# noway/nzcb-circom

Hardware: AMD Instinct MI355X
Metric: PLONK proofs/sec for nzcp_live (~2^21 constraints) at 1/2/4/8 MI355X (higher is better)
Workload: dtype u32 limbs: BN254 Fr/Fq Montgomery, 8x32-bit and 9x29-bit (MSM, NTT twiddles, quotient); 1 GPU; nzcp_live fullProve: NZCPPubIdentity(1,351,0,4,2,4) witness on the GPU (600560 signals) + PLONK proof, n=2^21, nPublic=3, 2970 inputs; domain_size=2097152, n_public=3, n_constraints=1785813, n_vars=1782570, n_additions=1182010, proofs_per_gpu=140, total_proofs=140, parallelism=batch-shard x1 (no collective), proofs_in_flight_per_gpu=5

## Files before the change

include/nzcb_internal.h:

```cpp
#ifndef NZCB_INTERNAL_H
#define NZCB_INTERNAL_H

#include "nzcb.h"

#ifdef __cplusplus
extern "C" {
#endif

int nzcb_ctx_kernel_stats(nzcb_ctx* ctx, int enable, double out[4]);

int nzcb_debug_guard_check(int device, size_t* checked, int* damaged, nzcb_err* err);
int nzcb_debug_guard_selftest(int device, nzcb_err* err);

#define NZCB_FAULT_QUOTIENT 1
#define NZCB_DEBUG_GENERIC_K 2
#define NZCB_FAULT_LANE_ALLOC 3
int nzcb_debug_inject_fault(nzcb_ctx* ctx, int kind);

int nzcb_debug_f29(int device, int op, const uint32_t* in, size_t count, uint32_t* out, nzcb_err* err);

int nzcb_synth_setup(int power, int n_public, int n_inputs, uint64_t seed, uint32_t n_constraints,
                     const uint8_t* tau, int device, uint8_t** zkey_out, size_t* zkey_len, uint8_t** wtns_out,
                     size_t* wtns_len, nzcb_err* err);
#define NZCB_SYNTH_FREE_PUBLIC 1u
int nzcb_synth_setup_ex(int power, int n_public, int n_inputs, uint64_t seed, uint32_t n_constraints, uint32_t flags,
                        const uint8_t* tau, int device, uint8_t** zkey_out, size_t* zkey_len, uint8_t** wtns_out,
                        size_t* wtns_len, nzcb_err* err);
typedef struct nzcb_engine nzcb_engine;
nzcb_engine* nzcb_engine_create(int device, int max_log_ntt, size_t max_msm_points, nzcb_err* err);
void nzcb_engine_destroy(nzcb_engine* e);
int nzcb_engine_ntt(nzcb_engine* e, const uint8_t* in_lem, uint8_t* out_lem, int log_n, int inverse, nzcb_err* err);
int nzcb_engine_msm(nzcb_engine* e, const uint8_t* bases_lem, const uint8_t* scalars, size_t n, int scalars_mont,
                    uint8_t* out_affine, nzcb_err* err);
int nzcb_debug_ntt_coset(nzcb_engine* e, const uint8_t* in_lem, uint8_t* out_lem, int log_n, const uint8_t* c_lem,
                         int fold_len, nzcb_err* err);
int nzcb_engine_ntt_dev(nzcb_engine* e, const void* in, void* out, int log_n, int inverse, nzcb_err* err);
int nzcb_engine_msm_dev(nzcb_engine* e, const void* bases, const void* scalars, size_t n, int scalars_mont,
                        uint8_t* out_affine, nzcb_err* err);
int nzcb_engine_time_ntt(nzcb_engine* e, const void* in, void* out, int log_n, int inverse, int reps, double* ms,
                         nzcb_err* err);
int nzcb_engine_random_fr(nzcb_engine* e, void* dev_out, size_t n, uint64_t seed, nzcb_err* err);
int nzcb_engine_fixed_base(nzcb_engine* e, const void* dev_scalars_mont, size_t n, void* dev_out, nzcb_err* err);
int nzcb_engine_lagrange_basis(nzcb_engine* e, const void* dev_ptau, size_t ptau_n, int log_n, void* dev_out,
                               nzcb_err* err);
int nzcb_engine_time_msm(nzcb_engine* e, const void* bases, const void* scalars, size_t n, int scalars_mont, int reps,
                         double* ms, double* acc_ms, nzcb_err* err);
int nzcb_engine_msm_fixed_dev(nzcb_engine* e, const void* bases, size_t n_table, const void* scalars, size_t n,
                              int scalars_mont, uint8_t* out_affine, nzcb_err* err);
int nzcb_engine_msm_table_dev(nzcb_engine* e, const void* bases, size_t n_table, const void* scalars, size_t n,
                              int scalars_mont, int window, int sparse, int fold, uint8_t* out_affine,
                              nzcb_err* err);
int nzcb_engine_msm_sets_dev(nzcb_engine* e, const void* bases, size_t n_table, const void* const* scalars, int sets,
                             size_t n, int scalars_mont, int sparse, uint8_t* out_affine, nzcb_err* err);
int nzcb_engine_time_msm2(nzcb_engine* e, const void* bases, const void* scalars, size_t n, int scalars_mont,
                          int fixed_base, int reps, double* out, nzcb_err* err);
int nzcb_engine_fr_mul(nzcb_engine* e, const uint8_t* a_lem, const uint8_t* b_lem, uint8_t* out_lem, size_t n,
                       int field_q, nzcb_err* err);

int nzcb_engine_g1_lincomb(int device, const uint8_t* points, const uint8_t* scalars, const uint32_t* group_end,
                           size_t groups, uint8_t* out, nzcb_err* err);
int nzcb_engine_verify_batch(const uint8_t* vk, const uint8_t* proofs, const uint8_t* pubs, size_t pub_stride,
                             int n_public, int count, int transcript_public, int device, const uint8_t* seed,
                             int* valid_out, uint8_t* points_out, int* pairing_checks, nzcb_err* err);
int nzcb_debug_verify_batch_timings(double* ms, int cap);

nzcb_r1cs* nzcb_engine_r1cs_create(const uint8_t* r1cs, size_t len, int device, uint32_t long_row_threshold,
                                   int witness_tile, nzcb_err* err);
int nzcb_debug_r1cs_check_timings(double* ms, int cap);

nzcb_p256_key* nzcb_engine_p256_key_create(const uint8_t pub_xy[64], int device, int window, nzcb_err* err);
#define NZCB_P256_OP_ADD 0
#define NZCB_P256_OP_SUB 1
#define NZCB_P256_OP_MUL 2
#define NZCB_P256_OP_SQR 3
#define NZCB_P256_OP_INV 4
int nzcb_debug_p256_field(int device, int op, int field, const uint8_t* a, const uint8_t* b, size_t count,
                          uint8_t* out, nzcb_err* err);
int nzcb_debug_p256_mul2(nzcb_p256_key* k, const uint8_t* u1, const uint8_t* u2, size_t count, uint8_t* out_xy,
                         nzcb_err* err);
int nzcb_debug_p256_timings(double* ms, int cap);

int nzcb_debug_nzcp_decode_timings(double* ms, int cap);

#ifdef __cplusplus
}
#endif
#endif
```

nzcb-circom_amd/csrc/capi_engine.hip:

```cpp
#include <chrono>
#include <cstring>
#include <map>
#include <memory>
#include <mutex>
#include <vector>

#include "../../include/nzcb_internal.h"
#include "engine.h"
#include "lagrange.h"

namespace nzcb {

Engine::Engine(int dev, int max_log_ntt, size_t max_msm_points) : device(dev) {
  NZ_HIP(hipSetDevice(dev));
  NZ_HIP(hipStreamCreateWithFlags(&stream, hipStreamNonBlocking));
  if (max_log_ntt >= 0) ntt_tables.init(max_log_ntt, stream);
  if (max_msm_points) msm_scratch.init(max_msm_points);
}

Engine::~Engine() {
  if (stream) (void)hipStreamDestroy(stream);
}

thread_local int g_guard_scope = 0;
// ... 8 lines not shown
  return m;
}
}

void guard_register(void* base, size_t bytes) {
  NZ_HIP(hipMemset((uint8_t*)base + bytes, kGuardByte, kGuardBytes));
  int dev = 0;
  NZ_HIP(hipGetDevice(&dev));
  std::lock_guard<std::mutex> lk(g_guard_mu);
  guard_map()[base] = GuardRec{bytes, dev};
}

void guard_unregister(void* base) {
  std::lock_guard<std::mutex> lk(g_guard_mu);
  guard_map().erase(base);
}

int guard_check(int device, size_t* checked, std::string* report) {
  std::vector<std::pair<void*, GuardRec>> recs;
  {
    std::lock_guard<std::mutex> lk(g_guard_mu);
    for (auto& kv : guard_map())
      if (device < 0 || kv.second.device == device) recs.push_back(kv);
  }
  std::vector<uint8_t> h(kGuardBytes);
  int bad = 0;
  for (auto& r : recs) {
    NZ_HIP(hipMemcpy(h.data(), (uint8_t*)r.first + r.second.bytes, kGuardBytes, hipMemcpyDeviceToHost));
    size_t k = 0;
    while (k < kGuardBytes && h[k] == kGuardByte) k++;
    if (k == kGuardBytes) continue;
    bad++;
    if (report && bad <= 8) {
      char line[160];
      std::snprintf(line, sizeof(line), "%sbuffer %p (%zu bytes, device %d): guard byte %zu overwritten",
                    report->empty() ? "" : "; ", r.first, r.second.bytes, r.second.device, k);
      *report += line;
    }
  }
  if (checked) *checked = recs.size();
  return bad;
}

__global__ void k_guard_poke(uint32_t* p, size_t at) {
  if (threadIdx.x == 0) p[at] = 0;
}

}

using namespace nzcb;

struct nzcb_engine {
  Engine eng;
  nzcb_engine(int d, int l, size_t m) : eng(d, l, m) {}
};

__global__ void fe_mul_kernel_r(const Fr* a, const Fr* b, Fr* o, size_t n) {
  size_t i = (size_t)blockIdx.x * blockDim.x + threadIdx.x;
  if (i < n) o[i] = a[i] * b[i];
}
__global__ void fe_mul_kernel_q(const Fq* a, const Fq* b, Fq* o, size_t n) {
  size_t i = (size_t)blockIdx.x * blockDim.x + threadIdx.x;
  if (i < n) o[i] = a[i] * b[i];
}

__global__ void random_fr_kernel(Fr* out, size_t n, uint64_t seed) {
  size_t i = (size_t)blockIdx.x * blockDim.x + threadIdx.x;
  if (i >= n) return;
  uint64_t x = seed ^ (0x9E3779B97F4A7C15ULL * (i + 1));
  Fr v;
  for (int k = 0; k < 4; k++) {
    x += 0x9E3779B97F4A7C15ULL;
    uint64_t z = x;
    z = (z ^ (z >> 30)) * 0xBF58476D1CE4E5B9ULL;
    z = (z ^ (z >> 27)) * 0x94D049BB133111EBULL;
    z ^= z >> 31;
    v.v[2 * k] = (uint32_t)z;
    v.v[2 * k + 1] = (uint32_t)(z >> 32);
  }
  v.v[7] &= 0x1fffffffu;
  out[i] = to_mont(v);
}

static void affine_out(const G1xyzz& r, uint8_t* out) {
  G1Affine a = xyzz_to_affine(r);
  Fq x = a.is_inf() ? Fq::zero() : from_mont(a.x);
  Fq y = a.is_inf() ? Fq::zero() : from_mont(a.y);
  std::memcpy(out, x.v, 32);
  std::memcpy(out + 32, y.v, 32);
}

extern "C" {

const char* nzcb_version(void) { return "nzcb-mi355x 0.1.0 (gfx950)"; }

int nzcb_device_count(void) {
  int n = 0;
  if (hipGetDeviceCount(&n) != hipSuccess) return 0;
  return n;
}

void nzcb_free(void* p) { std::free(p); }

nzcb_engine* nzcb_engine_create(int device, int max_log_ntt, size_t max_msm_points, nzcb_err* err) {
  return guarded_new<nzcb_engine>(
      err, [&] { return std::make_unique<nzcb_engine>(device, max_log_ntt, max_msm_points); });
}

void nzcb_engine_destroy(nzcb_engine* e) { delete e; }

void* nzcb_dev_alloc(size_t bytes) {
  void* p = nullptr;
  if (hipMalloc(&p, bytes) != hipSuccess) return nullptr;
  return p;
}
void* nzcb_dev_alloc_on(int device, size_t bytes) {
  int cur = 0;
  if (hipGetDevice(&cur) != hipSuccess || hipSetDevice(device) != hipSuccess) return nullptr;
  void* p = nullptr;
  if (hipMalloc(&p, bytes) != hipSuccess) p = nullptr;
  (void)hipSetDevice(cur);
  return p;
}
void nzcb_dev_free(void* p) {
  if (p) (void)hipFree(p);
}
int nzcb_memcpy_h2d(void* dst, const void* src, size_t bytes) {
  return hipMemcpy(dst, src, bytes, hipMemcpyHostToDevice) == hipSuccess ? 0 : NZCB_ERR_HIP;
}
int nzcb_memcpy_d2h(void* dst, const void* src, size_t bytes) {
  return hipMemcpy(dst, src, bytes, hipMemcpyDeviceToHost) == hipSuccess ? 0 : NZCB_ERR_HIP;
}
int nzcb_memcpy_d2d(void* dst, const void* src, size_t bytes) {
  if (hipMemcpyAsync(dst, src, bytes, hipMemcpyDeviceToDevice, nullptr) != hipSuccess) return NZCB_ERR_HIP;
  return hipStreamSynchronize(nullptr) == hipSuccess ? 0 : NZCB_ERR_HIP;
}
int nzcb_memcpy_d2d_async(void* dst, const void* src, size_t bytes, void* stream) {
  return hipMemcpyAsync(dst, src, bytes, hipMemcpyDeviceToDevice, (hipStream_t)stream) == hipSuccess ? 0
                                                                                              : NZCB_ERR_HIP;
}

int nzcb_engine_ntt_dev(nzcb_engine* e, const void* in, void* out, int log_n, int inverse, nzcb_err* err) {
  return guarded(err, [&] {
    Engine& g = e->eng;
    NZ_HIP(hipSetDevice(g.device));
    ntt(g.ntt_tables, (const Fr*)in, (Fr*)out, log_n, inverse != 0, g.stream);
    NZ_HIP(hipStreamSynchronize(g.stream));
  });
}

int nzcb_engine_ntt(nzcb_engine* e, const uint8_t* in_lem, uint8_t* out_lem, int log_n, int inverse, nzcb_err* err) {
  return guarded(err, [&] {
    Engine& g = e->eng;
    NZ_HIP(hipSetDevice(g.device));
    size_t n = size_t(1) << log_n;
    DevBuf<Fr> a(n), b(n);
    NZ_HIP(hipMemcpyAsync(a.p, in_lem, n * 32, hipMemcpyHostToDevice, g.stream));
    ntt(g.ntt_tables, a.p, b.p, log_n, inverse != 0, g.stream);
    NZ_HIP(hipMemcpyAsync(out_lem, b.p, n * 32, hipMemcpyDeviceToHost, g.stream));
    NZ_HIP(hipStreamSynchronize(g.stream));
  });
}

int nzcb_debug_ntt_coset(nzcb_engine* e, const uint8_t* in_lem, uint8_t* out_lem, int log_n, const uint8_t* c_lem,
                         int fold_len, nzcb_err* err) {
  return guarded(err, [&] {
    Engine& g = e->eng;
    if (log_n < 1 || log_n > g.ntt_tables.max_log || fold_len < 0 || (size_t)fold_len > (size_t(1) << log_n))
      throw Error(NZCB_ERR_ARG, "ntt coset: 1 <= log_n <= the engine's, 0 <= fold_len <= n");
    NZ_HIP(hipSetDevice(g.device));
    const size_t n = size_t(1) << log_n;
    Fr c;
    std::memcpy(c.v, c_lem, 32);
    DevBuf<Fr> a(n + (size_t)fold_len), b(n);
    DevBuf<NttTables::Tw> tw(n - 1);
    NZ_HIP(hipMemcpyAsync(a.p, in_lem, (n + (size_t)fold_len) * 32, hipMemcpyHostToDevice, g.stream));
    ntt_coset_twiddles(g.ntt_tables, c, log_n, tw.p, g.stream);
    NttIo io;
    io.in_len = n;
    io.tw = tw.p;
    if (fold_len) {
      Fr d = pow_u64(c, (uint64_t)n);
      for (int k = 0; k < 5; k++) d = d + d;
      io.fold_len = (size_t)fold_len;
      io.fold_n = n;
      io.fold_f = split29(d);
    }
    ntt(g.ntt_tables, a.p, b.p, log_n, false, g.stream, nullptr, &io);
    NZ_HIP(hipMemcpyAsync(out_lem, b.p, n * 32, hipMemcpyDeviceToHost, g.stream));
    NZ_HIP(hipStreamSynchronize(g.stream));
  });
}

int nzcb_engine_time_ntt(nzcb_engine* e, const void* in, void* out, int log_n, int inverse, int reps, double* ms,
                         nzcb_err* err) {
  return guarded(err, [&] {
    Engine& g = e->eng;
    NZ_HIP(hipSetDevice(g.device));
    hipEvent_t e0, e1;
    NZ_HIP(hipEventCreate(&e0));
    NZ_HIP(hipEventCreate(&e1));
    NZ_HIP(hipEventRecord(e0, g.stream));
    for (int i = 0; i < reps; i++) ntt(g.ntt_tables, (const Fr*)in, (Fr*)out, log_n, inverse != 0, g.stream);
    NZ_HIP(hipEventRecord(e1, g.stream));
    NZ_HIP(hipEventSynchronize(e1));
    float t = 0;
    NZ_HIP(hipEventElapsedTime(&t, e0, e1));
    *ms = t / (reps > 0 ? reps : 1);
    (void)hipEventDestroy(e0);
    (void)hipEventDestroy(e1);
  });
}

int nzcb_engine_msm_dev(nzcb_engine* e, const void* bases, const void* scalars, size_t n, int scalars_mont,
                        uint8_t* out_affine, nzcb_err* err) {
  return guarded(err, [&] {
    Engine& g = e->eng;
    NZ_HIP(hipSetDevice(g.device));
    G1xyzz r = msm(g.msm_scratch, (const G1Affine*)bases, (const Fr*)scalars, n, scalars_mont != 0, g.stream);
    affine_out(r, out_affine);
  });
}

int nzcb_engine_msm(nzcb_engine* e, const uint8_t* bases_lem, const uint8_t* scalars, size_t n, int scalars_mont,
                    uint8_t* out_affine, nzcb_err* err) {
  return guarded(err, [&] {
    Engine& g = e->eng;
    NZ_HIP(hipSetDevice(g.device));
    DevBuf<G1Affine> b(n ? n : 1);
    DevBuf<Fr> s(n ? n : 1);
    NZ_HIP(hipMemcpyAsync(b.p, bases_lem, n * 64, hipMemcpyHostToDevice, g.stream));
    NZ_HIP(hipMemcpyAsync(s.p, scalars, n * 32, hipMemcpyHostToDevice, g.stream));
    G1xyzz r = msm(g.msm_scratch, b.p, s.p, n, scalars_mont != 0, g.stream);
    affine_out(r, out_affine);
  });
}

int nzcb_engine_random_fr(nzcb_engine* e, void* dev_out, size_t n, uint64_t seed, nzcb_err* err) {
  return guarded(err, [&] {
    Engine& g = e->eng;
    NZ_HIP(hipSetDevice(g.device));
    hipLaunchKernelGGL(random_fr_kernel, dim3(grid_for(n, 256, 1u << 30)), dim3(256), 0, g.stream, (Fr*)dev_out, n,
                       seed);
    NZ_HIP(hipGetLastError());
    NZ_HIP(hipStreamSynchronize(g.stream));
  });
}

int nzcb_engine_fixed_base(nzcb_engine* e, const void* dev_scalars_mont, size_t n, void* dev_out, nzcb_err* err) {
  return guarded(err, [&] {
    Engine& g = e->eng;
    NZ_HIP(hipSetDevice(g.device));
    launch_fixed_base((const Fr*)dev_scalars_mont, n, (G1Affine*)dev_out, g.stream);
    NZ_HIP(hipStreamSynchronize(g.stream));
  });
}

int nzcb_engine_lagrange_basis(nzcb_engine* e, const void* dev_ptau, size_t ptau_n, int log_n, void* dev_out,
                               nzcb_err* err) {
  return guarded(err, [&] {
    Engine& g = e->eng;
    NZ_HIP(hipSetDevice(g.device));
    lagrange_basis((const G1Affine*)dev_ptau, ptau_n, log_n, (G1Affine*)dev_out, g.stream);
  });
}

int nzcb_engine_time_msm(nzcb_engine* e, const void* bases, const void* scalars, size_t n, int scalars_mont, int reps,
                         double* ms, double* acc_ms, nzcb_err* err) {
  return guarded(err, [&] {
    Engine& g = e->eng;
    NZ_HIP(hipSetDevice(g.device));
    MsmScratch& sc = g.msm_scratch;
    sc.prof = true;
    sc.prof_ms = 0;
    sc.prof_launches = 0;
    auto t0 = std::chrono::steady_clock::now();
    for (int i = 0; i < reps; i++)
      (void)msm(sc, (const G1Affine*)bases, (const Fr*)scalars, n, scalars_mont != 0, g.stream);
    *ms = std::chrono::duration<double, std::milli>(std::chrono::steady_clock::now() - t0).count() / (reps ? reps : 1);
    *acc_ms = sc.prof_ms / (sc.prof_launches ? sc.prof_launches : 1);
    sc.prof = false;
  });
}

int nzcb_engine_msm_fixed_dev(nzcb_engine* e, const void* bases, size_t n_table, const void* scalars, size_t n,
                              int scalars_mont, uint8_t* out_affine, nzcb_err* err) {
  return nzcb_engine_msm_table_dev(e, bases, n_table, scalars, n, scalars_mont, 0, 0, 0, out_affine, err);
}

int nzcb_engine_msm_table_dev(nzcb_engine* e, const void* bases, size_t n_table, const void* scalars, size_t n,
                              int scalars_mont, int window, int sparse, int fold, uint8_t* out_affine, nzcb_err* err) {
  return guarded(err, [&] {
    Engine& g = e->eng;
    NZ_HIP(hipSetDevice(g.device));
    if (n > n_table) throw Error(NZCB_ERR_ARG, "msm larger than its base table");
    if (window && (window < 16 || window > 20)) throw Error(NZCB_ERR_ARG, "msm table window: 16..20");
    MsmBaseTable t;
    t.build((const G1Affine*)bases, n_table, window ? window : fixed_base_window(), g.stream, fold != 0);
    t.sparse = sparse != 0;
    MsmScratch sc;
    sc.init(n ? n : 1, true);
    G1xyzz r = msm(sc, (const G1Affine*)bases, (const Fr*)scalars, n, scalars_mont != 0, g.stream, &t);
    affine_out(r, out_affine);
  });
}

int nzcb_engine_msm_sets_dev(nzcb_engine* e, const void* bases, size_t n_table, const void* const* scalars, int sets,
                             size_t n, int scalars_mont, int sparse, uint8_t* out_affine, nzcb_err* err) {
  return guarded(err, [&] {
    Engine& g = e->eng;
    NZ_HIP(hipSetDevice(g.device));
    if (n > n_table) throw Error(NZCB_ERR_ARG, "msm larger than its base table");
    if (sets < 1 || sets > 3 || !scalars) throw Error(NZCB_ERR_ARG, "msm sets: 1..3 scalar vectors");
    MsmBaseTable t;
    t.build((const G1Affine*)bases, n_table, lagrange_window(), g.stream);
    t.sparse = sparse != 0;
    MsmScratch sc;
    sc.init(n ? n : 1, true, 3, false);
    G1xyzz r[3] = {G1xyzz::inf(), G1xyzz::inf(), G1xyzz::inf()};
    msm_enqueue_sets(sc, (const Fr* const*)scalars, sets, n, scalars_mont != 0, g.stream, &t);
    msm_finish_sets(sc, g.stream, r);
    for (int k = 0; k < sets; k++) affine_out(r[k], out_affine + 64 * k);
  });
}

int nzcb_engine_time_msm2(nzcb_engine* e, const void* bases, const void* scalars, size_t n, int scalars_mont,
                          int fixed_base, int reps, double* out, nzcb_err* err) {
  return guarded(err, [&] {
    Engine& g = e->eng;
    NZ_HIP(hipSetDevice(g.device));
    std::unique_ptr<MsmBaseTable> t;
    std::unique_ptr<MsmScratch> own;
    MsmScratch* sc = &g.msm_scratch;
    double table_ms = 0;
    if (fixed_base) {
      auto t0 = std::chrono::steady_clock::now();
      t.reset(new MsmBaseTable());
      t->build((const G1Affine*)bases, n, fixed_base >= 2 ? lagrange_window() : fixed_base_window(), g.stream);
      t->sparse = fixed_base == 2;
      NZ_HIP(hipStreamSynchronize(g.stream));
      table_ms = std::chrono::duration<double, std::milli>(std::chrono::steady_clock::now() - t0).count();
      own.reset(new MsmScratch());
      own->init(n, true);
      sc = own.get();
    }
    sc->prof = true;
    sc->prof_phases = true;
    for (int w = 0; w < 3; w++)
      (void)msm(*sc, (const G1Affine*)bases, (const Fr*)scalars, n, scalars_mont != 0, g.stream, t.get());
    sc->prof_ms = 0;
    sc->prof_launches = 0;
    sc->prof_entries = 0;
    for (double& x : sc->phase_ms) x = 0;
    sc->host_ms = sc->enqueue_ms = sc->sort_host_ms = 0;
    auto t0 = std::chrono::steady_clock::now();
    for (int i = 0; i < reps; i++)
      (void)msm(*sc, (const G1Affine*)bases, (const Fr*)scalars, n, scalars_mont != 0, g.stream, t.get());
    const double r = reps > 0 ? reps : 1;
    out[0] = std::chrono::duration<double, std::milli>(std::chrono::steady_clock::now() - t0).count() / r;
    for (int i = 0; i < 7; i++) out[1 + i] = sc->phase_ms[i] / r;
    out[8] = table_ms;
    out[9] = (double)sc->prof_entries / r;
    out[10] = sc->host_ms / r;
    out[11] = sc->enqueue_ms / r;
    out[12] = sc->sort_host_ms / r;
    sc->prof = sc->prof_phases = false;
  });
}

int nzcb_engine_fr_mul(nzcb_engine* e, const uint8_t* a_lem, const uint8_t* b_lem, uint8_t* out_lem, size_t n,
                       int field_q, nzcb_err* err) {
  return guarded(err, [&] {
    Engine& g = e->eng;
    NZ_HIP(hipSetDevice(g.device));
    DevBuf<Fr> a(n), b(n), o(n);
    NZ_HIP(hipMemcpyAsync(a.p, a_lem, n * 32, hipMemcpyHostToDevice, g.stream));
    NZ_HIP(hipMemcpyAsync(b.p, b_lem, n * 32, hipMemcpyHostToDevice, g.stream));
    if (field_q)
      hipLaunchKernelGGL(fe_mul_kernel_q, dim3(grid_for(n, 256)), dim3(256), 0, g.stream, (const Fq*)a.p,
                         (const Fq*)b.p, (Fq*)o.p, n);
    else
      hipLaunchKernelGGL(fe_mul_kernel_r, dim3(grid_for(n, 256)), dim3(256), 0, g.stream, a.p, b.p, o.p, n);
    NZ_HIP(hipGetLastError());
    NZ_HIP(hipMemcpyAsync(out_lem, o.p, n * 32, hipMemcpyDeviceToHost, g.stream));
    NZ_HIP(hipStreamSynchronize(g.stream));
  });
}

struct nzcb_msm_table {
  int device = 0;
  size_t n = 0;
  MsmBaseTable table;
  MsmScratch sc;
  hipStream_t st = nullptr;
  ~nzcb_msm_table() {
    (void)hipSetDevice(device);
    if (st) (void)hipStreamDestroy(st);
  }
};

nzcb_msm_table* nzcb_msm_table_create(int device, const void* dev_bases, size_t n, nzcb_err* err) {
  return guarded_new<nzcb_msm_table>(err, [&] {
    if (!dev_bases || n == 0) throw Error(NZCB_ERR_ARG, "msm table: no bases");
    NZ_HIP(hipSetDevice(device));
    auto t = std::make_unique<nzcb_msm_table>();
    t->device = device;
    t->n = n;
    NZ_HIP(hipStreamCreateWithFlags(&t->st, hipStreamNonBlocking));
    t->table.build((const G1Affine*)dev_bases, n, fixed_base_window(), t->st);
    t->sc.init(n, true, 1, false);
    NZ_HIP(hipStreamSynchronize(t->st));
    return t;
  });
}

nzcb_msm_table* nzcb_msm_table_create_lagrange(int device, const void* dev_ptau, size_t ptau_n, int log_n, size_t lo,
                                               size_t hi, nzcb_err* err) {
  return guarded_new<nzcb_msm_table>(err, [&] {
    if (!dev_ptau || log_n < 1 || log_n > 28) throw Error(NZCB_ERR_ARG, "lagrange table: bad PTau or domain");
    const size_t nl = ((size_t)1 << log_n) + 2;
    if (ptau_n < nl) throw Error(NZCB_ERR_ARG, "lagrange table: fewer than n + 2 PTau points");
    if (lo >= hi || hi > nl) throw Error(NZCB_ERR_ARG, "lagrange table: bad point range");
    NZ_HIP(hipSetDevice(device));
    auto t = std::make_unique<nzcb_msm_table>();
    t->device = device;
    t->n = hi - lo;
    NZ_HIP(hipStreamCreateWithFlags(&t->st, hipStreamNonBlocking));
    {
      DevBuf<G1Affine> basis(nl);
      lagrange_basis((const G1Affine*)dev_ptau, ptau_n, log_n, basis.p, t->st);
      t->table.build(basis.p + lo, hi - lo, lagrange_window(), t->st);
      t->table.sparse = lagrange_sparse();
      NZ_HIP(hipStreamSynchronize(t->st));
    }
    t->sc.init(hi - lo, true, 1, false);
    return t;
  });
}

int nzcb_msm_table_run(nzcb_msm_table* t, const void* dev_scalars, size_t count, int scalars_mont,
                       uint8_t* out_affine, nzcb_err* err) {
  return guarded(err, [&] {
    if (!t || !out_affine || (count && !dev_scalars)) throw Error(NZCB_ERR_ARG, "msm table: null argument");
    if (count > t->n) throw Error(NZCB_ERR_ARG, "msm larger than its base table");
    NZ_HIP(hipSetDevice(t->device));
    G1xyzz r = count ? msm(t->sc, nullptr, (const Fr*)dev_scalars, count, scalars_mont != 0, t->st, &t->table)
                     : G1xyzz::inf();
    affine_out(r, out_affine);
  });
}

void nzcb_msm_table_destroy(nzcb_msm_table* t) { delete t; }

int nzcb_debug_guard_check(int device, size_t* checked, int* damaged, nzcb_err* err) {
  return guarded(err, [&] {
    std::string report;
    const int bad = guard_check(device, checked, &report);
    if (damaged) *damaged = bad;
    if (bad) throw Error(NZCB_ERR_INTERNAL, std::to_string(bad) + " damaged guard(s): " + report);
  });
}

int nzcb_debug_guard_selftest(int device, nzcb_err* err) {
  return guarded(err, [&] {
    NZ_HIP(hipSetDevice(device));
    size_t before = 0;
    guard_check(device, &before, nullptr);
    int bad = 0;
    {
      GuardScope gs;
      DevBuf<uint32_t> b(1000);
      hipLaunchKernelGGL(k_guard_poke, dim3(1), dim3(64), 0, nullptr, b.p, (size_t)1007);
      NZ_HIP(hipGetLastError());
      NZ_HIP(hipDeviceSynchronize());
      bad = guard_check(device, nullptr, nullptr);
    }
    const int after = guard_check(device, nullptr, nullptr);
    if (bad != 1 || after != 0)
      throw Error(NZCB_ERR_INTERNAL, "guard self-test: overrun found " + std::to_string(bad) + " time(s), " +
                                         std::to_string(after) + " left after release");
  });
}

}
```

nzcb-circom_amd/csrc/msm.h:

```cpp
#pragma once
#include <vector>

#include "common.h"
#include "ec.h"
#include "f29.h"

namespace nzcb {

struct MsmBaseTable {
  DevBuf<G1Affine> q;
  size_t n = 0, stride = 0;
  int c = 0, nw = 0;
  bool mont_folded = false;
  bool sparse = false;
  void build(const G1Affine* bases, size_t n, int c, hipStream_t st, bool fold_mont = false);
};

int fixed_base_window();
int lagrange_window();
bool lagrange_sparse();

struct MsmScratch {
  size_t max_points = 0;
  int max_lsets = 1;
  DevBuf<uint32_t> offsets;
  DevBuf<uint32_t> sorted;
  DevBuf<uint32_t> keys_in, keys_out, vals_in;
  DevBuf<uint8_t> sort_tmp;
  size_t sort_tmp_bytes = 0;
  DevBuf<uint32_t> bin_counts, vals_mid;
  DevBuf<uint32_t> lo_seg;
  DevBuf<G1xyzz> buckets;
  DevBuf<G1xyzz> carry_own;
  DevBuf<G1xyzz> carry_cont;
  DevBuf<Xyzz29> buckets29, carry_own29, carry_cont29;
  DevBuf<uint32_t> large;
  DevBuf<uint32_t> large_off;
  DevBuf<Xyzz29> large_part;
  DevBuf<Xyzz29> rowp29, colp29, lines29;
  DevBuf<G1xyzz> seg_tot;
  DevBuf<G1xyzz> seg_run;
  DevBuf<G1xyzz> parts;
  DevBuf<G1xyzz> win;
  G1xyzz* host_win = nullptr;
  uint32_t* host_total = nullptr;
  size_t host_win_cap = 0;
  int cur_c = 0, cur_nsets = 0, cur_nbits = 0, cur_seglen = 0;
  bool cur_fixed = false, cur_sparse = false;
  int cur_a = 0, cur_hb = 0;
  int cur_msets = 1;
  size_t cur_n = 0;
  uint32_t cur_nkeys = 0;
  bool prof = false, prof_phases = false;
  double prof_ms = 0;
  double phase_ms[7] = {0, 0, 0, 0, 0, 0, 0};
  double host_ms = 0;
  double enqueue_ms = 0;
  double sort_host_ms = 0;
  uint64_t prof_launches = 0, prof_points = 0, prof_entries = 0;
  hipEvent_t ev[8] = {nullptr, nullptr, nullptr, nullptr, nullptr, nullptr, nullptr, nullptr};
  hipEvent_t done = nullptr;
  void init(size_t max_points, bool fixed_base = false, int lagrange_sets = 1, bool generic = true);
  ~MsmScratch();
};

int msm_window_bits(size_t n);

void msm_enqueue(MsmScratch& sc, const G1Affine* bases, const Fr* scalars, size_t n, bool scalars_mont,
                 hipStream_t st, const MsmBaseTable* table = nullptr);
G1xyzz msm_finish(MsmScratch& sc, hipStream_t st);
void msm_enqueue_sets(MsmScratch& sc, const Fr* const* scalars, int sets, size_t n, bool scalars_mont,
                      hipStream_t st, const MsmBaseTable* table);
void msm_finish_sets(MsmScratch& sc, hipStream_t st, G1xyzz* out);

inline G1xyzz msm(MsmScratch& sc, const G1Affine* bases, const Fr* scalars, size_t n, bool mont, hipStream_t st,
                  const MsmBaseTable* table = nullptr) {
  msm_enqueue(sc, bases, scalars, n, mont, st, table);
  return msm_finish(sc, st);
}

G1Affine xyzz_to_affine(const G1xyzz& p);

}
```

nzcb-circom_amd/csrc/msm.hip:

```cpp
#include "msm.h"

#include "f29.h"

#include <chrono>
#include <cstdlib>
#include <type_traits>
#include <rocprim/rocprim.hpp>
#include <rocprofiler-sdk-roctx/roctx.h>

namespace nzcb {

static constexpr int kMsmThreads = 256;

#ifndef NZ_TAIL_PRIO
#define NZ_TAIL_PRIO 0
#endif
__device__ __forceinline__ void tail_prio() {
  if constexpr (NZ_TAIL_PRIO > 0) __builtin_amdgcn_s_setprio(NZ_TAIL_PRIO);
}

using SortConfig = rocprim::radix_sort_config<
    rocprim::default_config, rocprim::default_config,
    rocprim::radix_sort_onesweep_config<rocprim::kernel_config<1024, 16>, rocprim::kernel_config<1024, 16>, 10,
                                        rocprim::block_radix_rank_algorithm::match>>;

static void radix_sort(void* tmp, size_t& tmp_bytes, const uint32_t* kin, uint32_t* kout, const uint32_t* vin,
                       uint32_t* vout, size_t m, int end_bit, hipStream_t st) {
  NZ_HIP(rocprim::radix_sort_pairs<SortConfig>(tmp, tmp_bytes, kin, kout, vin, vout, m, 0, end_bit, st));
}

static constexpr uint32_t kChunk = 48;

static uint32_t chunk_for(size_t entries) {
  uint32_t c = kChunk;
  while (entries / c > (size_t(1) << 20)) c *= 2;
  return c;
}
static constexpr int kSegLen = 8;
static constexpr int kSumThreads = 256;
static constexpr int kSumPer = 4;
static constexpr int kPartThreads = 64;
static constexpr uint32_t kSeqSpan = 64;
static constexpr uint32_t kSeqSpan29 = 16;
static constexpr int kLargeBlocks = 32;
static constexpr int kLargePieceBlocks = 128;
static constexpr int kLargeFinalBlocks = 128;

static constexpr uint32_t kDynThreads = 1u << 18;
static constexpr uint32_t kDynMin = 8;
static constexpr uint32_t kSeqSpanSparse = 3;
static constexpr int kSparsePieceBlocks = 2048;
static constexpr int kSparseFinalBlocks = 512;
__host__ __device__ __forceinline__ uint32_t dyn_chunk(uint32_t m) {
  const uint32_t c = (m + kDynThreads - 1) / kDynThreads;
  return c < kDynMin ? kDynMin : c > kChunk ? kChunk : c;
}
static size_t dyn_threads_bound(size_t entries) {
  const size_t lo = std::min<size_t>(kDynThreads, (entries + kDynMin - 1) / kDynMin);
  return std::max<size_t>(lo, (entries + kChunk - 1) / kChunk);
}

static constexpr int kFbWindow = 20;
int fixed_base_window() {
  static const int c = [] {
    const char* e = std::getenv("NZCB_FB_WINDOW");
    const int v = e ? std::atoi(e) : kFbWindow;
    return (v >= 16 && v <= 20) ? v : kFbWindow;
  }();
  return c;
}

#ifndef NZ_LAGRANGE_WINDOW
#define NZ_LAGRANGE_WINDOW 17
#endif
int lagrange_window() { return NZ_LAGRANGE_WINDOW; }
bool lagrange_sparse() {
  static const bool v = [] {
    const char* e = std::getenv("NZCB_SPARSE");
    return e && std::atoi(e) != 0;
  }();
  return v;
}

int msm_window_bits(size_t n) {
  if (n >= (size_t(1) << 18)) return 16;
  int lg = ilog2(n ? n : 1);
  int c = lg - 3;
  if (c < 4) c = 4;
  if (c > 16) c = 16;
  return c;
}

static inline int num_windows(int c) { return (255 + c - 1) / c; }

template <int C, class F>
__device__ __forceinline__ void for_each_digit(const Fr& s, F&& f) {
  constexpr int NW = (255 + C - 1) / C;
  constexpr uint32_t MASK = (1u << C) - 1u;
  constexpr uint32_t HALF = 1u << (C - 1);
  uint32_t carry = 0;
#pragma unroll
  for (int w = 0; w < NW; w++) {
    const int bit = w * C;
    const int limb = bit >> 5;
    const int sh = bit & 31;
    uint64_t x = s.v[limb];
    if (limb + 1 < 8) x |= (uint64_t)s.v[limb + 1] << 32;
    uint32_t d = ((uint32_t)(x >> sh) & MASK) + carry;
    if (d > HALF) {
      uint32_t mag = (MASK + 1u) - d;
      if (mag) f(w, mag - 1u, 1u);
      carry = 1;
    } else {
      if (d) f(w, d - 1u, 0u);
      carry = 0;
    }
  }
}

#ifdef NZCB_MSM_STATS
template <class F>
static void for_each_digit_host(const Fr& s, int C, F&& f) {
  const int NW = (255 + C - 1) / C;
  const uint32_t MASK = (1u << C) - 1u, HALF = 1u << (C - 1);
  uint32_t carry = 0;
  for (int w = 0; w < NW; w++) {
    const int bit = w * C, limb = bit >> 5, sh = bit & 31;
    uint64_t x = s.v[limb];
    if (limb + 1 < 8) x |= (uint64_t)s.v[limb + 1] << 32;
    uint32_t d = ((uint32_t)(x >> sh) & MASK) + carry;
    if (d > HALF) {
      uint32_t mag = (MASK + 1u) - d;
      if (mag) f(w, mag - 1u, 1u);
      carry = 1;
    } else {
      if (d) f(w, d - 1u, 0u);
      carry = 0;
    }
  }
}
#endif

template <int C>
__global__ void __launch_bounds__(kMsmThreads)
msm_keys_kernel(const Fr* __restrict__ scalars, size_t n, int mont, uint32_t* __restrict__ keys,
                uint32_t* __restrict__ vals) {
  constexpr int NW = (255 + C - 1) / C;
  constexpr uint32_t NB = 1u << (C - 1);
  constexpr uint32_t SENTINEL = NW * NB;
  for (size_t i = (size_t)blockIdx.x * blockDim.x + threadIdx.x; i < n; i += (size_t)gridDim.x * blockDim.x) {
    Fr s = scalars[i];
    if (mont) s = from_mont_fr29(s);
    uint32_t k[NW];
#pragma unroll
    for (int w = 0; w < NW; w++) k[w] = SENTINEL;
    uint32_t sg[NW];
#pragma unroll
    for (int w = 0; w < NW; w++) sg[w] = 0;
    for_each_digit<C>(s, [&](int w, uint32_t b, uint32_t sign) {
      k[w] = (uint32_t)w * NB + b;
      sg[w] = sign << 31;
    });
#pragma unroll
    for (int w = 0; w < NW; w++) {
      keys[(size_t)w * n + i] = k[w];
      vals[(size_t)w * n + i] = (uint32_t)i | sg[w];
    }
  }
}

static constexpr int kBinThreads = 256;
static constexpr int kBinPer = 2;
static constexpr uint32_t kTileScalars = kBinThreads * kBinPer;
static constexpr int kLoThreads = 512;

static constexpr int kDigMont = 1;
static constexpr int kDigMinForm = 2;

__device__ __forceinline__ uint32_t scalar_min_form(Fr& s) {
  constexpr uint32_t H[8] = {0xf8000000u, 0xa1f0fac9u, 0x3cdcb848u, 0x9419f424u,
                             0x40c0ac2eu, 0xdc2822dbu, 0x7098d014u, 0x18322739u};
  bool gt = false, eq = true, lt_r = false, eq_r = true;
#pragma unroll
  for (int l = 7; l >= 0; l--) {
    gt = gt || (eq && s.v[l] > H[l]);
    eq = eq && s.v[l] == H[l];
    lt_r = lt_r || (eq_r && s.v[l] < FrParams::P[l]);
    eq_r = eq_r && s.v[l] == FrParams::P[l];
  }
  if (!(gt && lt_r)) return 0u;
  s = neg(s);
  return 1u;
}

template <int C, int NW>
__device__ __forceinline__ uint32_t bin_entries(const Fr* __restrict__ scalars, size_t i, int mont, size_t stride,
                                                uint32_t (&kk)[NW], uint32_t (&vv)[NW]) {
  Fr s = scalars[i];
  if (mont & kDigMont) s = from_mont_fr29(s);
  const uint32_t flip = (mont & kDigMinForm) ? scalar_min_form(s) : 0u;
  uint32_t live = 0;
#pragma unroll
  for (int w = 0; w < NW; w++) {
    kk[w] = 0;
    vv[w] = 0;
  }
  for_each_digit<C>(s, [&](int w, uint32_t b, uint32_t sign) {
    kk[w] = b;
    vv[w] = (uint32_t)((size_t)w * stride + i) | ((sign ^ flip) << 31);
    live |= 1u << w;
  });
  return live;
}

template <int KB> struct BinKeys {
  static constexpr int LO = KB - 8 > 8 ? KB - 8 : 8;
  using Lo = typename std::conditional<LO <= 8, uint8_t, uint16_t>::type;
  using Full = typename std::conditional<KB <= 16, uint16_t, uint32_t>::type;
};

static constexpr int kMaxSets = 3;
struct BinSets {
  const Fr* p[kMaxSets];
  uint32_t tps;
  uint32_t nb;
};

template <int C, int KB>
__global__ void __launch_bounds__(kBinThreads)
msm_bin_hist_kernel(BinSets sets, size_t n, int mont, uint32_t* __restrict__ counts, uint32_t ntiles) {
  constexpr int NW = (255 + C - 1) / C;
  constexpr int LO = BinKeys<KB>::LO;
  __shared__ uint32_t h[256];
  h[threadIdx.x] = 0;
  __syncthreads();
  const uint32_t set = blockIdx.x / sets.tps, lt = blockIdx.x - set * sets.tps;
  const Fr* __restrict__ scalars = sets.p[set];
  const uint32_t kbase = set * sets.nb;
#pragma unroll
  for (int j = 0; j < kBinPer; j++) {
    const size_t i = (size_t)lt * kTileScalars + (size_t)j * kBinThreads + threadIdx.x;
    if (i < n) {
      uint32_t kk[NW], vv[NW];
      const uint32_t live = bin_entries<C, NW>(scalars, i, mont, 0, kk, vv);
#pragma unroll
      for (int w = 0; w < NW; w++)
        if ((live >> w) & 1u) atomicAdd(&h[(kk[w] + kbase) >> LO], 1u);
    }
  }
  __syncthreads();
  counts[(size_t)threadIdx.x * ntiles + blockIdx.x] = h[threadIdx.x];
}

__device__ __forceinline__ uint32_t wave_incl_scan(uint32_t v) {
  const int lane = threadIdx.x & 63;
#pragma unroll
  for (int off = 1; off < 64; off <<= 1) {
    const uint32_t u = __shfl_up(v, off, 64);
    if (lane >= off) v += u;
  }
  return v;
}

__device__ __forceinline__ uint32_t scan256_excl(uint32_t v, uint32_t* wsum4, uint32_t& total) {
  const uint32_t inc = wave_incl_scan(threadIdx.x < 256 ? v : 0u);
  if (threadIdx.x < 256 && (threadIdx.x & 63) == 63) wsum4[threadIdx.x >> 6] = inc;
  __syncthreads();
  uint32_t off = 0;
  for (int w = 0; w < (int)(threadIdx.x >> 6) && w < 4; w++) off += wsum4[w];
  total = wsum4[0] + wsum4[1] + wsum4[2] + wsum4[3];
  __syncthreads();
  return threadIdx.x < 256 ? off + inc - v : 0u;
}

__global__ void __launch_bounds__(256)
msm_bin_rowscan_kernel(uint32_t* __restrict__ counts, uint32_t ntiles, uint32_t* __restrict__ tail) {
  __shared__ uint32_t wsum[4];
  uint32_t* row = counts + (size_t)blockIdx.x * ntiles;
  uint32_t carry = 0;
  for (uint32_t c0 = 0; c0 < ntiles; c0 += 256) {
    const uint32_t t = c0 + threadIdx.x;
    const uint32_t v = t < ntiles ? row[t] : 0u;
    uint32_t tot;
    const uint32_t ex = scan256_excl(v, wsum, tot);
    if (t < ntiles) row[t] = carry + ex;
    carry += tot;
  }
  if (threadIdx.x == 0) tail[blockIdx.x] = carry;
}

template <int C, int KB>
__global__ void __launch_bounds__(kBinThreads)
msm_bin_scatter_kernel(BinSets sets, size_t n, int mont, size_t stride, const uint32_t* __restrict__ counts,
                       uint32_t ntiles, typename BinKeys<KB>::Lo* __restrict__ lo2, uint32_t* __restrict__ vals2) {
  constexpr int NW = (255 + C - 1) / C;
  constexpr int TE = kTileScalars * NW;
  constexpr int LO = BinKeys<KB>::LO;
  __shared__ uint32_t lcount[256], lstart[256], gbase[256];
  __shared__ uint32_t lval[TE];
  __shared__ typename BinKeys<KB>::Full lkey[TE];
  const uint32_t set = blockIdx.x / sets.tps, lt = blockIdx.x - set * sets.tps;
  const Fr* __restrict__ scalars = sets.p[set];
  const uint32_t kbase = set * sets.nb;
  __shared__ uint32_t wsum[4];
  const uint32_t* tail = counts + (size_t)256 * ntiles;
  {
    uint32_t tot;
    const uint32_t st = scan256_excl(tail[threadIdx.x], wsum, tot);
    gbase[threadIdx.x] = st + counts[(size_t)threadIdx.x * ntiles + blockIdx.x];
    lcount[threadIdx.x] = 0;
  }
  __syncthreads();
  uint32_t kk[kBinPer][NW], vv[kBinPer][NW], rk[kBinPer][NW], live[kBinPer];
#pragma unroll
  for (int j = 0; j < kBinPer; j++) {
    const size_t i = (size_t)lt * kTileScalars + (size_t)j * kBinThreads + threadIdx.x;
    live[j] = 0;
    if (i < n) {
      live[j] = bin_entries<C, NW>(scalars, i, mont, stride, kk[j], vv[j]);
#pragma unroll
      for (int w = 0; w < NW; w++) {
        kk[j][w] += kbase;
        if ((live[j] >> w) & 1u) rk[j][w] = atomicAdd(&lcount[kk[j][w] >> LO], 1u);
      }
    }
  }
  __syncthreads();
  uint32_t total;
  {
    lstart[threadIdx.x] = scan256_excl(lcount[threadIdx.x], wsum, total);
  }
  __syncthreads();
#pragma unroll
  for (int j = 0; j < kBinPer; j++) {
#pragma unroll
    for (int w = 0; w < NW; w++) {
      if ((live[j] >> w) & 1u) {
        const uint32_t q = lstart[kk[j][w] >> LO] + rk[j][w];
        lkey[q] = (typename BinKeys<KB>::Full)kk[j][w];
        lval[q] = vv[j][w];
      }
    }
  }
  __syncthreads();
  for (uint32_t q = threadIdx.x; q < total; q += kBinThreads) {
    const uint32_t key = lkey[q], hb = key >> LO;
    const uint32_t pos = gbase[hb] + (q - lstart[hb]);
    lo2[pos] = (typename BinKeys<KB>::Lo)(key & ((1u << LO) - 1u));
    vals2[pos] = lval[q];
  }
}

template <int NT>
__device__ __forceinline__ uint32_t block_scan_excl(uint32_t* a, uint32_t count, uint32_t* wsum) {
  const uint32_t per = (count + NT - 1) / NT;
  const uint32_t b = threadIdx.x * per;
  uint32_t loc = 0;
  for (uint32_t i = 0; i < per; i++)
    if (b + i < count) loc += a[b + i];
  const uint32_t inc = wave_incl_scan(loc);
  if ((threadIdx.x & 63) == 63) wsum[threadIdx.x >> 6] = inc;
  __syncthreads();
  uint32_t off = 0, tot = 0;
#pragma unroll
  for (int w = 0; w < NT / 64; w++) {
    if (w < (int)(threadIdx.x >> 6)) off += wsum[w];
    tot += wsum[w];
  }
  uint32_t run = off + inc - loc;
  for (uint32_t i = 0; i < per; i++)
    if (b + i < count) {
      const uint32_t v = a[b + i];
      a[b + i] = run;
      run += v;
    }
  __syncthreads();
  return tot;
}

static constexpr uint32_t kLoSeg = 32768;
static constexpr uint32_t kLoU = 8;

__device__ __forceinline__ void lo_regions(const uint32_t* __restrict__ tail, uint32_t* wsum, uint32_t* rs,
                                           uint32_t* rf) {
  const uint32_t t = threadIdx.x;
  const uint32_t cnt = t < 256 ? tail[t] : 0u;
  uint32_t tot, nitems;
  const uint32_t st = scan256_excl(cnt, wsum, tot);
  const uint32_t f = scan256_excl((cnt + kLoSeg - 1) / kLoSeg, wsum, nitems);
  if (t < 256) {
    rs[t] = st;
    rf[t] = f;
  }
  if (t == 0) rf[256] = nitems;
  __syncthreads();
}

__device__ __forceinline__ uint32_t lo_region_of(const uint32_t* rf, uint32_t item) {
  uint32_t lo = 0, hi = 256;
  while (hi - lo > 1) {
    const uint32_t mid = (lo + hi) >> 1;
    if (rf[mid] <= item) lo = mid; else hi = mid;
  }
  return lo;
}

template <int LO>
__global__ void __launch_bounds__(kLoThreads)
msm_lo_count_kernel(const typename std::conditional<LO <= 8, uint8_t, uint16_t>::type* __restrict__ lo2,
                    const uint32_t* __restrict__ counts, uint32_t ntiles, uint32_t* __restrict__ segoff) {
  constexpr uint32_t NL = 1u << LO;
  __shared__ uint32_t h[NL], wsum[kLoThreads / 64], rs[256], rf[257];
  lo_regions(counts + (size_t)256 * ntiles, wsum, rs, rf);
  const uint32_t item = blockIdx.x;
  if (item >= rf[256]) return;
  const uint32_t r = lo_region_of(rf, item);
  const uint32_t* tail = counts + (size_t)256 * ntiles;
  const uint32_t s = rs[r] + (item - rf[r]) * kLoSeg;
  const uint32_t e = min(rs[r] + tail[r], s + kLoSeg);
  for (uint32_t i = threadIdx.x; i < NL; i += kLoThreads) h[i] = 0;
  __syncthreads();
  for (uint32_t p0 = s; p0 < e; p0 += kLoU * kLoThreads) {
    uint32_t k8[kLoU];
#pragma unroll
    for (uint32_t u = 0; u < kLoU; u++) {
      const uint32_t q = p0 + u * kLoThreads + threadIdx.x;
      k8[u] = q < e ? (uint32_t)lo2[q] : NL;
    }
#pragma unroll
    for (uint32_t u = 0; u < kLoU; u++)
      if (k8[u] < NL) atomicAdd(&h[k8[u]], 1u);
  }
  __syncthreads();
  for (uint32_t i = threadIdx.x; i < NL; i += kLoThreads) segoff[(size_t)item * NL + i] = h[i];
}

template <int LO>
__global__ void __launch_bounds__(kLoThreads)
msm_lo_scan_kernel(const uint32_t* __restrict__ counts, uint32_t ntiles, uint32_t* __restrict__ segoff,
                   uint32_t nkeys, uint32_t* __restrict__ offsets, uint32_t* __restrict__ large) {
  constexpr uint32_t NL = 1u << LO;
  __shared__ uint32_t h[NL], wsum[kLoThreads / 64], rs[256], rf[257];
  const uint32_t* tail = counts + (size_t)256 * ntiles;
  lo_regions(tail, wsum, rs, rf);
  const uint32_t hb = blockIdx.x;
  const uint32_t f0 = rf[hb], ns = rf[hb + 1] - f0, s = rs[hb];
  for (uint32_t i = threadIdx.x; i < NL; i += kLoThreads) {
    uint32_t run = 0;
    for (uint32_t g = 0; g < ns; g++) {
      uint32_t* c = segoff + (size_t)(f0 + g) * NL + i;
      const uint32_t v = *c;
      *c = run;
      run += v;
    }
    h[i] = run;
  }
  __syncthreads();
  block_scan_excl<kLoThreads>(h, NL, wsum);
  for (uint32_t i = threadIdx.x; i < NL; i += kLoThreads) {
    const uint32_t base = s + h[i];
    const uint32_t key = (hb << LO) | i;
    if (key < nkeys) offsets[key] = base;
    for (uint32_t g = 0; g < ns; g++) segoff[(size_t)(f0 + g) * NL + i] += base;
  }
  if (hb == 255 && threadIdx.x == 0) offsets[nkeys] = s + tail[255];
  if (hb == 0 && threadIdx.x == 0) large[0] = 0;
}

template <int LO, int NT = kLoThreads, uint32_t U = kLoU>
__global__ void __launch_bounds__(NT)
msm_lo_scatter_kernel(const typename std::conditional<LO <= 8, uint8_t, uint16_t>::type* __restrict__ lo2,
                      const uint32_t* __restrict__ vals2, const uint32_t* __restrict__ counts, uint32_t ntiles,
                      const uint32_t* __restrict__ segoff, uint32_t* __restrict__ sorted) {
  using Lo = typename std::conditional<LO <= 8, uint8_t, uint16_t>::type;
  constexpr uint32_t NL = 1u << LO;
  constexpr uint32_t kLoThreads = NT, kLoU = U;
  __shared__ uint32_t h[NL], lcnt[NL], lst[NL];
  __shared__ uint32_t wsum[kLoThreads / 64], rs[256], rf[257];
  __shared__ uint32_t lv[kLoU * kLoThreads];
  __shared__ Lo lk[kLoU * kLoThreads];
  lo_regions(counts + (size_t)256 * ntiles, wsum, rs, rf);
  const uint32_t item = blockIdx.x;
  if (item >= rf[256]) return;
  const uint32_t r = lo_region_of(rf, item);
  const uint32_t* tail = counts + (size_t)256 * ntiles;
  const uint32_t s = rs[r] + (item - rf[r]) * kLoSeg;
  const uint32_t e = min(rs[r] + tail[r], s + kLoSeg);
  for (uint32_t i = threadIdx.x; i < NL; i += kLoThreads) h[i] = segoff[(size_t)item * NL + i];
  for (uint32_t p0 = s; p0 < e; p0 += kLoU * kLoThreads) {
    uint32_t k8[kLoU], v8[kLoU], r8[kLoU];
    for (uint32_t i = threadIdx.x; i < NL; i += kLoThreads) lcnt[i] = 0;
    __syncthreads();
#pragma unroll
    for (uint32_t u = 0; u < kLoU; u++) {
      const uint32_t q = p0 + u * kLoThreads + threadIdx.x;
      k8[u] = q < e ? (uint32_t)lo2[q] : NL;
      v8[u] = q < e ? vals2[q] : 0u;
    }
#pragma unroll
    for (uint32_t u = 0; u < kLoU; u++) r8[u] = k8[u] < NL ? atomicAdd(&lcnt[k8[u]], 1u) : 0u;
    __syncthreads();
    for (uint32_t i = threadIdx.x; i < NL; i += kLoThreads) lst[i] = lcnt[i];
    __syncthreads();
    block_scan_excl<kLoThreads>(lst, NL, wsum);
#pragma unroll
    for (uint32_t u = 0; u < kLoU; u++)
      if (k8[u] < NL) {
        const uint32_t q = lst[k8[u]] + r8[u];
        lk[q] = (Lo)k8[u];
        lv[q] = v8[u];
      }
    __syncthreads();
    const uint32_t cnt = e - p0 < kLoU * kLoThreads ? e - p0 : kLoU * kLoThreads;
    for (uint32_t q = threadIdx.x; q < cnt; q += kLoThreads) {
      const uint32_t k = lk[q];
      sorted[h[k] + (q - lst[k])] = lv[q];
    }
    __syncthreads();
    for (uint32_t i = threadIdx.x; i < NL; i += kLoThreads) h[i] += lcnt[i];
  }
}

__global__ void __launch_bounds__(kMsmThreads)
msm_offsets_kernel(const uint32_t* __restrict__ skeys, size_t m, uint32_t nkeys, uint32_t* __restrict__ offsets) {
  size_t k = (size_t)blockIdx.x * blockDim.x + threadIdx.x;
  if (k > nkeys) return;
  size_t lo = 0, hi = m;
  while (lo < hi) {
    size_t mid = (lo + hi) >> 1;
    if (skeys[mid] < k) lo = mid + 1; else hi = mid;
  }
  offsets[k] = (uint32_t)lo;
}

__device__ __forceinline__ uint32_t find_key(const uint32_t* __restrict__ offsets, uint32_t nkeys, uint32_t pos) {
  uint32_t lo = 0, hi = nkeys;
  while (hi - lo > 1) {
    uint32_t mid = (lo + hi) >> 1;
    if (offsets[mid] <= pos) lo = mid; else hi = mid;
  }
  return lo;
}

__global__ void __launch_bounds__(kMsmThreads)
msm_accumulate_kernel(uint32_t chunk, const G1Affine* __restrict__ bases, const uint32_t* __restrict__ sorted,
                      const uint32_t* __restrict__ offsets, uint32_t nkeys, size_t nthreads,
                      G1xyzz* __restrict__ buckets, G1xyzz* __restrict__ carry_own,
                      G1xyzz* __restrict__ carry_cont) {
  size_t t = (size_t)blockIdx.x * blockDim.x + threadIdx.x;
  if (t >= nthreads) return;
  const uint32_t M = offsets[nkeys];
  const uint32_t s = (uint32_t)t * chunk;
  if (s >= M) return;
  const uint32_t e = (s + chunk < M) ? s + chunk : M;
  uint32_t k = find_key(offsets, nkeys, s);
  uint32_t kstart = offsets[k], kend = offsets[k + 1];
  G1xyzz acc = G1xyzz::inf();
  for (uint32_t pos = s; pos < e;) {
    const uint32_t ent = sorted[pos];
    const G1Affine P = bases[ent & 0x7fffffffu];
    if (!P.is_inf()) {
      Fq y = (ent >> 31) ? neg(P.y) : P.y;
      acc = xyzz_add_affine(acc, P.x, y);
    }
    pos++;
    if (pos == kend || pos == e) {
      const bool starts = kstart >= s;
      const bool ends = kend <= e;
      if (starts && ends) buckets[k] = acc;
      else if (!starts) carry_cont[t] = acc;
      else carry_own[t] = acc;
      acc = G1xyzz::inf();
      if (pos < e) {
        k = find_key(offsets, nkeys, pos);
        kstart = offsets[k];
        kend = offsets[k + 1];
      }
    }
  }
}

static __device__ __forceinline__ void mdbl29_rare(const F29& x, const F29& y, Xyzz29* out) { *out = mdbl29(x, y); }

__device__ __forceinline__ G1xyzz load_point(const G1xyzz& p) { return p; }
__device__ __forceinline__ G1xyzz load_point(const Xyzz29& a) {
  uint32_t z = 0;
#pragma unroll
  for (int i = 0; i < 9; i++) z |= a.ZZ.v[i];
  if (!z) return G1xyzz::inf();
  G1xyzz r;
  r.X = to_fq256(a.X);
  r.Y = to_fq256(a.Y);
  r.ZZ = to_fq256(a.ZZ);
  r.ZZZ = to_fq256(a.ZZZ);
  return r;
}

static constexpr uint32_t kLdsStride = kMsmThreads + 1;
template <bool kLdsIdx>
__global__ void __launch_bounds__(kMsmThreads) __attribute__((amdgpu_waves_per_eu(3, 8)))
msm_accumulate29_kernel(uint32_t chunk, const G1Affine* __restrict__ bases, const uint32_t* __restrict__ sorted,
                        const uint32_t* __restrict__ offsets, uint32_t nkeys, size_t nthreads,
                        Xyzz29* __restrict__ buckets, Xyzz29* __restrict__ carry_own,
                        Xyzz29* __restrict__ carry_cont) {
  __shared__ uint32_t sidx[kLdsIdx ? kChunk * kLdsStride : 1];
  const uint32_t t = blockIdx.x * blockDim.x + threadIdx.x;
  const uint32_t M = offsets[nkeys];
  if (!chunk) {
    chunk = dyn_chunk(M);
    tail_prio();
  }
  if (kLdsIdx) {
    const uint32_t wg0 = (uint32_t)blockIdx.x * kMsmThreads * chunk;
    if (wg0 >= M) return;
    const uint32_t inv = (uint32_t)((0x100000000ull + chunk - 1) / chunk);
    for (uint32_t j = threadIdx.x; j < kMsmThreads * chunk; j += kMsmThreads) {
      const uint32_t thr = __umulhi(j, inv), slot = j - thr * chunk;
      sidx[slot * kLdsStride + thr] = wg0 + j < M ? sorted[wg0 + j] : 0u;
    }
    __syncthreads();
  }
  if (t >= nthreads) return;
  const uint32_t s = (uint32_t)t * chunk;
  if (s >= M) return;
  const uint32_t e = (s + chunk < M) ? s + chunk : M;
  auto index_at = [&](uint32_t q) -> uint32_t {
    return kLdsIdx ? sidx[(q - s) * kLdsStride + threadIdx.x] : sorted[q];
  };
  uint32_t k = find_key(offsets, nkeys, s);
  uint32_t kstart = offsets[k], kend = offsets[k + 1];
  Xyzz29 acc;
  bool inf = true;
  uint32_t ent = index_at(s);
  G1Affine P = bases[ent & 0x7fffffffu];
  uint32_t ent_n = s + 1 < e ? index_at(s + 1) : 0u;
  for (uint32_t pos = s; pos < e;) {
    G1Affine Pn;
    uint32_t ent_nn = 0;
    if (pos + 1 < e) Pn = bases[ent_n & 0x7fffffffu];
    if (pos + 2 < e) ent_nn = index_at(pos + 2);
    if (!P.is_inf()) {
      const F29 x = split29(P.x);
      F29 y = split29(P.y);
      if (ent >> 31) y = neg29_nn(y);
      if (inf) {
        norm29(y);
        acc.X = x;
        acc.Y = y;
        acc.ZZ = f29_const(Fq29::ONE);
        acc.ZZZ = f29_const(Fq29::ONE);
        inf = false;
      } else {
        F29 U2, S2, PP, RR;
        mul29x2<Fq29>(x, acc.ZZ, y, acc.ZZZ, U2, S2);
        const F29 Pd = sub29(U2, acc.X, Fq29::K8);
        const F29 R = sub29(S2, acc.Y, Fq29::K4);
        sqr29x2(Pd, R, PP, RR);
        if (is0p29_fast(PP)) {
          if (is0p29(RR)) {
            norm29(y);
            mdbl29_rare(x, y, &acc);
          } else {
            inf = true;
          }
        } else {
          F29 PPP, Q, ZZ3, ZZZ3;
          mul29x2<Fq29>(Pd, PP, acc.X, PP, PPP, Q);
          const F29 X3 = sub2x29(RR, PPP, Q);
          mul29x2<Fq29>(acc.ZZ, PP, acc.ZZZ, PPP, ZZ3, ZZZ3);
          acc.Y = mul2sum29(R, sub29_nn(Q, X3, Fq29W::K10), neg4p29_nn(acc.Y), PPP);
          acc.ZZ = ZZ3;
          acc.ZZZ = ZZZ3;
          acc.X = X3;
        }
      }
    }
    pos++;
    if (pos == kend || pos == e) {
      const bool starts = kstart >= s;
      const bool ends = kend <= e;
      Xyzz29 out = acc;
      if (inf)
#pragma unroll
        for (int i = 0; i < 9; i++) out.ZZ.v[i] = 0;
      if (starts && ends) buckets[k] = out;
      else if (!starts) carry_cont[t] = out;
      else carry_own[t] = out;
      inf = true;
      while (pos < e && kend <= pos) {
        k++;
        kstart = kend;
        kend = offsets[k + 1];
      }
    }
    ent = ent_n;
    ent_n = ent_nn;
    P = Pn;
  }
}


__device__ __forceinline__ G1xyzz sum_run(const G1xyzz* carry_own, const G1xyzz* carry_cont, uint32_t c0,
                                          uint32_t c1) {
  G1xyzz v = carry_own[c0];
  for (uint32_t u = c0 + 1; u <= c1; u++) v = xyzz_add(v, carry_cont[u]);
  return v;
}

__global__ void __launch_bounds__(kMsmThreads)
msm_bucket_finalize_kernel(uint32_t chunk, const uint32_t* __restrict__ offsets, uint32_t nkeys, uint32_t span,
                           const G1xyzz* __restrict__ carry_own, const G1xyzz* __restrict__ carry_cont,
                           G1xyzz* __restrict__ buckets, uint32_t* __restrict__ large) {
  const size_t k = (size_t)blockIdx.x * blockDim.x + threadIdx.x;
  if (k >= nkeys) return;
  const uint32_t s = offsets[k], e = offsets[k + 1];
  if (e == s) return;
  const uint32_t c0 = s / chunk, c1 = (e - 1) / chunk;
  if (c0 == c1) return;
  if (c1 - c0 > span) {
    large[1 + atomicAdd(&large[0], 1u)] = (uint32_t)k;
    return;
  }
  buckets[k] = sum_run(carry_own, carry_cont, c0, c1);
}

__global__ void __launch_bounds__(kMsmThreads)
msm_finalize29_kernel(uint32_t chunk, const uint32_t* __restrict__ offsets, uint32_t nkeys, uint32_t span,
                      const Xyzz29* __restrict__ carry_own, const Xyzz29* __restrict__ carry_cont,
                      uint32_t* __restrict__ large, Xyzz29* __restrict__ out29) {
  tail_prio();
  __shared__ uint32_t pk[kMsmThreads], pu[kMsmThreads], pe[kMsmThreads];
  __shared__ uint32_t cnt;
  if (threadIdx.x == 0) cnt = 0;
  if (!chunk) chunk = dyn_chunk(offsets[nkeys]);
  __syncthreads();
  const size_t k = (size_t)blockIdx.x * blockDim.x + threadIdx.x;
  uint32_t c0 = 0, c1 = 0;
  bool mine = false;
  if (k < nkeys) {
    const uint32_t s = offsets[k], e = offsets[k + 1];
    if (e != s) {
      c0 = s / chunk;
      c1 = (e - 1) / chunk;
      if (c1 - c0 > span)
        large[1 + atomicAdd(&large[0], 1u)] = (uint32_t)k;
      else
        mine = c1 > c0;
    }
  }
  if (mine) {
    out29[k] = add29(carry_own[c0], carry_cont[c0 + 1]);
    if (c1 > c0 + 1) {
      const uint32_t i = atomicAdd(&cnt, 1u);
      pk[i] = (uint32_t)k;
      pu[i] = c0 + 2;
      pe[i] = c1;
    }
  }
  __syncthreads();
  if (threadIdx.x < cnt) {
    const uint32_t kk = pk[threadIdx.x], u1 = pe[threadIdx.x];
    Xyzz29 v = out29[kk];
    for (uint32_t u = pu[threadIdx.x]; u <= u1; u++) v = add29(v, carry_cont[u]);
    out29[kk] = v;
  }
}

__global__ void __launch_bounds__(kMsmThreads)
msm_bucket_reduce_kernel(const G1xyzz* __restrict__ buckets, const uint32_t* __restrict__ offsets, int nb,
                         int seglen, int nseg, int nsets, G1xyzz* __restrict__ seg_tot, G1xyzz* __restrict__ seg_run) {
  size_t t = (size_t)blockIdx.x * blockDim.x + threadIdx.x;
  if (t >= (size_t)nsets * nseg) return;
  const int w = (int)(t / nseg);
  const int g = (int)(t % nseg);
  const size_t base = (size_t)w * nb + (size_t)g * seglen;
  G1xyzz run = G1xyzz::inf(), tot = G1xyzz::inf();
  for (int j = seglen - 1; j >= 0; j--) {
    const uint32_t k = (uint32_t)(base + j);
    if (offsets[k + 1] != offsets[k]) run = xyzz_add(run, buckets[k]);
    if (!run.is_inf()) tot = xyzz_add(tot, run);
  }
  seg_tot[t] = tot;
  seg_run[t] = run;
}

__device__ __forceinline__ G1xyzz padd(const G1xyzz& a, const G1xyzz& b) { return xyzz_add(a, b); }
__device__ __forceinline__ Xyzz29 padd(const Xyzz29& a, const Xyzz29& b) { return add29(a, b); }
template <class P> __device__ __forceinline__ P pinf();
template <> __device__ __forceinline__ G1xyzz pinf<G1xyzz>() { return G1xyzz::inf(); }
template <> __device__ __forceinline__ Xyzz29 pinf<Xyzz29>() {
  Xyzz29 r;
#pragma unroll
  for (int i = 0; i < 9; i++) r.X.v[i] = r.Y.v[i] = r.ZZ.v[i] = r.ZZZ.v[i] = 0;
  return r;
}

template <int T, class Load, class Pt = G1xyzz>
__device__ __forceinline__ Pt block_sum(int per, Pt* sh, Load&& load) {
  constexpr int LG = T == 256 ? 8 : T == 128 ? 7 : T == 64 ? 6 : 5;
  const int tid = threadIdx.x;
  Pt acc = pinf<Pt>();
  for (int step = 0; step < per + LG; step++) {
    if (step == per) {
      sh[tid] = acc;
      __syncthreads();
    }
    bool doit;
    Pt lhs, rhs;
    if (step < per) {
      doit = load(step, rhs);
      lhs = acc;
    } else {
      const int stride = (T >> 1) >> (step - per);
      doit = tid < stride;
      if (doit) {
        lhs = sh[tid];
        rhs = sh[tid + stride];
      }
    }
    Pt r;
    if (doit) r = padd(lhs, rhs);
    if (step < per) {
      if (doit) acc = r;
    } else {
      if (doit) sh[tid] = r;
      __syncthreads();
    }
  }
  return sh[0];
}

__global__ void __launch_bounds__(kSumThreads)
msm_bucket_large_kernel(uint32_t chunk, const uint32_t* __restrict__ offsets, const uint32_t* __restrict__ large,
                        const G1xyzz* __restrict__ carry_own, const G1xyzz* __restrict__ carry_cont,
                        G1xyzz* __restrict__ buckets) {
  __shared__ G1xyzz sh[kSumThreads];
  const uint32_t count = large[0];
  for (uint32_t i = blockIdx.x; i < count; i += gridDim.x) {
    const uint32_t k = large[1 + i];
    const uint32_t c0 = offsets[k] / chunk, c1 = (offsets[k + 1] - 1) / chunk;
    const uint32_t span = c1 - c0 + 1;
    const int per = (int)((span + kSumThreads - 1) / kSumThreads);
    const G1xyzz r = block_sum<kSumThreads>(per, sh, [&](int step, G1xyzz& rhs) {
      const uint32_t u = (uint32_t)step * kSumThreads + threadIdx.x;
      if (u >= span) return false;
      rhs = u ? carry_cont[c0 + u] : carry_own[c0];
      return true;
    });
    if (threadIdx.x == 0) buckets[k] = r;
    __syncthreads();
  }
}

static constexpr uint32_t kPieceCarries = (uint32_t)kSumThreads;

__device__ __forceinline__ uint32_t carry_span(uint32_t chunk, const uint32_t* offsets, uint32_t k, uint32_t* c0) {
  *c0 = offsets[k] / chunk;
  return (offsets[k + 1] - 1) / chunk - *c0 + 1;
}

__global__ void __launch_bounds__(1024)
msm_large_scan_kernel(uint32_t chunk, const uint32_t* __restrict__ offsets, uint32_t nkeys,
                      const uint32_t* __restrict__ large, uint32_t* __restrict__ off) {
  tail_prio();
  __shared__ uint32_t sh[1024];
  const uint32_t count = large[0];
  const uint32_t ch = chunk ? chunk : dyn_chunk(offsets[nkeys]);
  const uint32_t tid = threadIdx.x;
  const uint32_t per = (count + 1023u) / 1024u;
  const uint32_t i0 = tid * per < count ? tid * per : count;
  const uint32_t i1 = i0 + per < count ? i0 + per : count;
  auto pieces = [&](uint32_t i) {
    uint32_t c0;
    return (carry_span(ch, offsets, large[1 + i], &c0) + kPieceCarries - 1) / kPieceCarries;
  };
  uint32_t sum = 0;
  for (uint32_t i = i0; i < i1; i++) sum += pieces(i);
  sh[tid] = sum;
  __syncthreads();
  for (uint32_t d = 1; d < 1024; d <<= 1) {
    const uint32_t v = tid >= d ? sh[tid - d] : 0u;
    __syncthreads();
    sh[tid] += v;
    __syncthreads();
  }
  uint32_t base = sh[tid] - sum;
  for (uint32_t i = i0; i < i1; i++) {
    off[i] = base;
    base += pieces(i);
  }
  if (tid == 1023) off[count] = sh[1023];
}

__device__ __forceinline__ Xyzz29 tree_sum29(Xyzz29 v, uint32_t cnt, Xyzz29* sh) {
  const uint32_t u = threadIdx.x;
  uint32_t h = 1;
  while (h < cnt) h <<= 1;
  h >>= 1;
  if (h) {
    if (u >= h && u < cnt) sh[u] = v;
    __syncthreads();
  }
  for (; h; h >>= 1) {
    if (u < h && u + h < cnt) v = add29(v, sh[u + h]);
    cnt = h;
    if (h > 1) {
      if (u >= (h >> 1) && u < h) sh[u] = v;
      __syncthreads();
    }
  }
  return v;
}

__global__ void __launch_bounds__(kSumThreads)
msm_large_piece29_kernel(uint32_t chunk, const uint32_t* __restrict__ offsets, uint32_t nkeys,
                         const uint32_t* __restrict__ large, const uint32_t* __restrict__ off,
                         const Xyzz29* __restrict__ carry_own, const Xyzz29* __restrict__ carry_cont,
                         Xyzz29* __restrict__ part) {
  tail_prio();
  __shared__ Xyzz29 sh[kSumThreads];
  const uint32_t count = large[0];
  const uint32_t total = off[count];
  const uint32_t ch = chunk ? chunk : dyn_chunk(offsets[nkeys]);
  for (uint32_t item = blockIdx.x; item < total; item += gridDim.x) {
    uint32_t lo = 0, hi = count;
    while (hi - lo > 1) {
      const uint32_t mid = (lo + hi) >> 1;
      if (off[mid] <= item) lo = mid; else hi = mid;
    }
    uint32_t c0;
    const uint32_t span = carry_span(ch, offsets, large[1 + lo], &c0);
    const uint32_t first = (item - off[lo]) * kPieceCarries;
    const uint32_t n = span - first < kPieceCarries ? span - first : kPieceCarries;
    const uint32_t u = first + threadIdx.x;
    Xyzz29 v;
    if (threadIdx.x < n) v = u ? carry_cont[c0 + u] : carry_own[c0];
    v = tree_sum29(v, n, sh);
    if (threadIdx.x == 0) part[item] = v;
    __syncthreads();
  }
}

template <int NT>
__global__ void __launch_bounds__(NT)
msm_large_final29_kernel(const uint32_t* __restrict__ large, const uint32_t* __restrict__ off,
                         const Xyzz29* __restrict__ part, Xyzz29* __restrict__ out29) {
  tail_prio();
  __shared__ Xyzz29 sh[NT];
  const uint32_t count = large[0];
  for (uint32_t i = blockIdx.x; i < count; i += gridDim.x) {
    const uint32_t p0 = off[i], np = off[i + 1] - p0;
    if (np == 1) {
      if (threadIdx.x == 0) out29[large[1 + i]] = part[p0];
      continue;
    }
    Xyzz29 v;
    if (threadIdx.x < np) v = part[p0 + threadIdx.x];
    for (uint32_t q = threadIdx.x + NT; q < np; q += NT) v = add29(v, part[p0 + q]);
    v = tree_sum29(v, np < NT ? np : NT, sh);
    if (threadIdx.x == 0) out29[large[1 + i]] = v;
    __syncthreads();
  }
}

__global__ void __launch_bounds__(kSumThreads)
msm_sums_kernel(const G1xyzz* __restrict__ seg_tot, const G1xyzz* __restrict__ seg_run, int nseg, int nslots,
                int nparts, G1xyzz* __restrict__ parts) {
  __shared__ G1xyzz sh[kSumThreads];
  const int p = blockIdx.x % nparts;
  const int wj = blockIdx.x / nparts;
  const int j = wj % nslots;
  const int w = wj / nslots;
  const int count = j == 0 ? nseg : nseg >> 1;
  const G1xyzz r = block_sum<kSumThreads>(kSumPer, sh, [&](int step, G1xyzz& rhs) {
    const int q = (p * kSumPer + step) * kSumThreads + (int)threadIdx.x;
    if (q >= count) return false;
    int g = q;
    if (j) {
      const int b = j - 1;
      g = ((q >> b) << (b + 1)) | (1 << b) | (q & ((1 << b) - 1));
    }
    rhs = j ? seg_run[(size_t)w * nseg + g] : seg_tot[(size_t)w * nseg + g];
    return true;
  });
  if (threadIdx.x == 0) parts[blockIdx.x] = r;
}

__global__ void __launch_bounds__(kPartThreads)
msm_parts_kernel(const G1xyzz* __restrict__ parts, int nparts, G1xyzz* __restrict__ out) {
  __shared__ G1xyzz sh[kPartThreads];
  const int per = (nparts + kPartThreads - 1) / kPartThreads;
  const G1xyzz r = block_sum<kPartThreads>(per, sh, [&](int step, G1xyzz& rhs) {
    const int q = step * kPartThreads + (int)threadIdx.x;
    if (q >= nparts) return false;
    rhs = parts[(size_t)blockIdx.x * nparts + q];
    return true;
  });
  if (threadIdx.x == 0) out[blockIdx.x] = r;
}

static constexpr int kTileSide = 16;
static constexpr int kLineThreads = 8;

__global__ void __launch_bounds__(256)
msm_tile29_kernel(const Xyzz29* __restrict__ buckets, const uint32_t* __restrict__ offsets, int a, int ltiles,
                  int htiles, Xyzz29* __restrict__ rowp, Xyzz29* __restrict__ colp) {
  tail_prio();
  __shared__ Xyzz29 sh[384];
  const int tid = threadIdx.x;
  const int ht = blockIdx.x / ltiles, lt = blockIdx.x - ht * ltiles;
  {
    const size_t per = (size_t)ltiles * htiles * kTileSide;
    buckets += (size_t)blockIdx.y * ltiles * htiles * kTileSide * kTileSide;
    offsets += (size_t)blockIdx.y * ltiles * htiles * kTileSide * kTileSide;
    rowp += blockIdx.y * per;
    colp += blockIdx.y * per;
  }
  {
    const int i = tid >> 4, j = tid & 15;
    const uint32_t k = ((uint32_t)(ht * kTileSide + i) << a) + (uint32_t)(lt * kTileSide + j);
    sh[tid] = offsets[k + 1] != offsets[k] ? buckets[k] : pinf<Xyzz29>();
  }
  __syncthreads();
#pragma unroll 1
  for (int s = 0; s < 4; s++) {
    const int m = 8 >> s;
    const bool act = tid < 32 * m;
    int l = 0, r = 0, d = 0;
    if (tid < 16 * m) {
      const int i = tid / m, j = tid - i * m;
      l = d = i * 16 + j;
      r = l + m;
    } else if (act) {
      const int u = tid - 16 * m, i = u >> 4, j = u & 15;
      const int base = s ? 256 : 0;
      l = base + i * 16 + j;
      r = base + (i + m) * 16 + j;
      d = 256 + i * 16 + j;
    }
    Xyzz29 x, y;
    if (act) {
      x = sh[l];
      y = sh[r];
    }
    __syncthreads();
    if (act) sh[d] = add29(x, y);
    __syncthreads();
  }
  if (tid < kTileSide)
    rowp[(size_t)(ht * kTileSide + tid) * ltiles + lt] = sh[tid * 16];
  else if (tid < 2 * kTileSide)
    colp[(size_t)(lt * kTileSide + tid - kTileSide) * htiles + ht] = sh[256 + tid - kTileSide];
}

static constexpr int kStrip = 16;
static constexpr int kStripMinC = 19;
__global__ void __launch_bounds__(256)
msm_strips29_kernel(const Xyzz29* __restrict__ buckets, const uint32_t* __restrict__ offsets, int a, int hb,
                    Xyzz29* __restrict__ rowp, Xyzz29* __restrict__ colp) {
  tail_prio();
  const int RJ = (1 << a) / kStrip, CI = (1 << hb) / kStrip;
  const size_t nrow = (size_t)RJ << hb, ncol = (size_t)CI << a;
  const size_t g = (size_t)blockIdx.x * 256 + threadIdx.x;
  if (g >= nrow + ncol) return;
  uint32_t k, step;
  size_t dst;
  Xyzz29* out;
  if (g < nrow) {
    const uint32_t h = (uint32_t)(g / RJ), j = (uint32_t)(g % RJ);
    k = (h << a) + j;
    step = (uint32_t)RJ;
    dst = g;
    out = rowp;
  } else {
    const size_t u = g - nrow;
    const uint32_t i = (uint32_t)(u >> a), l = (uint32_t)(u & ((1u << a) - 1));
    k = (i << a) + l;
    step = (uint32_t)CI << a;
    dst = (size_t)l * CI + i;
    out = colp;
  }
  Xyzz29 acc = pinf<Xyzz29>();
#pragma unroll 1
  for (int t = 0; t < kStrip; t++, k += step) {
    const Xyzz29 y = offsets[k + 1] != offsets[k] ? buckets[k] : pinf<Xyzz29>();
    acc = add29(acc, y);
  }
  out[dst] = acc;
}

__device__ __forceinline__ Xyzz29 shfl_xor29(const Xyzz29& v, int m) {
  Xyzz29 o;
#pragma unroll
  for (int i = 0; i < 9; i++) {
    o.X.v[i] = __shfl_xor(v.X.v[i], m);
    o.Y.v[i] = __shfl_xor(v.Y.v[i], m);
    o.ZZ.v[i] = __shfl_xor(v.ZZ.v[i], m);
    o.ZZZ.v[i] = __shfl_xor(v.ZZZ.v[i], m);
  }
  return o;
}

__global__ void __launch_bounds__(256)
msm_lines29_kernel(const Xyzz29* __restrict__ rowp, int ltiles, const Xyzz29* __restrict__ colp, int htiles,
                   int nrows, int ncols, Xyzz29* __restrict__ lines) {
  tail_prio();
  rowp += (size_t)blockIdx.y * nrows * ltiles;
  colp += (size_t)blockIdx.y * ncols * htiles;
  lines += (size_t)blockIdx.y * (nrows + ncols);
  constexpr int LG = kLineThreads == 8 ? 3 : kLineThreads == 4 ? 2 : kLineThreads == 16 ? 4 : 1;
  static_assert((1 << LG) == kLineThreads, "kLineThreads: 2, 4, 8 or 16");
  const int g = (int)((blockIdx.x * 256 + threadIdx.x) / kLineThreads);
  const int r = (int)(threadIdx.x & (kLineThreads - 1));
  const bool live = g < nrows + ncols;
  const bool row = g < nrows;
  const Xyzz29* src = row ? rowp + (size_t)g * ltiles : colp + (size_t)(g - nrows) * htiles;
  const int cnt = live ? (row ? ltiles : htiles) : 0;
  const int maxcnt = ltiles > htiles ? ltiles : htiles;
  const int nseq = (maxcnt + kLineThreads - 1) / kLineThreads - 1;
  Xyzz29 acc = r < cnt ? src[r] : pinf<Xyzz29>();
#pragma unroll 1
  for (int step = 0; step < nseq + LG; step++) {
    Xyzz29 y;
    if (step < nseq) {
      const int q = r + (step + 1) * kLineThreads;
      y = q < cnt ? src[q] : pinf<Xyzz29>();
    } else {
      y = shfl_xor29(acc, 1 << (step - nseq));
    }
    acc = add29(acc, y);
  }
  if (live && r == 0) lines[g] = acc;
}

__global__ void __launch_bounds__(kSumThreads)
msm_slots29_kernel(const Xyzz29* __restrict__ lines, int hb, int a, G1xyzz* __restrict__ out,
                   const uint32_t* __restrict__ entries, uint32_t* __restrict__ total_out) {
  tail_prio();
  lines += (size_t)blockIdx.y * (((size_t)1 << hb) + ((size_t)1 << a));
  out += (size_t)blockIdx.y * (hb + a + 1);
  __shared__ Xyzz29 sh[kSumThreads];
  const int s = blockIdx.x;
  const bool rows = s < hb;
  const bool plain = s == hb + a;
  const int b = rows ? s : s - hb;
  const int count = plain ? 1 << a : (rows ? 1 << (hb - 1) : 1 << (a - 1));
  const Xyzz29* src = rows ? lines : lines + ((size_t)1 << hb);
  const int per = (count + kSumThreads - 1) / kSumThreads;
  const Xyzz29 r = block_sum<kSumThreads>(per, sh, [&](int step, Xyzz29& rhs) {
    const int q = step * kSumThreads + (int)threadIdx.x;
    if (q >= count) return false;
    rhs = src[plain ? q : (((q >> b) << (b + 1)) | (1 << b) | (q & ((1 << b) - 1)))];
    return true;
  });
  if (threadIdx.x == 0) {
    host_put(out + s, load_point(r));
    if (s == 0 && blockIdx.y == 0 && total_out) host_put(total_out, *entries);
    host_put_done();
  }
}

__global__ void __launch_bounds__(kMsmThreads)
msm_table_kernel(const G1Affine* __restrict__ bases, size_t n, size_t stride, int c, int nw, Fq k261, int fold,
                 Fr kinv, G1Affine* __restrict__ q) {
  const size_t i = (size_t)blockIdx.x * blockDim.x + threadIdx.x;
  if (i >= n) return;
  const G1Affine P = bases[i];
  if (P.is_inf()) {
    for (int w = 0; w < nw; w++) q[(size_t)w * stride + i] = P;
    return;
  }
  G1xyzz acc = xyzz_from_affine(P);
  if (fold) {
    acc = G1xyzz::inf();
    for (int b = 253; b >= 0; b--) {
      acc = xyzz_dbl(acc);
      if ((kinv.v[b >> 5] >> (b & 31)) & 1u) acc = xyzz_add_affine(acc, P.x, P.y);
    }
  }
  for (int w = 0; w < nw; w++) {
    if (w)
      for (int k = 0; k < c; k++) acc = xyzz_dbl(acc);
    const Fq ti = inverse(acc.ZZ * acc.ZZZ);
    G1Affine r;
    r.x = acc.X * (acc.ZZZ * ti) * k261;
    r.y = acc.Y * (acc.ZZ * ti) * k261;
    q[(size_t)w * stride + i] = r;
  }
}

void MsmBaseTable::build(const G1Affine* bases, size_t npts, int cbits, hipStream_t st, bool fold_mont) {
  n = npts;
  mont_folded = fold_mont;
  stride = npts;
  c = cbits;
  nw = num_windows(c);
  if ((size_t)nw * stride >= (size_t(1) << 31)) throw Error(NZCB_ERR_ARG, "msm table too large for 31-bit indices");
  q.alloc((size_t)nw * stride);
  Fq thirty_two = Fq::zero();
  thirty_two.v[0] = 32;
  const Fq k261 = to_mont(thirty_two);
  Fr one_raw = Fr::zero();
  one_raw.v[0] = 1;
  const Fr kinv = from_mont(one_raw);
  hipLaunchKernelGGL(msm_table_kernel, dim3(grid_for(n, kMsmThreads, 1u << 30)), dim3(kMsmThreads), 0, st, bases, n,
                     stride, c, nw, k261, fold_mont ? 1 : 0, kinv, q.p);
  NZ_HIP(hipGetLastError());
}

static void lmark(const char* what) {
  static const bool on = std::getenv("NZCB_MARK_LAUNCHES") != nullptr;
  if (on) roctxMarkA(what);
}

static size_t lo_items_bound(size_t entries) { return 256 + entries / kLoSeg + 1; }

struct MsmPlan {
  int c, nw, nsets, seglen, nseg, nbits, nslots, nparts;
  int lb, a, hb, ltiles, htiles;
  int msets;
  uint32_t nb, nkeys;
  size_t entries;
};

static MsmPlan make_plan(size_t n, const MsmBaseTable* t, int msets = 1) {
  MsmPlan p;
  p.c = t ? t->c : msm_window_bits(n);
  p.nw = num_windows(p.c);
  p.nsets = t ? 1 : p.nw;
  p.msets = t ? msets : 1;
  p.nb = 1u << (p.c - 1);
  p.nkeys = p.nb * (uint32_t)p.nsets * (uint32_t)p.msets;
  p.seglen = (int)(p.nb < (uint32_t)kSegLen ? p.nb : kSegLen);
  p.nseg = (int)(p.nb / p.seglen);
  p.nbits = 0;
  while ((1 << p.nbits) < p.nseg) p.nbits++;
  p.nslots = p.nbits + 1;
  p.nparts = (p.nseg + kSumThreads * kSumPer - 1) / (kSumThreads * kSumPer);
  p.lb = p.c - 1;
  p.a = (p.lb + 1) / 2;
  p.hb = p.lb - p.a;
  p.ltiles = (1 << p.a) / kTileSide;
  p.htiles = (1 << p.hb) / kTileSide;
  p.entries = n * (size_t)p.nw * (size_t)p.msets;
  return p;
}

void MsmScratch::init(size_t maxp, bool fixed_base, int lagrange_sets, bool generic) {
  if (lagrange_sets < 1 || lagrange_sets > kMaxSets) throw Error(NZCB_ERR_ARG, "msm scratch: 1..3 Lagrange sets");
  if (!fixed_base) generic = true;
  max_points = maxp;
  max_lsets = lagrange_sets;
  size_t max_entries = 0, max_keys = 0, max_seg = 0, max_slots = 0, max_parts = 0, max_tiles = 0, max_lines = 0;
  auto fit = [&](const MsmPlan& p) {
    max_entries = std::max(max_entries, p.entries);
    max_keys = std::max(max_keys, (size_t)p.nkeys);
    if (p.nsets == 1) {
      max_slots = std::max(max_slots, (size_t)(p.lb + 1) * p.msets);
      max_tiles = std::max(max_tiles, (size_t)p.nb / kTileSide * p.msets);
      max_lines = std::max(max_lines, (((size_t)1 << p.hb) + ((size_t)1 << p.a)) * p.msets);
    } else {
      max_seg = std::max(max_seg, (size_t)p.nseg * p.nsets);
      max_slots = std::max(max_slots, (size_t)p.nslots * p.nsets);
      max_parts = std::max(max_parts, (size_t)p.nslots * p.nsets * p.nparts);
    }
  };
  for (size_t n = 1;; n <<= 1) {
    size_t m = n < maxp ? n : maxp;
    fit(make_plan(m, nullptr));
    if (m == maxp) break;
  }
  MsmPlan fp{};
  if (fixed_base) {
    MsmBaseTable t;
    t.c = fixed_base_window();
    fp = make_plan(maxp, &t);
    fit(fp);
    t.c = lagrange_window();
    const MsmPlan lp = make_plan(maxp, &t, lagrange_sets);
    fit(lp);
    if (lp.entries > fp.entries) fp = lp;
  }
  const size_t ge = generic ? max_entries : 1;
  offsets.alloc(max_keys + 1);
  sorted.alloc(max_entries);
  keys_in.alloc(ge);
  keys_out.alloc(max_entries);
  vals_in.alloc(ge);
  sort_tmp_bytes = 0;
  if (generic) {
    radix_sort(nullptr, sort_tmp_bytes, keys_in.p, keys_out.p, vals_in.p, sorted.p, max_entries, 21, nullptr);
  }
  sort_tmp.alloc(sort_tmp_bytes + 16);
  const size_t nthreads = std::max((max_entries + kChunk - 1) / kChunk, dyn_threads_bound(max_entries)) + 1;
  buckets.alloc(generic ? max_keys : 1);
  carry_own.alloc(generic ? nthreads : 1);
  carry_cont.alloc(generic ? nthreads : 1);
  large.alloc(max_keys + 1);
  if (fixed_base) {
    buckets29.alloc(max_keys);
    large_off.alloc(max_keys + 2);
    large_part.alloc(nthreads / kPieceCarries + max_keys + 1);
    carry_own29.alloc(nthreads);
    carry_cont29.alloc(nthreads);
    rowp29.alloc(max_tiles);
    colp29.alloc(max_tiles);
    lines29.alloc(max_lines);
    bin_counts.alloc((size_t)256 * ((maxp + kTileScalars - 1) / kTileScalars) * lagrange_sets + 256);
    vals_mid.alloc(max_entries);
    lo_seg.alloc(lo_items_bound(max_entries) * ((size_t)1 << BinKeys<19>::LO));
  }
  seg_tot.alloc(max_seg && generic ? max_seg : 1);
  seg_run.alloc(max_seg && generic ? max_seg : 1);
  parts.alloc(max_parts && generic ? max_parts : 1);
  win.alloc(max_slots);
  host_win_cap = max_slots;
  NZ_HIP(hipHostMalloc((void**)&host_win, (max_slots + 1) * sizeof(G1xyzz), hipHostMallocCoherent));
  host_total = (uint32_t*)(host_win + max_slots);
}

MsmScratch::~MsmScratch() {
  if (host_win) (void)hipHostFree(host_win);
  if (done) (void)hipEventDestroy(done);
  for (auto& e : ev)
    if (e) (void)hipEventDestroy(e);
}

static void keys_dispatch(int c, const Fr* scalars, size_t n, int mont, MsmScratch& sc, hipStream_t st) {
  auto launch = [&](auto cc) {
    constexpr int C = decltype(cc)::value;
    hipLaunchKernelGGL(msm_keys_kernel<C>, dim3(grid_for(n, kMsmThreads, 1u << 30)), dim3(kMsmThreads), 0, st,
                       scalars, n, mont, sc.keys_in.p, sc.vals_in.p);
  };
  switch (c) {
#define NZ_CASE(K) case K: launch(std::integral_constant<int, K>()); break;
    NZ_CASE(4) NZ_CASE(5) NZ_CASE(6) NZ_CASE(7) NZ_CASE(8) NZ_CASE(9) NZ_CASE(10) NZ_CASE(11) NZ_CASE(12)
    NZ_CASE(13) NZ_CASE(14) NZ_CASE(15) NZ_CASE(16)
#undef NZ_CASE
    default: throw Error(NZCB_ERR_INTERNAL, "bad msm window");
  }
  NZ_HIP(hipGetLastError());
}

G1Affine xyzz_to_affine(const G1xyzz& p) {
  G1Affine r;
  if (p.is_inf()) {
    r.x = Fq::zero();
    r.y = Fq::zero();
    return r;
  }
  r.x = p.X * inverse(p.ZZ);
  r.y = p.Y * inverse(p.ZZZ);
  return r;
}

template <class Mark>
static void fixed_bucketing(MsmScratch& sc, const MsmPlan& p, const BinSets& sets, size_t n, int mdig,
                            const MsmBaseTable* table, hipStream_t st, const Mark& mark) {
  const uint32_t tps = (uint32_t)((n + kTileScalars - 1) / kTileScalars);
  const uint32_t ntiles = tps * (uint32_t)p.msets;
  BinSets bs = sets;
  bs.tps = tps;
  bs.nb = p.nb;
  uint32_t* tail = sc.bin_counts.p + (size_t)256 * ntiles;
  auto run_bins = [&](auto cc, auto kb) {
    constexpr int C = decltype(cc)::value;
    constexpr int KB = decltype(kb)::value;
    using Lo = typename BinKeys<KB>::Lo;
    constexpr int LO = BinKeys<KB>::LO;
    Lo* lo2 = (Lo*)sc.keys_out.p;
    hipLaunchKernelGGL((msm_bin_hist_kernel<C, KB>), dim3(ntiles), dim3(kBinThreads), 0, st, bs, n, mdig,
                       sc.bin_counts.p, ntiles);
    NZ_HIP(hipGetLastError());
    lmark("mark: L hist");
    mark(1);
    hipLaunchKernelGGL(msm_bin_rowscan_kernel, dim3(256), dim3(256), 0, st, sc.bin_counts.p, ntiles, tail);
    lmark("mark: L rowscan");
    hipLaunchKernelGGL((msm_bin_scatter_kernel<C, KB>), dim3(ntiles), dim3(kBinThreads), 0, st, bs, n, mdig,
                       table->stride, sc.bin_counts.p, ntiles, lo2, sc.vals_mid.p);
    NZ_HIP(hipGetLastError());
    lmark("mark: L scatter");
    mark(2);
    const dim3 igrid((unsigned)lo_items_bound(p.entries));
    hipLaunchKernelGGL(msm_lo_count_kernel<LO>, igrid, dim3(kLoThreads), 0, st, (const Lo*)lo2, sc.bin_counts.p,
                       ntiles, sc.lo_seg.p);
    NZ_HIP(hipGetLastError());
    lmark("mark: L lo_count");
    hipLaunchKernelGGL(msm_lo_scan_kernel<LO>, dim3(256), dim3(kLoThreads), 0, st, sc.bin_counts.p, ntiles,
                       sc.lo_seg.p, p.nkeys, sc.offsets.p, sc.large.p);
    NZ_HIP(hipGetLastError());
    lmark("mark: L lo_scan");
    constexpr int sNT = LO > 8 ? 1024 : kLoThreads;
    constexpr uint32_t sU = LO > 8 ? 16 : kLoU;
    hipLaunchKernelGGL((msm_lo_scatter_kernel<LO, sNT, sU>), igrid, dim3(sNT), 0, st, (const Lo*)lo2, sc.vals_mid.p,
                       sc.bin_counts.p, ntiles, (const uint32_t*)sc.lo_seg.p, sc.sorted.p);
    NZ_HIP(hipGetLastError());
    lmark("mark: L lo_scatter");
  };
  using std::integral_constant;
  if (p.msets > 1) {
    if (p.c != 17) throw Error(NZCB_ERR_INTERNAL, "msm sets: the Lagrange window (17) only");
    run_bins(integral_constant<int, 17>(), integral_constant<int, 18>());
    return;
  }
  switch (p.c) {
    case 16: run_bins(integral_constant<int, 16>(), integral_constant<int, 15>()); break;
    case 17: run_bins(integral_constant<int, 17>(), integral_constant<int, 16>()); break;
    case 18: run_bins(integral_constant<int, 18>(), integral_constant<int, 17>()); break;
    case 19: run_bins(integral_constant<int, 19>(), integral_constant<int, 18>()); break;
    case 20: run_bins(integral_constant<int, 20>(), integral_constant<int, 19>()); break;
    default: throw Error(NZCB_ERR_INTERNAL, "bad fixed-base msm window");
  }
}

static void msm_enqueue_impl(MsmScratch& sc, const G1Affine* bases, const Fr* const* scalars, int msets, size_t n,
                             bool mont, hipStream_t st, const MsmBaseTable* table) {
  const auto t_enq = std::chrono::steady_clock::now();
  struct EnqueueClock {
    MsmScratch& sc;
    std::chrono::steady_clock::time_point t0;
    ~EnqueueClock() {
      if (sc.prof && sc.prof_phases)
        sc.enqueue_ms += std::chrono::duration<double, std::milli>(std::chrono::steady_clock::now() - t0).count();
    }
  } enqueue_clock{sc, t_enq};
  if (msets < 1 || msets > kMaxSets || (msets > 1 && (!table || msets > sc.max_lsets)))
    throw Error(NZCB_ERR_ARG, "msm sets: 1..3 over a table, within the scratch's sizing");
  sc.cur_n = n;
  sc.cur_msets = table ? msets : 1;
  if (n == 0) return;
  if (!sc.done) NZ_HIP(hipEventCreateWithFlags(&sc.done, hipEventDisableTiming));
  if (n > sc.max_points) throw Error(NZCB_ERR_ARG, "msm larger than scratch");
  if (table && n > table->n) throw Error(NZCB_ERR_ARG, "msm larger than its base table");
  if (table && table->mont_folded && !mont) throw Error(NZCB_ERR_ARG, "2^-256-folded table needs Montgomery scalars");
  if (table && (!sc.buckets29.p || !sc.bin_counts.p))
    throw Error(NZCB_ERR_ARG, "msm scratch was not sized for the fixed-base schedule");
  const int mdig = (mont && !(table && table->mont_folded)) ? 1 : 0;
  const MsmPlan p = make_plan(n, table, msets);
#ifdef NZCB_MSM_STATS
  if (table && !table->mont_folded) {
    NZ_HIP(hipStreamSynchronize(st));
    for (int k = 0; k < msets; k++) {
      std::vector<Fr> h(n);
      NZ_HIP(hipMemcpy(h.data(), scalars[k], n * sizeof(Fr), hipMemcpyDeviceToHost));
      size_t e_pos = 0, e_min = 0, nneg = 0, zero = 0, hist[17] = {0};
      for (size_t i = 0; i < n; i++) {
        Fr v = mdig ? from_mont(h[i]) : h[i];
        if (v.is_zero()) { zero++; continue; }
        const Fr w = neg(v);
        auto digits = [&](const Fr& x) {
          size_t d = 0;
          for_each_digit_host(x, p.c, [&](int, uint32_t, uint32_t) { d++; });
          return d;
        };
        const size_t dp = digits(v), dn = digits(w);
        e_pos += dp;
        e_min += dp <= dn ? dp : dn;
        if (dn < dp) nneg++;
        const size_t dm = dp <= dn ? dp : dn;
        hist[dm < 16 ? dm : 16]++;
      }
      fprintf(stderr, "MSMSCALARS set=%d n=%zu c=%d zero=%zu entries=%zu entries_minform=%zu flipped=%zu hist_minform=",
              k, n, p.c, zero, e_pos, e_min, nneg);
      for (int b = 0; b < 17; b++) fprintf(stderr, "%zu%c", hist[b], b == 16 ? '\n' : ',');
    }
  }
#endif
  if (p.entries > sc.sorted.n || p.nkeys + 1 > sc.offsets.n)
    throw Error(NZCB_ERR_ARG, "msm scratch was not sized for this schedule");
  if (table && ((size_t)p.nb / kTileSide * msets > sc.rowp29.n ||
                (((size_t)1 << p.hb) + ((size_t)1 << p.a)) * msets > sc.lines29.n ||
                (size_t)(p.lb + 1) * msets > sc.host_win_cap || (msets > 1 && p.c >= kStripMinC)))
    throw Error(NZCB_ERR_ARG, "msm scratch was not sized for this window");
  sc.cur_c = p.c;
  sc.cur_nsets = p.nsets;
  sc.cur_nbits = p.nbits;
  sc.cur_seglen = p.seglen;
  sc.cur_nkeys = p.nkeys;
  sc.cur_fixed = table != nullptr;
  sc.cur_a = p.a;
  sc.cur_hb = p.hb;
  sc.cur_msets = p.msets;
  const bool phases = sc.prof && sc.prof_phases;
  if (sc.prof && !sc.ev[0])
    for (auto& e : sc.ev) NZ_HIP(hipEventCreate(&e));
  auto mark = [&](int i) {
    if (phases) NZ_HIP(hipEventRecord(sc.ev[i], st));
  };
  mark(0);
  if (table) {
    BinSets bs{};
    for (int k = 0; k < msets; k++) bs.p[k] = scalars[k];
    fixed_bucketing(sc, p, bs, n, mdig | (table->mont_folded ? 0 : kDigMinForm), table, st, mark);
  } else {
    keys_dispatch(p.c, scalars[0], n, mdig, sc, st);
    mark(1);
    size_t tmp = sc.sort_tmp_bytes;
    int end_bit = 1;
    while ((1u << end_bit) <= p.nkeys) end_bit++;
    const auto t_sort = std::chrono::steady_clock::now();
    radix_sort(sc.sort_tmp.p, tmp, sc.keys_in.p, sc.keys_out.p, sc.vals_in.p, sc.sorted.p, p.entries, end_bit, st);
    if (phases)
      sc.sort_host_ms += std::chrono::duration<double, std::milli>(std::chrono::steady_clock::now() - t_sort).count();
    mark(2);
    hipLaunchKernelGGL(msm_offsets_kernel, dim3(grid_for((size_t)p.nkeys + 1, kMsmThreads, 1u << 30)),
                       dim3(kMsmThreads), 0, st, sc.keys_out.p, p.entries, p.nkeys, sc.offsets.p);
    NZ_HIP(hipGetLastError());
  }
  if (sc.prof) NZ_HIP(hipEventRecord(sc.ev[3], st));
  const bool sparse = table && table->sparse;
  sc.cur_sparse = sparse;
  const uint32_t chunk = sparse ? 0u : chunk_for(p.entries);
  const size_t nthreads = sparse ? dyn_threads_bound(p.entries) : (p.entries + chunk - 1) / chunk;
  const dim3 agrid(grid_for(nthreads, kMsmThreads, 1u << 30));
  const G1Affine* gather = table ? table->q.p : bases;
  if (table) {
    if (chunk == kChunk || sparse)
      hipLaunchKernelGGL(msm_accumulate29_kernel<true>, agrid, dim3(kMsmThreads), 0, st, chunk, gather, sc.sorted.p,
                         sc.offsets.p, p.nkeys, nthreads, sc.buckets29.p, sc.carry_own29.p, sc.carry_cont29.p);
    else
      hipLaunchKernelGGL(msm_accumulate29_kernel<false>, agrid, dim3(kMsmThreads), 0, st, chunk, gather, sc.sorted.p,
                         sc.offsets.p, p.nkeys, nthreads, sc.buckets29.p, sc.carry_own29.p, sc.carry_cont29.p);
  } else {
    hipLaunchKernelGGL(msm_accumulate_kernel, agrid, dim3(kMsmThreads), 0, st, chunk, gather, sc.sorted.p, sc.offsets.p,
                       p.nkeys, nthreads, sc.buckets.p, sc.carry_own.p, sc.carry_cont.p);
  }
  NZ_HIP(hipGetLastError());
  lmark("mark: L accumulate");
  if (sc.prof) NZ_HIP(hipEventRecord(sc.ev[4], st));
  const dim3 fgrid(grid_for(p.nkeys, kMsmThreads, 1u << 30));
  if (table) {
    hipLaunchKernelGGL(msm_finalize29_kernel, fgrid, dim3(kMsmThreads), 0, st, chunk, sc.offsets.p, p.nkeys,
                       sparse ? kSeqSpanSparse : kSeqSpan29, (const Xyzz29*)sc.carry_own29.p,
                       (const Xyzz29*)sc.carry_cont29.p, sc.large.p, sc.buckets29.p);
    NZ_HIP(hipGetLastError());
    lmark("mark: L finalize");
    hipLaunchKernelGGL(msm_large_scan_kernel, dim3(1), dim3(1024), 0, st, chunk, sc.offsets.p, p.nkeys, sc.large.p,
                       sc.large_off.p);
    NZ_HIP(hipGetLastError());
    lmark("mark: L large_scan");
    hipLaunchKernelGGL(msm_large_piece29_kernel, dim3(sparse ? kSparsePieceBlocks : kLargePieceBlocks),
                       dim3(kSumThreads), 0, st, chunk, sc.offsets.p, p.nkeys, sc.large.p, sc.large_off.p,
                       (const Xyzz29*)sc.carry_own29.p, (const Xyzz29*)sc.carry_cont29.p, sc.large_part.p);
    NZ_HIP(hipGetLastError());
    lmark("mark: L piece");
    if (sparse)
      hipLaunchKernelGGL(msm_large_final29_kernel<kSumThreads>, dim3(kSparseFinalBlocks), dim3(kSumThreads), 0, st,
                         sc.large.p, sc.large_off.p, sc.large_part.p, sc.buckets29.p);
    else
      hipLaunchKernelGGL(msm_large_final29_kernel<64>, dim3(kLargeFinalBlocks), dim3(64), 0, st, sc.large.p,
                         sc.large_off.p, sc.large_part.p, sc.buckets29.p);
    NZ_HIP(hipGetLastError());
    lmark("mark: L final");
    mark(5);
    int lparts = p.ltiles, hparts = p.htiles;
    if (p.c >= kStripMinC) {
      lparts = (1 << p.a) / kStrip;
      hparts = (1 << p.hb) / kStrip;
      const size_t nthr = ((size_t)lparts << p.hb) + ((size_t)hparts << p.a);
      hipLaunchKernelGGL(msm_strips29_kernel, dim3(grid_for(nthr, 256, 1u << 30)), dim3(256), 0, st,
                         (const Xyzz29*)sc.buckets29.p, sc.offsets.p, p.a, p.hb, sc.rowp29.p, sc.colp29.p);
    } else {
      hipLaunchKernelGGL(msm_tile29_kernel, dim3((unsigned)(p.ltiles * p.htiles), (unsigned)p.msets), dim3(256), 0, st,
                         (const Xyzz29*)sc.buckets29.p, sc.offsets.p, p.a, p.ltiles, p.htiles, sc.rowp29.p, sc.colp29.p);
    }
    NZ_HIP(hipGetLastError());
    mark(6);
    const int nrows = 1 << p.hb, ncols = 1 << p.a;
    hipLaunchKernelGGL(msm_lines29_kernel, dim3(grid_for((size_t)(nrows + ncols) * kLineThreads, 256), (unsigned)p.msets),
                       dim3(256), 0,
                       st, (const Xyzz29*)sc.rowp29.p, lparts, (const Xyzz29*)sc.colp29.p, hparts, nrows, ncols,
                       sc.lines29.p);
    NZ_HIP(hipGetLastError());
    lmark("mark: L lines");
    hipLaunchKernelGGL(msm_slots29_kernel, dim3(p.hb + p.a + 1, (unsigned)p.msets), dim3(kSumThreads), 0, st,
                       (const Xyzz29*)sc.lines29.p, p.hb, p.a, sc.host_win, (const uint32_t*)sc.offsets.p + p.nkeys,
                       sc.prof ? sc.host_total : nullptr);
    NZ_HIP(hipGetLastError());
    lmark("mark: L slots");
    mark(7);
    NZ_HIP(hipEventRecord(sc.done, st));
    return;
  }
  NZ_HIP(hipMemsetAsync(sc.large.p, 0, sizeof(uint32_t), st));
  hipLaunchKernelGGL(msm_bucket_finalize_kernel, fgrid, dim3(kMsmThreads), 0, st, chunk, sc.offsets.p, p.nkeys,
                     kSeqSpan, (const G1xyzz*)sc.carry_own.p, (const G1xyzz*)sc.carry_cont.p, sc.buckets.p, sc.large.p);
  NZ_HIP(hipGetLastError());
  hipLaunchKernelGGL(msm_bucket_large_kernel, dim3(kLargeBlocks), dim3(kSumThreads), 0, st, chunk, sc.offsets.p,
                     sc.large.p, (const G1xyzz*)sc.carry_own.p, (const G1xyzz*)sc.carry_cont.p, sc.buckets.p);
  NZ_HIP(hipGetLastError());
  mark(5);
  hipLaunchKernelGGL(msm_bucket_reduce_kernel, dim3(grid_for((size_t)p.nsets * p.nseg, kMsmThreads, 1u << 30)),
                     dim3(kMsmThreads), 0, st, sc.buckets.p, sc.offsets.p, (int)p.nb, p.seglen, p.nseg, p.nsets,
                     sc.seg_tot.p, sc.seg_run.p);
  NZ_HIP(hipGetLastError());
  mark(6);
  hipLaunchKernelGGL(msm_sums_kernel, dim3(p.nsets * p.nslots * p.nparts), dim3(kSumThreads), 0, st, sc.seg_tot.p,
                     sc.seg_run.p, p.nseg, p.nslots, p.nparts, sc.parts.p);
  NZ_HIP(hipGetLastError());
  hipLaunchKernelGGL(msm_parts_kernel, dim3(p.nsets * p.nslots), dim3(kPartThreads), 0, st, sc.parts.p, p.nparts,
                     sc.win.p);
  NZ_HIP(hipGetLastError());
  mark(7);
  if (sc.prof) NZ_HIP(hipMemcpyAsync(sc.host_total, sc.offsets.p + p.nkeys, 4, hipMemcpyDeviceToHost, st));
  NZ_HIP(hipMemcpyAsync(sc.host_win, sc.win.p, (size_t)p.nsets * p.nslots * sizeof(G1xyzz), hipMemcpyDeviceToHost,
                        st));
  NZ_HIP(hipEventRecord(sc.done, st));
}

void msm_enqueue(MsmScratch& sc, const G1Affine* bases, const Fr* scalars, size_t n, bool mont, hipStream_t st,
                 const MsmBaseTable* table) {
  const Fr* one[1] = {scalars};
  msm_enqueue_impl(sc, bases, one, 1, n, mont, st, table);
}

void msm_enqueue_sets(MsmScratch& sc, const Fr* const* scalars, int sets, size_t n, bool mont, hipStream_t st,
                      const MsmBaseTable* table) {
  if (!table) throw Error(NZCB_ERR_ARG, "msm sets: a table schedule");
  msm_enqueue_impl(sc, nullptr, scalars, sets, n, mont, st, table);
}

static G1xyzz fixed_window_result(const G1xyzz* s, int hb, int a) {
  G1xyzz acc = G1xyzz::inf();
  for (int b = hb - 1; b >= 0; b--) acc = xyzz_add(xyzz_dbl(acc), s[b]);
  for (int i = 0; i < a; i++) acc = xyzz_dbl(acc);
  G1xyzz col = G1xyzz::inf();
  for (int b = a - 1; b >= 0; b--) col = xyzz_add(xyzz_dbl(col), s[hb + b]);
  return xyzz_add(xyzz_add(acc, col), s[hb + a]);
}

void msm_finish_sets(MsmScratch& sc, hipStream_t st, G1xyzz* out) {
  const int msets = sc.cur_msets;
  if (sc.cur_n == 0) {
    for (int k = 0; k < msets; k++) out[k] = G1xyzz::inf();
    return;
  }
  out[0] = msm_finish(sc, st);
  for (int k = 1; k < msets; k++) out[k] = fixed_window_result(sc.host_win + (size_t)k * (sc.cur_hb + sc.cur_a + 1),
                                                               sc.cur_hb, sc.cur_a);
}

G1xyzz msm_finish(MsmScratch& sc, hipStream_t st) {
  if (sc.cur_n == 0) return G1xyzz::inf();
  NZ_HIP(hipEventSynchronize(sc.done));
#ifdef NZCB_MSM_STATS
  if (sc.cur_fixed) {
    std::vector<uint32_t> off(sc.cur_nkeys + 1);
    NZ_HIP(hipMemcpy(off.data(), sc.offsets.p, off.size() * 4, hipMemcpyDeviceToHost));
    uint32_t cnt = 0;
    NZ_HIP(hipMemcpy(&cnt, sc.large.p, 4, hipMemcpyDeviceToHost));
    uint32_t pieces = 0;
    NZ_HIP(hipMemcpy(&pieces, sc.large_off.p + cnt, 4, hipMemcpyDeviceToHost));
    const uint32_t M = off.back();
    const uint32_t chunk = sc.cur_sparse ? dyn_chunk(M) : chunk_for(sc.cur_n * (size_t)num_windows(sc.cur_c));
    size_t h[12] = {0};
    uint32_t mx = 0;
    uint64_t carries_large = 0, carries_mid = 0;
    for (uint32_t k = 0; k < sc.cur_nkeys; k++) {
      if (off[k + 1] == off[k]) { h[0]++; continue; }
      const uint32_t sp = (off[k + 1] - 1) / chunk - off[k] / chunk + 1;
      mx = sp > mx ? sp : mx;
      int b = 1;
      while (b < 11 && sp > (1u << (b - 1))) b++;
      h[b]++;
      if (sp > (sc.cur_sparse ? kSeqSpanSparse : kSeqSpan29) + 1) carries_large += sp; else if (sp > 1) carries_mid += sp;
    }
    fprintf(stderr, "MSMSTATS n=%zu c=%d entries=%u chunk=%u large=%u pieces=%u maxspan=%u carries_mid=%llu "
            "carries_large=%llu spans[empty,1,2,<=4,<=8,..,<=512,>512]=", sc.cur_n, sc.cur_c, M, chunk, cnt, pieces, mx,
            (unsigned long long)carries_mid, (unsigned long long)carries_large);
    for (int b = 0; b < 12; b++) fprintf(stderr, "%zu%c", h[b], b == 11 ? '\n' : ',');
  }
#endif
  const int c = sc.cur_c, nsets = sc.cur_nsets, nslots = sc.cur_nbits + 1;
  if (sc.prof) {
    float t = 0;
    NZ_HIP(hipEventElapsedTime(&t, sc.ev[3], sc.ev[4]));
    const uint32_t total = *sc.host_total;
    sc.prof_ms += t;
    sc.prof_launches++;
    sc.prof_points += sc.cur_n;
    sc.prof_entries += total;
    if (sc.prof_phases) {
      for (int i = 0; i < 7; i++) {
        float ms = 0;
        NZ_HIP(hipEventElapsedTime(&ms, sc.ev[i], sc.ev[i + 1]));
        sc.phase_ms[i] += ms;
      }
    }
  }
  const auto t_host = std::chrono::steady_clock::now();
  struct HostClock {
    MsmScratch& sc;
    std::chrono::steady_clock::time_point t0;
    ~HostClock() {
      if (sc.prof && sc.prof_phases)
        sc.host_ms += std::chrono::duration<double, std::milli>(std::chrono::steady_clock::now() - t0).count();
    }
  } host_clock{sc, t_host};
  if (sc.cur_fixed) return fixed_window_result(sc.host_win, sc.cur_hb, sc.cur_a);
  int lg_seg = 0;
  while ((1 << lg_seg) < sc.cur_seglen) lg_seg++;
  G1xyzz res = G1xyzz::inf();
  for (int w = nsets - 1; w >= 0; w--) {
    const G1xyzz* s = sc.host_win + (size_t)w * nslots;
    G1xyzz acc = G1xyzz::inf();
    for (int b = nslots - 2; b >= 0; b--) {
      acc = xyzz_dbl(acc);
      acc = xyzz_add(acc, s[1 + b]);
    }
    for (int i = 0; i < lg_seg; i++) acc = xyzz_dbl(acc);
    const G1xyzz W = xyzz_add(acc, s[0]);
    if (nsets > 1)
      for (int i = 0; i < c; i++) res = xyzz_dbl(res);
    res = xyzz_add(res, W);
  }
  return res;
}

}
```

nzcb-circom_amd/nzcb/__init__.py:

```python
from __future__ import annotations

import ctypes
import json
import os
from ctypes import POINTER, c_char, c_double, c_int, c_size_t, c_uint8, c_uint32, c_uint64, c_void_p

_HERE = os.path.dirname(os.path.abspath(__file__))
LIB_PATH = os.environ.get("NZCB_LIB", os.path.join(os.path.dirname(_HERE), "lib", "libnzcb.so"))

PROOF_BYTES = 9 * 64 + 7 * 32
BLINDING_BYTES = 11 * 32
VK_BYTES = 8 + 2 * 32 + 8 * 64 + 4 * 32 + 32
PROOF_POINTS = ("A", "B", "C", "Z", "T1", "T2", "T3", "Wxi", "Wxiw")
PROOF_EVALS = ("eval_a", "eval_b", "eval_c", "eval_s1", "eval_s2", "eval_zw", "eval_r")
VK_POINTS = ("Qm", "Ql", "Qr", "Qo", "Qc", "S1", "S2", "S3")

ERROR_NAMES = {
    0: "OK", 1: "ARG", 2: "FORMAT", 3: "NOT_PLONK", 4: "CURVE", 5: "WITNESS_LEN", 6: "COPY",
    7: "T_DIV", 8: "TZ", 9: "DIVPOL", 10: "HIP", 11: "INTERNAL",
}

EXPORTED_SYMBOLS = [
    "nzcb_version", "nzcb_device_count", "nzcb_ctx_create", "nzcb_ctx_destroy", "nzcb_ctx_set_logger",
    "nzcb_ctx_set_transcript_public", "nzcb_ctx_info", "nzcb_prove", "nzcb_prove_witness", "nzcb_prove_device",
    "nzcb_ctx_kernel_stats",
    "nzcb_ctx_last_timings", "nzcb_proof_to_json", "nzcb_public_to_json", "nzcb_synth_setup", "nzcb_free",
    "nzcb_engine_create", "nzcb_engine_destroy", "nzcb_engine_ntt", "nzcb_engine_msm", "nzcb_dev_alloc",
    "nzcb_dev_free", "nzcb_memcpy_h2d", "nzcb_memcpy_d2h", "nzcb_engine_ntt_dev", "nzcb_engine_msm_dev",
    "nzcb_engine_time_ntt", "nzcb_engine_fr_mul", "nzcb_engine_random_fr", "nzcb_engine_fixed_base",
    "nzcb_engine_time_msm", "nzcb_engine_msm_fixed_dev", "nzcb_engine_msm_table_dev", "nzcb_engine_msm_sets_dev", "nzcb_engine_time_msm2", "nzcb_ctx_set_lanes",
    "nzcb_ctx_lanes", "nzcb_prove_batch", "nzcb_vk_from_zkey", "nzcb_vk_from_zkey_file", "nzcb_vk_to_json", "nzcb_verify",
    "nzcb_proof_to_calldata", "nzcb_vk_to_solidity", "nzcb_engine_lagrange_basis", "nzcb_ctx_set_msm_devices", "nzcb_nzcp_input_signals", "nzcb_nzcp_witness",
    "nzcb_nzcp_witness_dev", "nzcb_synth_setup_ex", "nzcb_memcpy_d2d",
    "nzcb_plonk_setup", "nzcb_prove_batch_status", "nzcb_wprog_remap", "nzcb_prove_logged", "nzcb_memcpy_d2d_async",
    "nzcb_debug_guard_check", "nzcb_debug_guard_selftest", "nzcb_debug_inject_fault", "nzcb_debug_f29",
    "nzcb_debug_ntt_coset",
    "nzcb_msm_table_create_lagrange",
    "nzcb_verify_batch", "nzcb_engine_g1_lincomb", "nzcb_engine_verify_batch", "nzcb_debug_verify_batch_timings",
    "nzcb_r1cs_create", "nzcb_r1cs_create_file", "nzcb_r1cs_info", "nzcb_r1cs_check", "nzcb_r1cs_destroy",
    "nzcb_engine_r1cs_create", "nzcb_debug_r1cs_check_timings",
    "nzcb_p256_key_create", "nzcb_p256_verify", "nzcb_p256_key_destroy", "nzcb_engine_p256_key_create",
    "nzcb_debug_p256_field", "nzcb_debug_p256_mul2", "nzcb_debug_p256_timings",
    "nzcb_nzcp_pass_layout", "nzcb_nzcp_decode", "nzcb_nzcp_decode_dev", "nzcb_debug_nzcp_decode_timings",
]

NZCB_FAULT_QUOTIENT = 1
NZCB_DEBUG_GENERIC_K = 2
NZCB_FAULT_LANE_ALLOC = 3
VERIFY_HOST = -1
R1CS_HOST = -1
WITNESS_WTNS, WITNESS_HOST, WITNESS_DEVICE = 0, 1, 2
P256_HOST = -1
SIG_OK, SIG_INVALID, SIG_RANGE = 0, 1, 2
NZCP_HOST = -1
PASS_MAX_URI = 2048
PASS_STATUS_NAMES = ("OK", "LENGTH", "PREFIX", "BASE32", "TRUNCATED", "CBOR", "NOT_COSE", "HEADER",
                     "CLAIMS")
PASS_HAS_ALG, PASS_HAS_KID, PASS_HAS_ISS, PASS_HAS_NBF, PASS_HAS_EXP, PASS_HAS_CTI, PASS_HAS_SIG = (
    1, 2, 4, 8, 16, 32, 64)
P256_OPS = {"add": 0, "sub": 1, "mul": 2, "sqr": 3, "inv": 4}


def lagrange_commit_enabled() -> bool:
    import re
    e = os.environ.get("NZCB_LAGRANGE_COMMIT")
    if e is None:
        return True
    m = re.match(r"\s*[+-]?\d+", e)
    return bool(m) and int(m.group()) != 0


def guard_check(device: int = -1) -> int:
    err, checked, bad = _Err(), c_size_t(0), c_int(0)
    _check(load().nzcb_debug_guard_check(device, ctypes.byref(checked), ctypes.byref(bad), ctypes.byref(err)), err)
    return checked.value


F29_WORDS = {1: (27, 9), 2: (54, 18), 3: (18, 9), 4: (36, 18), 5: (18, 18), 6: (36, 9), 7: (10, 9)}


def f29_check(op: int, words, device: int = 0):
    win, wout = F29_WORDS[op]
    count = len(words) // win
    assert count * win == len(words)
    arr = (c_uint32 * max(1, len(words)))(*words)
    out = (c_uint32 * max(1, count * wout))()
    err = _Err()
    _check(load().nzcb_debug_f29(device, op, arr, count, out, ctypes.byref(err)), err)
    return list(out)[:count * wout]


def guard_selftest(device: int = 0) -> None:
    err = _Err()
    _check(load().nzcb_debug_guard_selftest(device, ctypes.byref(err)), err)


class NzcbError(RuntimeError):
    def __init__(self, code: int, msg: str):
        super().__init__(msg)
        self.code = code
        self.name = ERROR_NAMES.get(code, str(code))


class _Err(ctypes.Structure):
    _fields_ = [("code", c_int), ("msg", c_char * 256)]


class NzcpParams(ctypes.Structure):
    _fields_ = [("is_live", ctypes.c_int32), ("max_tbs_bytes", ctypes.c_int32),
                ("max_array_len_vc", ctypes.c_int32), ("max_map_len_vc", ctypes.c_int32)]


class NzcpRecord(ctypes.Structure):
    _fields_ = [("status", ctypes.c_int32), ("detail", ctypes.c_int32), ("exp", ctypes.c_uint32),
                ("vc_pos", ctypes.c_int32), ("given_len", ctypes.c_int32), ("family_len", ctypes.c_int32),
                ("dob_len", ctypes.c_int32), ("nullifier_len", ctypes.c_int32),
                ("tbs_sha256", c_uint8 * 32), ("nullifier_sha512", c_uint8 * 64), ("nullifier", c_uint8 * 64),
                ("pub", (c_uint8 * 32) * 3)]


class NzcpPass(ctypes.Structure):
    _fields_ = [("status", ctypes.c_int32), ("detail", c_uint32), ("version", c_uint32), ("present", c_uint32),
                ("alg", ctypes.c_int32), ("kid_len", c_uint32), ("iss_len", c_uint32), ("cti_len", c_uint32),
                ("sig_len", c_uint32), ("cose_len", c_uint32), ("protected_off", c_uint32),
                ("protected_len", c_uint32), ("payload_off", c_uint32), ("payload_len", c_uint32),
                ("tbs_len", c_uint32), ("fits", c_uint32), ("nbf", c_uint64), ("exp", c_uint64),
                ("kid", c_uint8 * 32), ("cti", c_uint8 * 32), ("iss", c_uint8 * 64), ("sig", c_uint8 * 64),
                ("tbs_sha256", c_uint8 * 32)]


NZCP_LIVE = dict(is_live=1, max_tbs_bytes=351, max_array_len_vc=0, max_map_len_vc=4)
NZCP_EXAMPLE = dict(is_live=0, max_tbs_bytes=314, max_array_len_vc=0, max_map_len_vc=4)

LOG_FN = ctypes.CFUNCTYPE(None, c_void_p, ctypes.c_char_p)
MSM_SEND_FN = ctypes.CFUNCTYPE(c_int, c_void_p, c_int, c_void_p, c_size_t)
MSM_GATHER_FN = ctypes.CFUNCTYPE(c_int, c_void_p, c_int, POINTER(c_uint8), POINTER(c_uint8))
MSM_LAGRANGE = 0x100

_lib = None


def load(path: str | None = None):
    global _lib
    if _lib is not None and path is None:
        return _lib
    if os.environ.get("GPU_MAX_HW_QUEUES", "4") == "4":
        os.environ["GPU_MAX_HW_QUEUES"] = "24"
    lib = ctypes.CDLL(path or LIB_PATH)
    u8p = POINTER(c_uint8)
    sigs = {
        "nzcb_version": (ctypes.c_char_p, []),
        "nzcb_device_count": (c_int, []),
        "nzcb_ctx_create": (c_void_p, [u8p, c_size_t, c_int, POINTER(_Err)]),
        "nzcb_ctx_destroy": (None, [c_void_p]),
        "nzcb_ctx_set_logger": (None, [c_void_p, LOG_FN, c_void_p]),
        "nzcb_ctx_set_transcript_public": (None, [c_void_p, c_int]),
        "nzcb_ctx_info": (c_int, [c_void_p, POINTER(c_uint32)]),
        "nzcb_prove": (c_int, [c_void_p, u8p, c_size_t, u8p, u8p, u8p, c_size_t, POINTER(_Err)]),
        "nzcb_prove_witness": (c_int, [c_void_p, u8p, c_size_t, u8p, u8p, u8p, c_size_t, POINTER(_Err)]),
        "nzcb_prove_device": (c_int, [c_void_p, c_void_p, c_size_t, u8p, u8p, u8p, c_size_t, POINTER(_Err)]),
        "nzcb_prove_logged": (c_int, [c_void_p, c_void_p, c_size_t, c_int, u8p, u8p, u8p, c_size_t, LOG_FN, c_void_p,
                                      POINTER(_Err)]),
        "nzcb_ctx_kernel_stats": (c_int, [c_void_p, c_int, POINTER(c_double)]),
        "nzcb_ctx_set_lanes": (c_int, [c_void_p, c_int, POINTER(_Err)]),
        "nzcb_ctx_set_msm_devices": (c_int, [c_void_p, POINTER(c_int), c_int, POINTER(_Err)]),
        "nzcb_vk_from_zkey": (c_int, [u8p, c_size_t, u8p, POINTER(_Err)]),
        "nzcb_vk_from_zkey_file": (c_int, [ctypes.c_char_p, u8p, POINTER(_Err)]),
        "nzcb_vk_to_json": (c_int, [u8p, ctypes.c_char_p, c_size_t]),
        "nzcb_verify": (c_int, [u8p, u8p, u8p, c_int, c_int, POINTER(c_int), POINTER(_Err)]),
        "nzcb_proof_to_calldata": (c_int, [u8p, u8p, c_int, ctypes.c_char_p, c_size_t]),
        "nzcb_vk_to_solidity": (c_int, [u8p, ctypes.c_char_p, c_int, ctypes.c_char_p, c_size_t]),
        "nzcb_engine_lagrange_basis": (c_int, [c_void_p, c_void_p, c_size_t, c_int, c_void_p, POINTER(_Err)]),
        "nzcb_ctx_lanes": (c_int, [c_void_p]),
        "nzcb_prove_batch": (c_int, [c_void_p, POINTER(c_void_p), c_size_t, c_int, c_int, u8p, u8p, u8p, c_size_t,
                                     POINTER(_Err)]),
        "nzcb_prove_batch_status": (c_int, [c_void_p, POINTER(c_void_p), c_size_t, c_int, c_int, u8p, u8p, u8p,
                                            c_size_t, POINTER(c_int), POINTER(_Err)]),
        "nzcb_ctx_last_timings": (c_int, [c_void_p, POINTER(c_double), c_int]),
        "nzcb_proof_to_json": (c_int, [u8p, ctypes.c_char_p, c_size_t]),
        "nzcb_public_to_json": (c_int, [u8p, c_int, ctypes.c_char_p, c_size_t]),
        "nzcb_synth_setup": (c_int, [c_int, c_int, c_int, c_uint64, c_uint32, u8p, c_int,
                                     POINTER(POINTER(c_uint8)), POINTER(c_size_t),
                                     POINTER(POINTER(c_uint8)), POINTER(c_size_t), POINTER(_Err)]),
        "nzcb_synth_setup_ex": (c_int, [c_int, c_int, c_int, c_uint64, c_uint32, c_uint32, u8p, c_int,
                                        POINTER(POINTER(c_uint8)), POINTER(c_size_t),
                                        POINTER(POINTER(c_uint8)), POINTER(c_size_t), POINTER(_Err)]),
        "nzcb_free": (None, [c_void_p]),
        "nzcb_engine_create": (c_void_p, [c_int, c_int, c_size_t, POINTER(_Err)]),
        "nzcb_engine_destroy": (None, [c_void_p]),
        "nzcb_engine_ntt": (c_int, [c_void_p, u8p, u8p, c_int, c_int, POINTER(_Err)]),
        "nzcb_debug_ntt_coset": (c_int, [c_void_p, u8p, u8p, c_int, u8p, c_int, POINTER(_Err)]),
        "nzcb_engine_msm": (c_int, [c_void_p, u8p, u8p, c_size_t, c_int, u8p, POINTER(_Err)]),
        "nzcb_dev_alloc": (c_void_p, [c_size_t]),
        "nzcb_dev_alloc_on": (c_void_p, [c_int, c_size_t]),
        "nzcb_dev_free": (None, [c_void_p]),
        "nzcb_memcpy_h2d": (c_int, [c_void_p, c_void_p, c_size_t]),
        "nzcb_memcpy_d2h": (c_int, [c_void_p, c_void_p, c_size_t]),
        "nzcb_memcpy_d2d": (c_int, [c_void_p, c_void_p, c_size_t]),
        "nzcb_memcpy_d2d_async": (c_int, [c_void_p, c_void_p, c_size_t, c_void_p]),
        "nzcb_engine_ntt_dev": (c_int, [c_void_p, c_void_p, c_void_p, c_int, c_int, POINTER(_Err)]),
        "nzcb_engine_msm_dev": (c_int, [c_void_p, c_void_p, c_void_p, c_size_t, c_int, u8p, POINTER(_Err)]),
        "nzcb_engine_time_ntt": (c_int, [c_void_p, c_void_p, c_void_p, c_int, c_int, c_int, POINTER(c_double),
                                         POINTER(_Err)]),
        "nzcb_engine_fr_mul": (c_int, [c_void_p, u8p, u8p, u8p, c_size_t, c_int, POINTER(_Err)]),
        "nzcb_engine_random_fr": (c_int, [c_void_p, c_void_p, c_size_t, c_uint64, POINTER(_Err)]),
        "nzcb_engine_fixed_base": (c_int, [c_void_p, c_void_p, c_size_t, c_void_p, POINTER(_Err)]),
        "nzcb_engine_time_msm": (c_int, [c_void_p, c_void_p, c_void_p, c_size_t, c_int, c_int, POINTER(c_double),
                                         POINTER(c_double), POINTER(_Err)]),
        "nzcb_engine_msm_fixed_dev": (c_int, [c_void_p, c_void_p, c_size_t, c_void_p, c_size_t, c_int, u8p,
                                              POINTER(_Err)]),
        "nzcb_engine_msm_table_dev": (c_int, [c_void_p, c_void_p, c_size_t, c_void_p, c_size_t, c_int, c_int, c_int,
                                              c_int, u8p, POINTER(_Err)]),
        "nzcb_engine_msm_sets_dev": (c_int, [c_void_p, c_void_p, c_size_t, POINTER(c_void_p), c_int, c_size_t, c_int,
                                             c_int, u8p, POINTER(_Err)]),
        "nzcb_plonk_setup": (c_int, [ctypes.c_char_p, c_size_t, ctypes.c_char_p, c_size_t, c_int, POINTER(POINTER(c_uint8)),
                                     POINTER(c_size_t), POINTER(_Err)]),
        "nzcb_nzcp_input_signals": (c_size_t, [POINTER(NzcpParams)]),
        "nzcb_nzcp_witness": (c_int, [c_int, POINTER(NzcpParams), u8p, c_int, POINTER(NzcpRecord), POINTER(_Err)]),
        "nzcb_nzcp_witness_dev": (c_int, [c_int, POINTER(NzcpParams), c_void_p, c_int, c_void_p, c_void_p, c_size_t,
                                          c_void_p, POINTER(_Err)]),
        "nzcb_engine_time_msm2": (c_int, [c_void_p, c_void_p, c_void_p, c_size_t, c_int, c_int, c_int,
                                          POINTER(c_double), POINTER(_Err)]),
        "nzcb_ctx_create_devices": (c_void_p, [u8p, c_size_t, POINTER(c_int), c_int, POINTER(_Err)]),
        "nzcb_ctx_devices": (c_int, [c_void_p]),
        "nzcb_ctx_set_msm_split": (c_int, [c_void_p, c_int, c_size_t, c_size_t, MSM_SEND_FN, MSM_GATHER_FN,
                                           c_void_p, POINTER(_Err)]),
        "nzcb_msm_table_create": (c_void_p, [c_int, c_void_p, c_size_t, POINTER(_Err)]),
        "nzcb_msm_table_create_lagrange": (c_void_p, [c_int, c_void_p, c_size_t, c_int, c_size_t, c_size_t,
                                                      POINTER(_Err)]),
        "nzcb_msm_table_run": (c_int, [c_void_p, c_void_p, c_size_t, c_int, u8p, POINTER(_Err)]),
        "nzcb_msm_table_destroy": (None, [c_void_p]),
        "nzcb_ptau_synth": (c_int, [c_int, u8p, c_int, POINTER(POINTER(c_uint8)), POINTER(c_size_t), POINTER(_Err)]),
        "nzcb_wprog_create": (c_void_p, [ctypes.c_char_p, c_size_t, c_int, POINTER(_Err)]),
        "nzcb_wprog_destroy": (None, [c_void_p]),
        "nzcb_wprog_info": (c_int, [c_void_p, POINTER(c_uint32)]),
        "nzcb_wprog_run_dev": (c_int, [c_void_p, c_void_p, c_int, c_void_p, c_size_t, POINTER(ctypes.c_int32),
                                       c_void_p, POINTER(_Err)]),
        "nzcb_wprog_run": (c_int, [c_void_p, ctypes.c_char_p, c_int, u8p, POINTER(ctypes.c_int32), POINTER(_Err)]),
        "nzcb_wprog_remap": (c_int, [ctypes.c_char_p, c_size_t, ctypes.c_char_p, c_size_t, ctypes.c_char_p, c_size_t,
                                     POINTER(POINTER(c_uint8)), POINTER(c_size_t), POINTER(c_uint32), POINTER(_Err)]),
        "nzcb_debug_guard_check": (c_int, [c_int, POINTER(c_size_t), POINTER(c_int), POINTER(_Err)]),
        "nzcb_debug_guard_selftest": (c_int, [c_int, POINTER(_Err)]),
        "nzcb_debug_inject_fault": (c_int, [c_void_p, c_int]),
        "nzcb_debug_f29": (c_int, [c_int, c_int, POINTER(c_uint32), c_size_t, POINTER(c_uint32), POINTER(_Err)]),
        "nzcb_verify_batch": (c_int, [u8p, u8p, u8p, c_size_t, c_int, c_int, c_int, c_int, u8p, POINTER(c_int),
                                      POINTER(_Err)]),
        "nzcb_engine_g1_lincomb": (c_int, [c_int, u8p, u8p, POINTER(c_uint32), c_size_t, u8p, POINTER(_Err)]),
        "nzcb_engine_verify_batch": (c_int, [u8p, u8p, u8p, c_size_t, c_int, c_int, c_int, c_int, u8p, POINTER(c_int),
                                             u8p, POINTER(c_int), POINTER(_Err)]),
        "nzcb_debug_verify_batch_timings": (c_int, [POINTER(c_double), c_int]),
        "nzcb_r1cs_create": (c_void_p, [ctypes.c_char_p, c_size_t, c_int, POINTER(_Err)]),
        "nzcb_r1cs_create_file": (c_void_p, [ctypes.c_char_p, c_int, POINTER(_Err)]),
        "nzcb_engine_r1cs_create": (c_void_p, [ctypes.c_char_p, c_size_t, c_int, c_uint32, c_int, POINTER(_Err)]),
        "nzcb_r1cs_info": (c_int, [c_void_p, POINTER(c_uint32)]),
        "nzcb_r1cs_check": (c_int, [c_void_p, c_void_p, c_size_t, c_int, c_int, c_size_t, POINTER(c_uint32),
                                    POINTER(c_uint32), c_uint32, c_void_p, POINTER(_Err)]),
        "nzcb_r1cs_destroy": (None, [c_void_p]),
        "nzcb_debug_r1cs_check_timings": (c_int, [POINTER(c_double), c_int]),
        "nzcb_p256_key_create": (c_void_p, [ctypes.c_char_p, c_int, POINTER(_Err)]),
        "nzcb_engine_p256_key_create": (c_void_p, [ctypes.c_char_p, c_int, c_int, POINTER(_Err)]),
        "nzcb_p256_verify": (c_int, [c_void_p, c_void_p, c_size_t, c_void_p, c_size_t, c_int, c_int,
                                     POINTER(ctypes.c_int32), c_void_p, POINTER(_Err)]),
        "nzcb_p256_key_destroy": (None, [c_void_p]),
        "nzcb_debug_p256_field": (c_int, [c_int, c_int, c_int, ctypes.c_char_p, ctypes.c_char_p, c_size_t, u8p,
                                          POINTER(_Err)]),
        "nzcb_debug_p256_mul2": (c_int, [c_void_p, ctypes.c_char_p, ctypes.c_char_p, c_size_t, u8p, POINTER(_Err)]),
        "nzcb_debug_p256_timings": (c_int, [POINTER(c_double), c_int]),
        "nzcb_nzcp_pass_layout": (None, [POINTER(c_uint32)]),
        "nzcb_nzcp_decode": (c_int, [c_int, ctypes.c_char_p, POINTER(c_uint32), c_int, POINTER(NzcpParams),
                                     ctypes.c_char_p, POINTER(NzcpPass), u8p, u8p, c_size_t, POINTER(_Err)]),
        "nzcb_nzcp_decode_dev": (c_int, [c_int, c_void_p, c_void_p, c_int, POINTER(NzcpParams), c_void_p, c_void_p,
                                         c_void_p, c_void_p, c_size_t, c_void_p, POINTER(_Err)]),
        "nzcb_debug_nzcp_decode_timings": (c_int, [POINTER(c_double), c_int]),
    }
    lib.missing_symbols = []
    for name, (res, args) in sigs.items():
        try:
            fn = getattr(lib, name)
        except AttributeError:
            lib.missing_symbols.append(name)
            continue
        fn.restype = res
        fn.argtypes = args
    if "nzcb_nzcp_pass_layout" not in lib.missing_symbols:
        lay = (c_uint32 * 3)()
        lib.nzcb_nzcp_pass_layout(lay)
        if list(lay) != [ctypes.sizeof(NzcpPass), NzcpPass.sig.offset, NzcpPass.tbs_sha256.offset]:
            raise OSError(f"NzcpPass does not mirror nzcb_nzcp_pass: the library reports {list(lay)}")
    _lib = lib
    return lib


def _buf(data: bytes):
    return (c_uint8 * len(data)).from_buffer_copy(data) if data else (c_uint8 * 1)()


def _out(n: int):
    return (c_uint8 * max(n, 1))()


def _check(rc: int, err: _Err):
    if rc != 0:
        raise NzcbError(rc, err.msg.decode(errors="replace"))


def version() -> str:
    return load().nzcb_version().decode()


def device_count() -> int:
    return load().nzcb_device_count()


def nzcp_input_signals(params: dict) -> int:
    return load().nzcb_nzcp_input_signals(ctypes.byref(NzcpParams(**params)))


def _record_dict(r: NzcpRecord) -> dict:
    return {
        "status": r.status, "detail": r.detail, "exp": r.exp, "vc_pos": r.vc_pos, "given_len": r.given_len,
        "family_len": r.family_len, "dob_len": r.dob_len, "nullifier_len": r.nullifier_len,
        "tbs_sha256": bytes(r.tbs_sha256), "nullifier_sha512": bytes(r.nullifier_sha512),
        "nullifier": bytes(r.nullifier), "out": [int.from_bytes(bytes(r.pub[k]), "little") for k in range(3)],
    }


def nzcp_witness(inputs: bytes, count: int, params: dict = NZCP_LIVE, device: int = 0) -> list:
    lib = load()
    prm = NzcpParams(**params)
    need = lib.nzcb_nzcp_input_signals(ctypes.byref(prm)) * 32 * count
    if len(inputs) != need:
        raise ValueError(f"nzcp inputs are {len(inputs)} bytes, expected {need}")
    recs = (NzcpRecord * max(count, 1))()
    err = _Err()
    _check(lib.nzcb_nzcp_witness(device, ctypes.byref(prm), _buf(inputs), count, recs, ctypes.byref(err)), err)
    return [_record_dict(recs[i]) for i in range(count)]


def nzcp_witness_dev(dev_inputs: int, count: int, params: dict = NZCP_LIVE, device: int = 0,
                     dev_records: int | None = None, dev_witness: int | None = None, witness_stride: int = 0,
                     stream: int | None = None):
    lib = load()
    err = _Err()
    _check(lib.nzcb_nzcp_witness_dev(device, ctypes.byref(NzcpParams(**params)), dev_inputs, count, dev_records,
                                     dev_witness, witness_stride, stream, ctypes.byref(err)), err)


def nzcp_records_from_bytes(raw: bytes, count: int) -> list:
    size = ctypes.sizeof(NzcpRecord)
    return [_record_dict(NzcpRecord.from_buffer_copy(raw[i * size:(i + 1) * size])) for i in range(count)]


def _pass_dict(r: NzcpPass) -> dict:
    has = lambda bit: bool(r.present & bit)
    return {
        "status": r.status, "status_name": PASS_STATUS_NAMES[r.status], "detail": r.detail, "version": r.version,
        "present": r.present, "alg": r.alg if has(PASS_HAS_ALG) else None,
        "kid": bytes(r.kid)[:min(r.kid_len, 32)] if has(PASS_HAS_KID) else None, "kid_len": r.kid_len,
        "iss": bytes(r.iss)[:min(r.iss_len, 64)].decode(errors="replace") if has(PASS_HAS_ISS) else None,
        "iss_len": r.iss_len, "nbf": r.nbf if has(PASS_HAS_NBF) else None,
        "exp": r.exp if has(PASS_HAS_EXP) else None,
        "cti": bytes(r.cti)[:min(r.cti_len, 32)] if has(PASS_HAS_CTI) else None, "cti_len": r.cti_len,
        "sig": bytes(r.sig) if has(PASS_HAS_SIG) else None, "sig_len": r.sig_len, "cose_len": r.cose_len,
        "protected_off": r.protected_off, "protected_len": r.protected_len, "payload_off": r.payload_off,
        "payload_len": r.payload_len, "tbs_len": r.tbs_len, "fits": r.fits, "tbs_sha256": bytes(r.tbs_sha256),
    }


def nzcp_passes_from_bytes(raw: bytes, count: int) -> list:
    size = ctypes.sizeof(NzcpPass)
    return [_pass_dict(NzcpPass.from_buffer_copy(raw[i * size:(i + 1) * size])) for i in range(count)]


def pack_uris(uris):
    raw = [u.encode("utf-8", "surrogateescape") if isinstance(u, str) else bytes(u) for u in uris]
    offs, at = [0], 0
    for b in raw:
        at += len(b)
        offs.append(at)
    if at > 1 << 31:
        raise ValueError("more than 2^31 bytes of URIs")
    return b"".join(raw), (c_uint32 * len(offs))(*offs)


def nzcp_decode_raw(uris, params: dict | None = None, data20=None, device: int = 0, want_tbs: int = 0,
                    offsets=None):
    lib = load()
    if offsets is None:
        blob, offs = pack_uris(uris)
    else:
        blob, offs = bytes(uris), (c_uint32 * len(offsets))(*offsets)
    count = len(offs) - 1
    if data20 is not None:
        data20 = b"".join(data20) if isinstance(data20, (list, tuple)) else bytes(data20)
        if len(data20) != 20 * count:
            raise ValueError("data is 20 bytes per pass")
    prm = NzcpParams(**params) if params else None
    recs = (NzcpPass * max(count, 1))()
    inputs = _out(lib.nzcb_nzcp_input_signals(ctypes.byref(prm)) * 32 * count) if prm else None
    tbs = _out(want_tbs * count) if want_tbs else None
    err = _Err()
    _check(lib.nzcb_nzcp_decode(device, blob, offs, count, ctypes.byref(prm) if prm else None, data20, recs, inputs,
                                tbs, want_tbs, ctypes.byref(err)), err)
    size = ctypes.sizeof(NzcpPass)
    return (bytes(recs)[:size * count],
            bytes(inputs)[:lib.nzcb_nzcp_input_signals(ctypes.byref(prm)) * 32 * count] if prm else None,
            bytes(tbs)[:want_tbs * count] if want_tbs else None)


def nzcp_decode(uris, params: dict | None = None, data20=None, device: int = 0):
    uris = list(uris)
    recs, inputs, _ = nzcp_decode_raw(uris, params, data20, device)
    out = nzcp_passes_from_bytes(recs, len(uris))
    return (out, inputs) if params else out


def nzcp_decode_dev(dev_uris: int, dev_offsets: int, count: int, dev_passes: int, params: dict | None = None,
                    dev_data20: int | None = None, dev_inputs: int | None = None, dev_tbs: int | None = None,
                    tbs_stride: int = 0, device: int = 0, stream: int | None = None):
    lib = load()
    err = _Err()
    prm = NzcpParams(**params) if params else None
    _check(lib.nzcb_nzcp_decode_dev(device, dev_uris, dev_offsets, count, ctypes.byref(prm) if prm else None,
                                    dev_data20, dev_passes, dev_inputs, dev_tbs, tbs_stride, stream,
                                    ctypes.byref(err)), err)


def nzcp_decode_timings() -> list:
    ms = (c_double * 2)()
    n = load().nzcb_debug_nzcp_decode_timings(ms, 2)
    return list(ms)[:n]


class Engine:

    def __init__(self, device: int = 0, max_log_ntt: int = 12, max_msm_points: int = 1 << 12):
        self.lib = load()
        err = _Err()
        self.h = self.lib.nzcb_engine_create(device, max_log_ntt, max_msm_points, ctypes.byref(err))
        if not self.h:
            raise NzcbError(err.code, err.msg.decode(errors="replace"))

    def close(self):
        if self.h:
            self.lib.nzcb_engine_destroy(self.h)
            self.h = None

    __del__ = close

    def ntt(self, data_lem: bytes, log_n: int, inverse: bool = False) -> bytes:
        n = 1 << log_n
        assert len(data_lem) == 32 * n
        out = _out(32 * n)
        err = _Err()
        _check(self.lib.nzcb_engine_ntt(self.h, _buf(data_lem), out, log_n, int(inverse), ctypes.byref(err)), err)
        return bytes(out)

    def ntt_coset(self, data_lem: bytes, log_n: int, c_lem: bytes) -> bytes:
        n = 1 << log_n
        fold = len(data_lem) // 32 - n
        assert len(data_lem) == 32 * (n + fold) and fold >= 0 and len(c_lem) == 32
        out = _out(32 * n)
        err = _Err()
        _check(self.lib.nzcb_debug_ntt_coset(self.h, _buf(data_lem), out, log_n, _buf(c_lem), fold,
                                             ctypes.byref(err)), err)
        return bytes(out)

    def msm(self, bases_lem: bytes, scalars: bytes, scalars_mont: bool = False) -> bytes:
        n = len(scalars) // 32
        assert len(bases_lem) == 64 * n
        out = _out(64)
        err = _Err()
        _check(self.lib.nzcb_engine_msm(self.h, _buf(bases_lem), _buf(scalars), n, int(scalars_mont), out,
                                        ctypes.byref(err)), err)
        return bytes(out)

    def field_mul(self, a_lem: bytes, b_lem: bytes, field_q: bool = False) -> bytes:
        n = len(a_lem) // 32
        out = _out(32 * n)
        err = _Err()
        _check(self.lib.nzcb_engine_fr_mul(self.h, _buf(a_lem), _buf(b_lem), out, n, int(field_q),
                                           ctypes.byref(err)), err)
        return bytes(out)

    def time_ntt(self, dev_in: int, dev_out: int, log_n: int, inverse: bool, reps: int) -> float:
        ms = c_double()
        err = _Err()
        _check(self.lib.nzcb_engine_time_ntt(self.h, dev_in, dev_out, log_n, int(inverse), reps, ctypes.byref(ms),
                                             ctypes.byref(err)), err)
        return ms.value

    def random_fr(self, dev_out: int, n: int, seed: int):
        err = _Err()
        _check(self.lib.nzcb_engine_random_fr(self.h, dev_out, n, seed, ctypes.byref(err)), err)

    def fixed_base(self, dev_scalars: int, n: int, dev_out: int):
        err = _Err()
        _check(self.lib.nzcb_engine_fixed_base(self.h, dev_scalars, n, dev_out, ctypes.byref(err)), err)

    def lagrange_basis(self, dev_ptau: int, ptau_n: int, log_n: int, dev_out: int):
        err = _Err()
        _check(self.lib.nzcb_engine_lagrange_basis(self.h, dev_ptau, ptau_n, log_n, dev_out, ctypes.byref(err)), err)

    def time_msm(self, dev_bases: int, dev_scalars: int, n: int, scalars_mont: bool, reps: int):
        ms = c_double()
        acc = c_double()
        err = _Err()
        _check(self.lib.nzcb_engine_time_msm(self.h, dev_bases, dev_scalars, n, int(scalars_mont), reps,
                                             ctypes.byref(ms), ctypes.byref(acc), ctypes.byref(err)), err)
        return ms.value, acc.value

    MSM_PHASES = ("keys", "sort", "offsets", "accumulate", "finalize", "reduce", "sums")

    def time_msm_phases(self, dev_bases: int, dev_scalars: int, n: int, scalars_mont: bool, fixed_base: bool,
                        reps: int) -> dict:
        out = (c_double * 13)()
        err = _Err()
        _check(self.lib.nzcb_engine_time_msm2(self.h, dev_bases, dev_scalars, n, int(scalars_mont), int(fixed_base),
                                              reps, out, ctypes.byref(err)), err)
        d = {"wall": out[0], "table_build": out[8], "entries": out[9]}
        d.update({k: out[1 + i] for i, k in enumerate(self.MSM_PHASES)})
        d["host_finish"] = out[10]
        d["host_enqueue"] = out[11]
        d["host_sort_call"] = out[12]
        return d

    def msm_fixed_dev(self, dev_bases: int, n_table: int, dev_scalars: int, n: int, scalars_mont: bool,
                      window: int = 0, sparse: bool = False, fold: bool = False) -> bytes:
        out = _out(64)
        err = _Err()
        if window or sparse or fold:
            _check(self.lib.nzcb_engine_msm_table_dev(self.h, dev_bases, n_table, dev_scalars, n, int(scalars_mont),
                                                      int(window), int(sparse), int(fold), out, ctypes.byref(err)),
                   err)
        else:
            _check(self.lib.nzcb_engine_msm_fixed_dev(self.h, dev_bases, n_table, dev_scalars, n, int(scalars_mont),
                                                      out, ctypes.byref(err)), err)
        return bytes(out)

    def msm_sets_dev(self, dev_bases: int, n_table: int, dev_scalars: list, n: int, scalars_mont: bool, *,
                     sparse: bool) -> list:
        k = len(dev_scalars)
        out = _out(64 * k)
        err = _Err()
        arr = (c_void_p * k)(*dev_scalars)
        _check(self.lib.nzcb_engine_msm_sets_dev(self.h, dev_bases, n_table, arr, k, n, int(scalars_mont),
                                                 int(bool(sparse)), out, ctypes.byref(err)), err)
        return [bytes(out)[64 * i:64 * i + 64] for i in range(k)]

    def msm_dev(self, dev_bases: int, dev_scalars: int, n: int, scalars_mont: bool) -> bytes:
        out = _out(64)
        err = _Err()
        _check(self.lib.nzcb_engine_msm_dev(self.h, dev_bases, dev_scalars, n, int(scalars_mont), out,
                                            ctypes.byref(err)), err)
        return bytes(out)

    @staticmethod
    def g1_lincomb(points: bytes, scalars: bytes, group_end, device: int = 0) -> list:
        groups = len(group_end)
        n = group_end[-1] if groups else 0
        assert len(points) == 64 * n and len(scalars) == 32 * n
        ends = (c_uint32 * max(groups, 1))(*group_end)
        out = _out(64 * groups)
        err = _Err()
        _check(load().nzcb_engine_g1_lincomb(device, _buf(points), _buf(scalars), ends, groups, out,
                                             ctypes.byref(err)), err)
        return [bytes(out)[64 * g:64 * g + 64] for g in range(groups)]

    @staticmethod
    def verify_batch(vk: bytes, proofs, publics, transcript_public: bool = True, device: int = 0,
                     seed: bytes | None = None, n_public: int | None = None):
        count = len(proofs)
        assert len(publics) == count and all(len(p) == PROOF_BYTES for p in proofs)
        if n_public is None:
            n_public = len(publics[0]) // 32 if count else 0
        stride = max([32 * n_public] + [len(p) for p in publics])
        pubs = b"".join(bytes(p).ljust(stride, b"\0") for p in publics)
        assert seed is None or len(seed) == 32
        valid = (c_int * max(count, 1))()
        pts = _out(128 * count)
        checks = c_int(0)
        err = _Err()
        _check(load().nzcb_engine_verify_batch(_buf(vk), _buf(b"".join(proofs)), _buf(pubs), stride, n_public, count,
                                               int(transcript_public), device, _buf(seed) if seed else None, valid,
                                               pts, ctypes.byref(checks), ctypes.byref(err)), err)
        raw = bytes(pts)
        return ([bool(valid[i]) for i in range(count)], [raw[128 * i:128 * i + 128] for i in range(count)],
                checks.value)

    @staticmethod
    def verify_batch_timings() -> list:
        ms = (c_double * 6)()
        k = load().nzcb_debug_verify_batch_timings(ms, 6)
        return list(ms)[:k]


def dev_alloc(nbytes: int) -> int:
    p = load().nzcb_dev_alloc(nbytes)
    if not p:
        raise NzcbError(10, "hipMalloc failed")
    return p


def dev_free(p: int):
    load().nzcb_dev_free(p)


def h2d(dst: int, data: bytes):
    buf = ctypes.create_string_buffer(data, len(data))
    rc = load().nzcb_memcpy_h2d(dst, buf, len(data))
    if rc:
        raise NzcbError(rc, "h2d failed")


def memcpy_h2d_ptr(dst: int, src_addr: int, nbytes: int):
    rc = load().nzcb_memcpy_h2d(dst, src_addr, nbytes)
    if rc:
        raise NzcbError(rc, "h2d failed")


def d2d(dst: int, src: int, nbytes: int):
    if load().nzcb_memcpy_d2d(dst, src, nbytes) != 0:
        raise NzcbError(10, "hipMemcpy D2D failed")


def d2d_async(dst: int, src: int, nbytes: int, stream: int):
    if load().nzcb_memcpy_d2d_async(dst, src, nbytes, stream) != 0:
        raise NzcbError(10, "hipMemcpyAsync D2D failed")


def d2h(src: int, nbytes: int) -> bytes:
    buf = ctypes.create_string_buffer(nbytes)
    rc = load().nzcb_memcpy_d2h(buf, src, nbytes)
    if rc:
        raise NzcbError(rc, "d2h failed")
    return buf.raw


def _read(x) -> bytes:
    if isinstance(x, (bytes, bytearray, memoryview)):
        return bytes(x)
    if isinstance(x, dict) and x.get("type") == "mem":
        return bytes(x["data"])
    with open(x, "rb") as f:
        return f.read()


class ProverContext:

    def __init__(self, zkey, device: int = 0, logger=None, transcript_public: bool = True, _raw=None,
                 devices=None):
        self.lib = load()
        self.devices = list(devices) if devices else [device]
        self.device = self.devices[0]
        err = _Err()
        vk = _out(VK_BYTES)
        if _raw is not None:
            zptr, zlen = ctypes.cast(_raw[0], POINTER(c_uint8)), _raw[1]
        else:
            data = _read(zkey)
            zptr, zlen = _buf(data), len(data)
        if len(self.devices) > 1:
            devs = (c_int * len(self.devices))(*self.devices)
            self.h = self.lib.nzcb_ctx_create_devices(zptr, zlen, devs, len(self.devices), ctypes.byref(err))
        else:
            self.h = self.lib.nzcb_ctx_create(zptr, zlen, self.device, ctypes.byref(err))
        if not self.h:
            raise NzcbError(err.code, err.msg.decode(errors="replace"))
        verr = _Err()
        _check(self.lib.nzcb_vk_from_zkey(zptr, zlen, vk, ctypes.byref(verr)), verr)
        self.vk = bytes(vk)
        info = (c_uint32 * 5)()
        self.lib.nzcb_ctx_info(self.h, info)
        self.domain_size, self.n_public, self.n_vars, self.n_additions, self.n_constraints = list(info)
        self._logcb = None
        if logger is not None:
            self.set_logger(logger)
        if not transcript_public:
            self.lib.nzcb_ctx_set_transcript_public(self.h, 0)

    def set_logger(self, logger):
        fn = getattr(logger, "debug", logger)
        self._logcb = LOG_FN(lambda _u, m: fn(m.decode()))
        self.lib.nzcb_ctx_set_logger(self.h, self._logcb, None)

    def close(self):
        if getattr(self, "h", None):
            self.lib.nzcb_ctx_destroy(self.h)
            self.h = None

    __del__ = close

    def prove_raw(self, wtns, blinding: bytes | None = None):
        data = _read(wtns)
        proof = _out(PROOF_BYTES)
        pub = _out(32 * self.n_public)
        err = _Err()
        bl = _buf(blinding) if blinding is not None else None
        if blinding is not None and len(blinding) != BLINDING_BYTES:
            raise ValueError("blinding must be 11 x 32 bytes")
        _check(self.lib.nzcb_prove(self.h, _buf(data), len(data), bl, proof, pub, 32 * self.n_public,
                                   ctypes.byref(err)), err)
        return bytes(proof), bytes(pub)[:32 * self.n_public]

    def prove_witness_raw(self, witness_le: bytes, blinding: bytes | None = None):
        n = len(witness_le) // 32
        proof = _out(PROOF_BYTES)
        pub = _out(32 * self.n_public)
        err = _Err()
        bl = _buf(blinding) if blinding is not None else None
        _check(self.lib.nzcb_prove_witness(self.h, _buf(witness_le), n, bl, proof, pub, 32 * self.n_public,
                                           ctypes.byref(err)), err)
        return bytes(proof), bytes(pub)[:32 * self.n_public]

    def prove_device_raw(self, dev_witness: int, n_witness: int, blinding: bytes | None = None):
        proof = _out(PROOF_BYTES)
        pub = _out(32 * self.n_public)
        err = _Err()
        bl = _buf(blinding) if blinding is not None else None
        _check(self.lib.nzcb_prove_device(self.h, dev_witness, n_witness, bl, proof, pub, 32 * self.n_public,
                                          ctypes.byref(err)), err)
        return bytes(proof), bytes(pub)[:32 * self.n_public]

    def set_lanes(self, lanes: int):
        err = _Err()
        _check(self.lib.nzcb_ctx_set_lanes(self.h, lanes, ctypes.byref(err)), err)

    def set_msm_devices(self, devices):
        arr = (c_int * len(devices))(*devices)
        err = _Err()
        _check(self.lib.nzcb_ctx_set_msm_devices(self.h, arr, len(devices), ctypes.byref(err)), err)

    def set_msm_split(self, world: int, own_points: int, send, gather, own_lagrange: int = 0):
        if world <= 1:
            self._split_cbs = None
            _check(self.lib.nzcb_ctx_set_msm_split(self.h, 1, 0, 0, MSM_SEND_FN(), MSM_GATHER_FN(), None,
                                                   ctypes.byref(_Err())), _Err())
            return

        def _send(_u, slot, ptr, count):
            try:
                send(slot, ptr, count)
                return 0
            except Exception:
                import traceback
                traceback.print_exc()
                return 1

        def _gather(_u, slot, own, out):
            try:
                parts = gather(slot, ctypes.string_at(own, 64))
                if len(parts) != 64 * world:
                    return 1
                ctypes.memmove(out, parts, len(parts))
                return 0
            except Exception:
                import traceback
                traceback.print_exc()
                return 1

        self._split_cbs = (MSM_SEND_FN(_send), MSM_GATHER_FN(_gather))
        err = _Err()
        _check(self.lib.nzcb_ctx_set_msm_split(self.h, world, own_points, own_lagrange, self._split_cbs[0],
                                               self._split_cbs[1], None, ctypes.byref(err)), err)

    @property
    def lanes(self) -> int:
        return self.lib.nzcb_ctx_lanes(self.h)

    def prove_batch_raw(self, witnesses, n_witness: int | None = None, blindings=None, on_device: bool = False,
                        statuses: list | None = None):
        count = len(witnesses)
        keep = []
        ptrs = (c_void_p * max(count, 1))()
        for i, w in enumerate(witnesses):
            if on_device:
                ptrs[i] = w
            else:
                b = _buf(w)
                keep.append(b)
                ptrs[i] = ctypes.cast(b, c_void_p).value
                if n_witness is None:
                    n_witness = len(w) // 32
        bl = None
        if blindings is not None:
            bl = _buf(b"".join(x if x is not None else random_blinding() for x in blindings))
        proofs = _out(PROOF_BYTES * count)
        stride = 32 * max(self.n_public, 1)
        pubs = _out(stride * count)
        err = _Err()
        if statuses is None:
            _check(self.lib.nzcb_prove_batch(self.h, ptrs, n_witness or 0, count, int(on_device), bl, proofs, pubs,
                                             stride, ctypes.byref(err)), err)
        else:
            st = (c_int * max(count, 1))()
            rc = self.lib.nzcb_prove_batch_status(self.h, ptrs, n_witness or 0, count, int(on_device), bl, proofs,
                                                  pubs, stride, st, ctypes.byref(err))
            if rc and not any(st[i] for i in range(count)):
                _check(rc, err)
            statuses[:] = [st[i] for i in range(count)]
        P, Q = bytes(proofs), bytes(pubs)
        return [(P[i * PROOF_BYTES:(i + 1) * PROOF_BYTES], Q[i * stride:i * stride + 32 * self.n_public])
                for i in range(count)]

    def inject_fault(self, kind: int = NZCB_FAULT_QUOTIENT) -> None:
        if self.lib.nzcb_debug_inject_fault(self.h, kind) != 0:
            raise ValueError(f"bad fault kind {kind}")

    def kernel_stats(self, enable: int = -1):
        out = (c_double * 4)()
        self.lib.nzcb_ctx_kernel_stats(self.h, enable, out)
        return tuple(out)

    def prove(self, wtns, blinding: bytes | None = None):
        proof, pub = self.prove_raw(wtns, blinding)
        return {"proof": proof_to_json(proof), "publicSignals": public_to_json(pub, self.n_public)}

    def last_timings(self):
        ms = (c_double * 11)()
        k = self.lib.nzcb_ctx_last_timings(self.h, ms, 11)
        names = ["total", "witness", "round1", "round2", "round3", "round4", "round5", "msm_host_wait",
                 "ntt_host_enqueue", "msm_gpu", "ntt_gpu"]
        out = dict(zip(names[:k], list(ms)[:k]))
        return {key: v for key, v in out.items() if v >= 0}


class MsmTable:

    def __init__(self, dev_bases: int, n: int, device: int = 0, _handle=None):
        self.lib = load()
        err = _Err()
        self.n = n
        self.h = _handle or self.lib.nzcb_msm_table_create(device, dev_bases, n, ctypes.byref(err))
        if not self.h:
            raise NzcbError(err.code, err.msg.decode(errors="replace"))

    @classmethod
    def lagrange(cls, dev_ptau: int, ptau_n: int, log_n: int, lo: int, hi: int, device: int = 0):
        lib = load()
        err = _Err()
        h = lib.nzcb_msm_table_create_lagrange(device, dev_ptau, ptau_n, log_n, lo, hi, ctypes.byref(err))
        if not h:
# ... 656 lines not shown
```

Before: 48.43 proofs/s.

## Accumulate MSM buckets with length-sorted capped segments instead of fixed chunks

Adds a segment plan for the fixed-base MSM accumulation. A histogram kernel and a scatter kernel split each bucket into segments of at most kSegMax entries, ordered by length. A new per-segment accumulate kernel processes them, and finalize and large-carry kernels read a carry-run description. The intent is to balance work across threads and cut warp divergence compared with the fixed-chunk split. It costs two extra planning kernels and more scratch buffers. The path is on by default through NZCB_ACC_SEGMENTS, and a debug API exposes the plan.

```diff
diff --git a/include/nzcb_internal.h b/include/nzcb_internal.h
--- a/include/nzcb_internal.h
+++ b/include/nzcb_internal.h
@@ -50,6 +50,9 @@
 int nzcb_engine_msm_table_dev(nzcb_engine* e, const void* bases, size_t n_table, const void* scalars, size_t n,
                               int scalars_mont, int window, int sparse, int fold, uint8_t* out_affine,
                               nzcb_err* err);
+int nzcb_debug_msm_plan(nzcb_engine* e, const void* bases, size_t n_table, const void* scalars, size_t n,
+                        int scalars_mont, int window, int fold, uint32_t* info, uint32_t* offsets, size_t offsets_cap,
+                        uint32_t* seg, size_t seg_cap, uint8_t* out_affine, nzcb_err* err);
 int nzcb_engine_msm_sets_dev(nzcb_engine* e, const void* bases, size_t n_table, const void* const* scalars, int sets,
                              size_t n, int scalars_mont, int sparse, uint8_t* out_affine, nzcb_err* err);
 int nzcb_engine_time_msm2(nzcb_engine* e, const void* bases, const void* scalars, size_t n, int scalars_mont,
diff --git a/nzcb-circom_amd/csrc/capi_engine.hip b/nzcb-circom_amd/csrc/capi_engine.hip
--- a/nzcb-circom_amd/csrc/capi_engine.hip
+++ b/nzcb-circom_amd/csrc/capi_engine.hip
@@ -334,6 +334,38 @@
     sc.init(n ? n : 1, true);
     G1xyzz r = msm(sc, (const G1Affine*)bases, (const Fr*)scalars, n, scalars_mont != 0, g.stream, &t);
     affine_out(r, out_affine);
+  });
+}
+
+int nzcb_debug_msm_plan(nzcb_engine* e, const void* bases, size_t n_table, const void* scalars, size_t n,
+                        int scalars_mont, int window, int fold, uint32_t* info, uint32_t* offsets, size_t offsets_cap,
+                        uint32_t* seg, size_t seg_cap, uint8_t* out_affine, nzcb_err* err) {
+  return guarded(err, [&] {
+    Engine& g = e->eng;
+    NZ_HIP(hipSetDevice(g.device));
+    if (n > n_table) throw Error(NZCB_ERR_ARG, "msm larger than its base table");
+    if (window && (window < 16 || window > 20)) throw Error(NZCB_ERR_ARG, "msm table window: 16..20");
+    MsmBaseTable t;
+    t.build((const G1Affine*)bases, n_table, window ? window : fixed_base_window(), g.stream, fold != 0);
+    MsmScratch sc;
+    sc.init(n ? n : 1, true);
+    G1xyzz r = msm(sc, (const G1Affine*)bases, (const Fr*)scalars, n, scalars_mont != 0, g.stream, &t);
+    affine_out(r, out_affine);
+    std::vector<uint32_t> off, start, len, bucket;
+    info[0] = msm_debug_plan(sc, g.stream, off, start, len, bucket) ? 1u : 0u;
+    info[1] = info[2] = 0;
+    info[3] = kSegMax;
+    if (!info[0]) return;
+    info[1] = (uint32_t)(off.size() - 1);
+    info[2] = (uint32_t)start.size();
+    if (off.size() > offsets_cap || 3 * start.size() > seg_cap)
+      throw Error(NZCB_ERR_ARG, "msm plan: the output arrays are too small");
+    std::memcpy(offsets, off.data(), off.size() * 4);
+    if (!start.empty()) {
+      std::memcpy(seg, start.data(), start.size() * 4);
+      std::memcpy(seg + start.size(), len.data(), start.size() * 4);
+      std::memcpy(seg + 2 * start.size(), bucket.data(), start.size() * 4);
+    }
   });
 }
 
diff --git a/nzcb-circom_amd/csrc/msm.h b/nzcb-circom_amd/csrc/msm.h
--- a/nzcb-circom_amd/csrc/msm.h
+++ b/nzcb-circom_amd/csrc/msm.h
@@ -4,6 +4,7 @@
 #include "common.h"
 #include "ec.h"
 #include "f29.h"
+#include "msm_seg.h"
 
 namespace nzcb {
 
@@ -19,6 +20,7 @@
 int fixed_base_window();
 int lagrange_window();
 bool lagrange_sparse();
+bool acc_segments();
 
 struct MsmScratch {
   size_t max_points = 0;
@@ -37,6 +39,7 @@
   DevBuf<uint32_t> large;
   DevBuf<uint32_t> large_off;
   DevBuf<Xyzz29> large_part;
+  DevBuf<uint32_t> seg_start, seg_len, seg_bucket, seg_dst, seg_cnt, seg_meta, seg_mk, seg_mfs, seg_mnp;
   DevBuf<Xyzz29> rowp29, colp29, lines29;
   DevBuf<G1xyzz> seg_tot;
   DevBuf<G1xyzz> seg_run;
@@ -47,6 +50,7 @@
   size_t host_win_cap = 0;
   int cur_c = 0, cur_nsets = 0, cur_nbits = 0, cur_seglen = 0;
   bool cur_fixed = false, cur_sparse = false;
+  bool cur_seg = false;
   int cur_a = 0, cur_hb = 0;
   int cur_msets = 1;
   size_t cur_n = 0;
@@ -79,6 +83,9 @@
   return msm_finish(sc, st);
 }
 
+bool msm_debug_plan(MsmScratch& sc, hipStream_t st, std::vector<uint32_t>& offsets, std::vector<uint32_t>& start,
+                    std::vector<uint32_t>& len, std::vector<uint32_t>& bucket);
+
 G1Affine xyzz_to_affine(const G1xyzz& p);
 
 }
diff --git a/nzcb-circom_amd/csrc/msm.hip b/nzcb-circom_amd/csrc/msm.hip
--- a/nzcb-circom_amd/csrc/msm.hip
+++ b/nzcb-circom_amd/csrc/msm.hip
@@ -78,6 +78,14 @@
   static const bool v = [] {
     const char* e = std::getenv("NZCB_SPARSE");
     return e && std::atoi(e) != 0;
+  }();
+  return v;
+}
+
+bool acc_segments() {
+  static const bool v = [] {
+    const char* e = std::getenv("NZCB_ACC_SEGMENTS");
+    return e ? std::atoi(e) != 0 : true;
   }();
   return v;
 }
@@ -596,6 +604,44 @@
   return r;
 }
 
+__device__ __forceinline__ void acc_entry29(Xyzz29& acc, bool& inf, const G1Affine& P, uint32_t ent) {
+  if (P.is_inf()) return;
+  const F29 x = split29(P.x);
+  F29 y = split29(P.y);
+  if (ent >> 31) y = neg29_nn(y);
+  if (inf) {
+    norm29(y);
+    acc.X = x;
+    acc.Y = y;
+    acc.ZZ = f29_const(Fq29::ONE);
+    acc.ZZZ = f29_const(Fq29::ONE);
+    inf = false;
+  } else {
+    F29 U2, S2, PP, RR;
+    mul29x2<Fq29>(x, acc.ZZ, y, acc.ZZZ, U2, S2);
+    const F29 Pd = sub29(U2, acc.X, Fq29::K8);
+    const F29 R = sub29(S2, acc.Y, Fq29::K4);
+    sqr29x2(Pd, R, PP, RR);
+    if (is0p29_fast(PP)) {
+      if (is0p29(RR)) {
+        norm29(y);
+        mdbl29_rare(x, y, &acc);
+      } else {
+        inf = true;
+      }
+    } else {
+      F29 PPP, Q, ZZ3, ZZZ3;
+      mul29x2<Fq29>(Pd, PP, acc.X, PP, PPP, Q);
+      const F29 X3 = sub2x29(RR, PPP, Q);
+      mul29x2<Fq29>(acc.ZZ, PP, acc.ZZZ, PPP, ZZ3, ZZZ3);
+      acc.Y = mul2sum29(R, sub29_nn(Q, X3, Fq29W::K10), neg4p29_nn(acc.Y), PPP);
+      acc.ZZ = ZZ3;
+      acc.ZZZ = ZZZ3;
+      acc.X = X3;
+    }
+  }
+}
+
 static constexpr uint32_t kLdsStride = kMsmThreads + 1;
 template <bool kLdsIdx>
 __global__ void __launch_bounds__(kMsmThreads) __attribute__((amdgpu_waves_per_eu(3, 8)))
@@ -639,42 +685,7 @@
     uint32_t ent_nn = 0;
     if (pos + 1 < e) Pn = bases[ent_n & 0x7fffffffu];
     if (pos + 2 < e) ent_nn = index_at(pos + 2);
-    if (!P.is_inf()) {
-      const F29 x = split29(P.x);
-      F29 y = split29(P.y);
-      if (ent >> 31) y = neg29_nn(y);
-      if (inf) {
-        norm29(y);
-        acc.X = x;
-        acc.Y = y;
-        acc.ZZ = f29_const(Fq29::ONE);
-        acc.ZZZ = f29_const(Fq29::ONE);
-        inf = false;
-      } else {
-        F29 U2, S2, PP, RR;
-        mul29x2<Fq29>(x, acc.ZZ, y, acc.ZZZ, U2, S2);
-        const F29 Pd = sub29(U2, acc.X, Fq29::K8);
-        const F29 R = sub29(S2, acc.Y, Fq29::K4);
-        sqr29x2(Pd, R, PP, RR);
-        if (is0p29_fast(PP)) {
-          if (is0p29(RR)) {
-            norm29(y);
-            mdbl29_rare(x, y, &acc);
-          } else {
-            inf = true;
-          }
-        } else {
-          F29 PPP, Q, ZZ3, ZZZ3;
-          mul29x2<Fq29>(Pd, PP, acc.X, PP, PPP, Q);
-          const F29 X3 = sub2x29(RR, PPP, Q);
-          mul29x2<Fq29>(acc.ZZ, PP, acc.ZZZ, PPP, ZZ3, ZZZ3);
-          acc.Y = mul2sum29(R, sub29_nn(Q, X3, Fq29W::K10), neg4p29_nn(acc.Y), PPP);
-          acc.ZZ = ZZ3;
-          acc.ZZZ = ZZZ3;
-          acc.X = X3;
-        }
-      }
-    }
+    acc_entry29(acc, inf, P, ent);
     pos++;
     if (pos == kend || pos == e) {
       const bool starts = kstart >= s;
@@ -695,6 +706,144 @@
     }
     ent = ent_n;
     ent_n = ent_nn;
+    P = Pn;
+  }
+}
+
+struct SegPlan {
+  uint32_t *start, *len, *bucket, *dst;
+  uint32_t *mk, *mfs, *mnp;
+  uint32_t* meta;
+};
+
+static constexpr int kSegThreads = 256;
+static constexpr uint32_t kSegWaves = kSegThreads / 64;
+
+__global__ void __launch_bounds__(kSegThreads)
+msm_seg_hist_kernel(const uint32_t* __restrict__ offsets, uint32_t nkeys, uint32_t ntiles,
+                    uint32_t* __restrict__ cnt, uint32_t* __restrict__ meta) {
+  __shared__ uint32_t h[kSegWaves][kSegMax + 1];
+  const uint32_t wave = threadIdx.x >> 6, lane = threadIdx.x & 63;
+  const uint32_t tile = blockIdx.x * kSegWaves + wave;
+  for (uint32_t i = threadIdx.x; i < kSegWaves * (kSegMax + 1); i += kSegThreads) (&h[0][0])[i] = 0;
+  if (blockIdx.x == 0 && threadIdx.x == 0) meta[1] = 0;
+  __syncthreads();
+  if (tile < ntiles) {
+    for (uint32_t it = 0; it < kSegTile / 64; it++) {
+      const uint32_t k = tile * kSegTile + it * 64 + lane;
+      if (k >= nkeys) break;
+      const uint32_t len = offsets[k + 1] - offsets[k];
+      const uint32_t whole = len / kSegMax, rest = len % kSegMax;
+      if (whole) atomicAdd(&h[wave][kSegMax], whole);
+      if (rest) atomicAdd(&h[wave][rest], 1u);
+    }
+  }
+  __syncthreads();
+  if (tile < ntiles)
+    for (uint32_t L = 1 + lane; L <= kSegMax; L += 64) cnt[(size_t)(kSegMax - L) * ntiles + tile] = h[wave][L];
+}
+
+__global__ void __launch_bounds__(kSegThreads)
+msm_seg_scatter_kernel(const uint32_t* __restrict__ offsets, uint32_t nkeys, uint32_t ntiles,
+                       const uint32_t* __restrict__ cnt, SegPlan pl) {
+  __shared__ uint32_t cb[256], wsum[4];
+  __shared__ uint32_t base_s[kSegWaves][kSegMax + 1];
+  const uint32_t wave = threadIdx.x >> 6, lane = threadIdx.x & 63;
+  const uint32_t tile = blockIdx.x * kSegWaves + wave;
+  uint32_t total;
+  const uint32_t* tail = cnt + (size_t)kSegMax * ntiles;
+  cb[threadIdx.x] = scan256_excl(threadIdx.x < kSegMax ? tail[threadIdx.x] : 0u, wsum, total);
+  if (blockIdx.x == 0 && threadIdx.x == 0) pl.meta[0] = total;
+  __syncthreads();
+  volatile uint32_t* base = base_s[wave];
+  if (tile < ntiles)
+    for (uint32_t L = 1 + lane; L <= kSegMax; L += 64)
+      base[L] = cb[kSegMax - L] + cnt[(size_t)(kSegMax - L) * ntiles + tile];
+  __syncthreads();
+  if (tile >= ntiles) return;
+  for (uint32_t it = 0; it < kSegTile / 64; it++) {
+    const uint32_t k0 = tile * kSegTile + it * 64;
+    if (k0 >= nkeys) break;
+    const uint32_t k = k0 + lane;
+    const uint32_t s = k < nkeys ? offsets[k] : 0u;
+    const uint32_t len = k < nkeys ? offsets[k + 1] - s : 0u;
+    const uint32_t whole = len / kSegMax, rest = len % kSegMax;
+    const bool cut = whole + (rest ? 1u : 0u) > 1;
+    const uint32_t incl = wave_incl_scan(whole);
+    const uint32_t wtot = __shfl(incl, 63, 64);
+    const uint32_t fs = base[kSegMax] + incl - whole;
+    if (lane == 0 && wtot) base[kSegMax] = fs + wtot;
+    const uint32_t dst = cut ? 0x80000000u | fs : k;
+    for (uint32_t j = 0; j < whole; j++) {
+      pl.start[fs + j] = s + j * kSegMax;
+      pl.len[fs + j] = kSegMax;
+      pl.bucket[fs + j] = k;
+      pl.dst[fs + j] = dst;
+    }
+    uint64_t same = __ballot(rest != 0);
+#pragma unroll
+    for (uint32_t b = 0; (1u << b) < kSegMax; b++) {
+      const uint64_t bb = __ballot((rest >> b) & 1u);
+      same &= ((rest >> b) & 1u) ? bb : ~bb;
+    }
+    if (rest) {
+      const uint32_t rank = __popcll(same & ((1ull << lane) - 1ull));
+      const uint32_t at = base[rest] + rank;
+      if (rank == 0) base[rest] = at + __popcll(same);
+      pl.start[at] = s + whole * kSegMax;
+      pl.len[at] = rest;
+      pl.bucket[at] = k;
+      pl.dst[at] = dst;
+    }
+    if (cut) {
+      const uint32_t m = atomicAdd(&pl.meta[1], 1u);
+      pl.mk[m] = k;
+      pl.mfs[m] = fs;
+      pl.mnp[m] = whole | (rest ? 0x80000000u : 0u);
+    }
+  }
+}
+
+typedef uint32_t u32x4 __attribute__((ext_vector_type(4)));
+typedef u32x4 u32x4_a4 __attribute__((aligned(4)));
+
+__global__ void __launch_bounds__(kMsmThreads) __attribute__((amdgpu_waves_per_eu(3, 8)))
+msm_accumulate29_seg_kernel(const G1Affine* __restrict__ bases, const uint32_t* __restrict__ sorted,
+                            const uint32_t* __restrict__ seg_start, const uint32_t* __restrict__ seg_len,
+                            const uint32_t* __restrict__ seg_dst, const uint32_t* __restrict__ meta,
+                            Xyzz29* __restrict__ buckets, Xyzz29* __restrict__ carry_own,
+                            Xyzz29* __restrict__ carry_cont) {
+  const uint32_t i = blockIdx.x * kMsmThreads + threadIdx.x;
+  const uint32_t nseg = meta[0];
+  if (i >= nseg) return;
+  const uint32_t s = seg_start[i], len = seg_len[i];
+  u32x4 g = *(const u32x4_a4*)(sorted + s);
+  uint32_t ent = g.x, nxt = g.y;
+  g.x = g.z;
+  g.y = g.w;
+  G1Affine P = bases[ent & 0x7fffffffu];
+  Xyzz29 acc;
+  bool inf = true;
+  const uint32_t dst = seg_dst[i];
+  Xyzz29* o = !(dst >> 31) ? buckets + dst : len == kSegMax ? carry_cont + i : carry_own + (dst & 0x7fffffffu);
+  for (uint32_t j = 0; j < len;) {
+    G1Affine Pn;
+    if (j + 1 < len) Pn = bases[nxt & 0x7fffffffu];
+    acc_entry29(acc, inf, P, ent);
+    j++;
+    if (j == len) {
+      Xyzz29 out = acc;
+      if (inf)
+#pragma unroll
+        for (int u = 0; u < 9; u++) out.ZZ.v[u] = 0;
+      *o = out;
+    }
+    ent = nxt;
+    nxt = g.x;
+    g.x = g.y;
+    g.y = g.z;
+    g.z = g.w;
+    if ((j & 3u) == 2u && j + 2 < len) g = *(const u32x4_a4*)(sorted + s + j + 2);
     P = Pn;
   }
 }
@@ -724,45 +873,70 @@
   buckets[k] = sum_run(carry_own, carry_cont, c0, c1);
 }
 
+struct CarryRun {
+  uint32_t k, c0, span, own;
+};
+template <bool kSeg>
+__device__ __forceinline__ CarryRun carry_run(uint32_t chunk, const uint32_t* __restrict__ offsets,
+                                              const SegPlan& pl, uint32_t id) {
+  CarryRun r;
+  if (kSeg) {
+    const uint32_t np = pl.mnp[id];
+    r.k = pl.mk[id];
+    r.c0 = pl.mfs[id];
+    r.own = np & 0x7fffffffu;
+    r.span = r.own + (np >> 31);
+  } else {
+    r.k = id;
+    r.c0 = offsets[id] / chunk;
+    r.span = (offsets[id + 1] - 1) / chunk - r.c0 + 1;
+    r.own = 0;
+  }
+  return r;
+}
+__device__ __forceinline__ const Xyzz29& carry_at(const Xyzz29* __restrict__ carry_own,
+                                                  const Xyzz29* __restrict__ carry_cont, const CarryRun& r,
+                                                  uint32_t u) {
+  return u == r.own ? carry_own[r.c0] : carry_cont[r.c0 + u];
+}
+
+template <bool kSeg>
 __global__ void __launch_bounds__(kMsmThreads)
 msm_finalize29_kernel(uint32_t chunk, const uint32_t* __restrict__ offsets, uint32_t nkeys, uint32_t span,
                       const Xyzz29* __restrict__ carry_own, const Xyzz29* __restrict__ carry_cont,
-                      uint32_t* __restrict__ large, Xyzz29* __restrict__ out29) {
+                      uint32_t* __restrict__ large, Xyzz29* __restrict__ out29, SegPlan pl) {
   tail_prio();
-  __shared__ uint32_t pk[kMsmThreads], pu[kMsmThreads], pe[kMsmThreads];
+  __shared__ uint32_t pk[kMsmThreads], pc[kMsmThreads], pe[kMsmThreads], po[kMsmThreads];
   __shared__ uint32_t cnt;
   if (threadIdx.x == 0) cnt = 0;
-  if (!chunk) chunk = dyn_chunk(offsets[nkeys]);
-  __syncthreads();
-  const size_t k = (size_t)blockIdx.x * blockDim.x + threadIdx.x;
-  uint32_t c0 = 0, c1 = 0;
+  if (!kSeg && !chunk) chunk = dyn_chunk(offsets[nkeys]);
+  __syncthreads();
+  const size_t id = (size_t)blockIdx.x * blockDim.x + threadIdx.x;
+  CarryRun r{0, 0, 0, 0};
   bool mine = false;
-  if (k < nkeys) {
-    const uint32_t s = offsets[k], e = offsets[k + 1];
-    if (e != s) {
-      c0 = s / chunk;
-      c1 = (e - 1) / chunk;
-      if (c1 - c0 > span)
-        large[1 + atomicAdd(&large[0], 1u)] = (uint32_t)k;
-      else
-        mine = c1 > c0;
-    }
+  if (id < (kSeg ? pl.meta[1] : nkeys) && (kSeg || offsets[id + 1] != offsets[id])) {
+    r = carry_run<kSeg>(chunk, offsets, pl, (uint32_t)id);
+    if (r.span - 1 > span)
+      large[1 + atomicAdd(&large[0], 1u)] = (uint32_t)id;
+    else
+      mine = r.span > 1;
   }
   if (mine) {
-    out29[k] = add29(carry_own[c0], carry_cont[c0 + 1]);
-    if (c1 > c0 + 1) {
+    out29[r.k] = add29(carry_at(carry_own, carry_cont, r, 0), carry_at(carry_own, carry_cont, r, 1));
+    if (r.span > 2) {
       const uint32_t i = atomicAdd(&cnt, 1u);
-      pk[i] = (uint32_t)k;
-      pu[i] = c0 + 2;
-      pe[i] = c1;
+      pk[i] = r.k;
+      pc[i] = r.c0;
+      pe[i] = r.span;
+      po[i] = r.own;
     }
   }
   __syncthreads();
   if (threadIdx.x < cnt) {
-    const uint32_t kk = pk[threadIdx.x], u1 = pe[threadIdx.x];
-    Xyzz29 v = out29[kk];
-    for (uint32_t u = pu[threadIdx.x]; u <= u1; u++) v = add29(v, carry_cont[u]);
-    out29[kk] = v;
+    const CarryRun w{pk[threadIdx.x], pc[threadIdx.x], pe[threadIdx.x], po[threadIdx.x]};
+    Xyzz29 v = out29[w.k];
+    for (uint32_t u = 2; u < w.span; u++) v = add29(v, carry_at(carry_own, carry_cont, w, u));
+    out29[w.k] = v;
   }
 }
 
@@ -854,25 +1028,20 @@
 
 static constexpr uint32_t kPieceCarries = (uint32_t)kSumThreads;
 
-__device__ __forceinline__ uint32_t carry_span(uint32_t chunk, const uint32_t* offsets, uint32_t k, uint32_t* c0) {
-  *c0 = offsets[k] / chunk;
-  return (offsets[k + 1] - 1) / chunk - *c0 + 1;
-}
-
+template <bool kSeg>
 __global__ void __launch_bounds__(1024)
 msm_large_scan_kernel(uint32_t chunk, const uint32_t* __restrict__ offsets, uint32_t nkeys,
-                      const uint32_t* __restrict__ large, uint32_t* __restrict__ off) {
+                      const uint32_t* __restrict__ large, uint32_t* __restrict__ off, SegPlan pl) {
   tail_prio();
   __shared__ uint32_t sh[1024];
   const uint32_t count = large[0];
-  const uint32_t ch = chunk ? chunk : dyn_chunk(offsets[nkeys]);
+  const uint32_t ch = kSeg || chunk ? chunk : dyn_chunk(offsets[nkeys]);
   const uint32_t tid = threadIdx.x;
   const uint32_t per = (count + 1023u) / 1024u;
   const uint32_t i0 = tid * per < count ? tid * per : count;
   const uint32_t i1 = i0 + per < count ? i0 + per : count;
   auto pieces = [&](uint32_t i) {
-    uint32_t c0;
-    return (carry_span(ch, offsets, large[1 + i], &c0) + kPieceCarries - 1) / kPieceCarries;
+    return (carry_run<kSeg>(ch, offsets, pl, large[1 + i]).span + kPieceCarries - 1) / kPieceCarries;
   };
   uint32_t sum = 0;
   for (uint32_t i = i0; i < i1; i++) sum += pieces(i);
@@ -912,53 +1081,55 @@
   return v;
 }
 
+template <bool kSeg>
 __global__ void __launch_bounds__(kSumThreads)
 msm_large_piece29_kernel(uint32_t chunk, const uint32_t* __restrict__ offsets, uint32_t nkeys,
                          const uint32_t* __restrict__ large, const uint32_t* __restrict__ off,
                          const Xyzz29* __restrict__ carry_own, const Xyzz29* __restrict__ carry_cont,
-                         Xyzz29* __restrict__ part) {
+                         Xyzz29* __restrict__ part, SegPlan pl) {
   tail_prio();
   __shared__ Xyzz29 sh[kSumThreads];
   const uint32_t count = large[0];
   const uint32_t total = off[count];
-  const uint32_t ch = chunk ? chunk : dyn_chunk(offsets[nkeys]);
+  const uint32_t ch = kSeg || chunk ? chunk : dyn_chunk(offsets[nkeys]);
   for (uint32_t item = blockIdx.x; item < total; item += gridDim.x) {
     uint32_t lo = 0, hi = count;
     while (hi - lo > 1) {
       const uint32_t mid = (lo + hi) >> 1;
       if (off[mid] <= item) lo = mid; else hi = mid;
     }
-    uint32_t c0;
-    const uint32_t span = carry_span(ch, offsets, large[1 + lo], &c0);
+    const CarryRun r = carry_run<kSeg>(ch, offsets, pl, large[1 + lo]);
     const uint32_t first = (item - off[lo]) * kPieceCarries;
-    const uint32_t n = span - first < kPieceCarries ? span - first : kPieceCarries;
+    const uint32_t n = r.span - first < kPieceCarries ? r.span - first : kPieceCarries;
     const uint32_t u = first + threadIdx.x;
     Xyzz29 v;
-    if (threadIdx.x < n) v = u ? carry_cont[c0 + u] : carry_own[c0];
+    if (threadIdx.x < n) v = carry_at(carry_own, carry_cont, r, u);
     v = tree_sum29(v, n, sh);
     if (threadIdx.x == 0) part[item] = v;
     __syncthreads();
   }
 }
 
-template <int NT>
+template <int NT, bool kSeg = false>
 __global__ void __launch_bounds__(NT)
 msm_large_final29_kernel(const uint32_t* __restrict__ large, const uint32_t* __restrict__ off,
-                         const Xyzz29* __restrict__ part, Xyzz29* __restrict__ out29) {
+                         const Xyzz29* __restrict__ part, Xyzz29* __restrict__ out29,
+                         const uint32_t* __restrict__ seg_mk) {
   tail_prio();
   __shared__ Xyzz29 sh[NT];
   const uint32_t count = large[0];
   for (uint32_t i = blockIdx.x; i < count; i += gridDim.x) {
     const uint32_t p0 = off[i], np = off[i + 1] - p0;
+    const uint32_t k = kSeg ? seg_mk[large[1 + i]] : large[1 + i];
     if (np == 1) {
-      if (threadIdx.x == 0) out29[large[1 + i]] = part[p0];
+      if (threadIdx.x == 0) out29[k] = part[p0];
       continue;
     }
     Xyzz29 v;
     if (threadIdx.x < np) v = part[p0 + threadIdx.x];
     for (uint32_t q = threadIdx.x + NT; q < np; q += NT) v = add29(v, part[p0 + q]);
     v = tree_sum29(v, np < NT ? np : NT, sh);
-    if (threadIdx.x == 0) out29[large[1 + i]] = v;
+    if (threadIdx.x == 0) out29[k] = v;
     __syncthreads();
   }
 }
@@ -1283,7 +1454,7 @@
   }
   const size_t ge = generic ? max_entries : 1;
   offsets.alloc(max_keys + 1);
-  sorted.alloc(max_entries);
+  sorted.alloc(max_entries + 4);
   keys_in.alloc(ge);
   keys_out.alloc(max_entries);
   vals_in.alloc(ge);
@@ -1292,7 +1463,8 @@
     radix_sort(nullptr, sort_tmp_bytes, keys_in.p, keys_out.p, vals_in.p, sorted.p, max_entries, 21, nullptr);
   }
   sort_tmp.alloc(sort_tmp_bytes + 16);
-  const size_t nthreads = std::max((max_entries + kChunk - 1) / kChunk, dyn_threads_bound(max_entries)) + 1;
+  const size_t nthreads = std::max({(max_entries + kChunk - 1) / kChunk, dyn_threads_bound(max_entries),
+                                    seg_whole_bound(max_entries)}) + 1;
   buckets.alloc(generic ? max_keys : 1);
   carry_own.alloc(generic ? nthreads : 1);
   carry_cont.alloc(generic ? nthreads : 1);
@@ -1300,7 +1472,7 @@
   if (fixed_base) {
     buckets29.alloc(max_keys);
     large_off.alloc(max_keys + 2);
-    large_part.alloc(nthreads / kPieceCarries + max_keys + 1);
+    large_part.alloc(std::max(nthreads, seg_carry_bound(max_entries, max_keys)) / kPieceCarries + max_keys + 1);
     carry_own29.alloc(nthreads);
     carry_cont29.alloc(nthreads);
     rowp29.alloc(max_tiles);
@@ -1309,6 +1481,18 @@
     bin_counts.alloc((size_t)256 * ((maxp + kTileScalars - 1) / kTileScalars) * lagrange_sets + 256);
     vals_mid.alloc(max_entries);
     lo_seg.alloc(lo_items_bound(max_entries) * ((size_t)1 << BinKeys<19>::LO));
+    if (acc_segments()) {
+      const size_t ns = seg_bound(max_entries, max_keys), nm = seg_multi_bound(max_entries, max_keys) + 1;
+      seg_start.alloc(ns);
+      seg_len.alloc(ns);
+      seg_bucket.alloc(ns);
+      seg_dst.alloc(ns);
+      seg_cnt.alloc(seg_counters(max_keys));
+      seg_meta.alloc(2);
+      seg_mk.alloc(nm);
+      seg_mfs.alloc(nm);
+      seg_mnp.alloc(nm);
+    }
   }
   seg_tot.alloc(max_seg && generic ? max_seg : 1);
   seg_run.alloc(max_seg && generic ? max_seg : 1);
@@ -1466,8 +1650,15 @@
     }
   }
 #endif
-  if (p.entries > sc.sorted.n || p.nkeys + 1 > sc.offsets.n)
+  if (p.entries + 4 > sc.sorted.n || p.nkeys + 1 > sc.offsets.n)
     throw Error(NZCB_ERR_ARG, "msm scratch was not sized for this schedule");
+  const bool seg = table && !table->sparse && msets == 1 && acc_segments();
+  if (seg && (seg_bound(p.entries, p.nkeys) > sc.seg_start.n || seg_counters(p.nkeys) > sc.seg_cnt.n ||
+              seg_multi_bound(p.entries, p.nkeys) + 1 > sc.seg_mk.n ||
+              seg_whole_bound(p.entries) + 1 > sc.carry_cont29.n ||
+              seg_carry_bound(p.entries, p.nkeys) / kPieceCarries + seg_multi_bound(p.entries, p.nkeys) + 1 >
+                  sc.large_part.n))
+    throw Error(NZCB_ERR_ARG, "msm scratch was not sized for the segment plan");
   if (table && ((size_t)p.nb / kTileSide * msets > sc.rowp29.n ||
                 (((size_t)1 << p.hb) + ((size_t)1 << p.a)) * msets > sc.lines29.n ||
                 (size_t)(p.lb + 1) * msets > sc.host_win_cap || (msets > 1 && p.c >= kStripMinC)))
@@ -1478,6 +1669,7 @@
   sc.cur_seglen = p.seglen;
   sc.cur_nkeys = p.nkeys;
   sc.cur_fixed = table != nullptr;
+  sc.cur_seg = seg;
   sc.cur_a = p.a;
   sc.cur_hb = p.hb;
   sc.cur_msets = p.msets;
@@ -1507,6 +1699,22 @@
                        dim3(kMsmThreads), 0, st, sc.keys_out.p, p.entries, p.nkeys, sc.offsets.p);
     NZ_HIP(hipGetLastError());
   }
+  const SegPlan pl{sc.seg_start.p, sc.seg_len.p, sc.seg_bucket.p, sc.seg_dst.p,
+                   sc.seg_mk.p,    sc.seg_mfs.p, sc.seg_mnp.p,   sc.seg_meta.p};
+  if (seg) {
+    const uint32_t ntiles = (uint32_t)seg_tiles(p.nkeys);
+    const dim3 tgrid((ntiles + kSegWaves - 1) / kSegWaves);
+    hipLaunchKernelGGL(msm_seg_hist_kernel, tgrid, dim3(kSegThreads), 0, st, (const uint32_t*)sc.offsets.p, p.nkeys,
+                       ntiles, sc.seg_cnt.p, sc.seg_meta.p);
+    NZ_HIP(hipGetLastError());
+    hipLaunchKernelGGL(msm_bin_rowscan_kernel, dim3(kSegMax), dim3(256), 0, st, sc.seg_cnt.p, ntiles,
+                       sc.seg_cnt.p + (size_t)kSegMax * ntiles);
+    NZ_HIP(hipGetLastError());
+    hipLaunchKernelGGL(msm_seg_scatter_kernel, tgrid, dim3(kSegThreads), 0, st, (const uint32_t*)sc.offsets.p, p.nkeys,
+                       ntiles, (const uint32_t*)sc.seg_cnt.p, pl);
+    NZ_HIP(hipGetLastError());
+    lmark("mark: L seg_plan");
+  }
   if (sc.prof) NZ_HIP(hipEventRecord(sc.ev[3], st));
   const bool sparse = table && table->sparse;
   sc.cur_sparse = sparse;
@@ -1514,7 +1722,12 @@
   const size_t nthreads = sparse ? dyn_threads_bound(p.entries) : (p.entries + chunk - 1) / chunk;
   const dim3 agrid(grid_for(nthreads, kMsmThreads, 1u << 30));
   const G1Affine* gather = table ? table->q.p : bases;
-  if (table) {
+  if (seg) {
+    const dim3 sgrid(grid_for(seg_bound(p.entries, p.nkeys), kMsmThreads, 1u << 30));
+    hipLaunchKernelGGL(msm_accumulate29_seg_kernel, sgrid, dim3(kMsmThreads), 0, st, gather, (const uint32_t*)sc.sorted.p,
+                       (const uint32_t*)pl.start, (const uint32_t*)pl.len, (const uint32_t*)pl.dst,
+                       (const uint32_t*)pl.meta, sc.buckets29.p, sc.carry_own29.p, sc.carry_cont29.p);
+  } else if (table) {
     if (chunk == kChunk || sparse)
       hipLaunchKernelGGL(msm_accumulate29_kernel<true>, agrid, dim3(kMsmThreads), 0, st, chunk, gather, sc.sorted.p,
                          sc.offsets.p, p.nkeys, nthreads, sc.buckets29.p, sc.carry_own29.p, sc.carry_cont29.p);
@@ -1530,28 +1743,34 @@
   if (sc.prof) NZ_HIP(hipEventRecord(sc.ev[4], st));
   const dim3 fgrid(grid_for(p.nkeys, kMsmThreads, 1u << 30));
   if (table) {
-    hipLaunchKernelGGL(msm_finalize29_kernel, fgrid, dim3(kMsmThreads), 0, st, chunk, sc.offsets.p, p.nkeys,
-                       sparse ? kSeqSpanSparse : kSeqSpan29, (const Xyzz29*)sc.carry_own29.p,
-                       (const Xyzz29*)sc.carry_cont29.p, sc.large.p, sc.buckets29.p);
-    NZ_HIP(hipGetLastError());
-    lmark("mark: L finalize");
-    hipLaunchKernelGGL(msm_large_scan_kernel, dim3(1), dim3(1024), 0, st, chunk, sc.offsets.p, p.nkeys, sc.large.p,
-                       sc.large_off.p);
-    NZ_HIP(hipGetLastError());
-    lmark("mark: L large_scan");
-    hipLaunchKernelGGL(msm_large_piece29_kernel, dim3(sparse ? kSparsePieceBlocks : kLargePieceBlocks),
-                       dim3(kSumThreads), 0, st, chunk, sc.offsets.p, p.nkeys, sc.large.p, sc.large_off.p,
-                       (const Xyzz29*)sc.carry_own29.p, (const Xyzz29*)sc.carry_cont29.p, sc.large_part.p);
-    NZ_HIP(hipGetLastError());
-    lmark("mark: L piece");
-    if (sparse)
-      hipLaunchKernelGGL(msm_large_final29_kernel<kSumThreads>, dim3(kSparseFinalBlocks), dim3(kSumThreads), 0, st,
-                         sc.large.p, sc.large_off.p, sc.large_part.p, sc.buckets29.p);
-    else
-      hipLaunchKernelGGL(msm_large_final29_kernel<64>, dim3(kLargeFinalBlocks), dim3(64), 0, st, sc.large.p,
-                         sc.large_off.p, sc.large_part.p, sc.buckets29.p);
-    NZ_HIP(hipGetLastError());
-    lmark("mark: L final");
+    auto finalize = [&](auto kseg) {
+      constexpr bool kSeg = decltype(kseg)::value;
+      const dim3 grid = kSeg ? dim3(grid_for(seg_multi_bound(p.entries, p.nkeys) + 1, kMsmThreads, 1u << 30)) : fgrid;
+      hipLaunchKernelGGL(msm_finalize29_kernel<kSeg>, grid, dim3(kMsmThreads), 0, st, chunk, sc.offsets.p, p.nkeys,
+                         sparse ? kSeqSpanSparse : kSeqSpan29, (const Xyzz29*)sc.carry_own29.p,
+                         (const Xyzz29*)sc.carry_cont29.p, sc.large.p, sc.buckets29.p, pl);
+      NZ_HIP(hipGetLastError());
+      lmark("mark: L finalize");
+      hipLaunchKernelGGL(msm_large_scan_kernel<kSeg>, dim3(1), dim3(1024), 0, st, chunk, sc.offsets.p, p.nkeys,
+                         sc.large.p, sc.large_off.p, pl);
+      NZ_HIP(hipGetLastError());
+      lmark("mark: L large_scan");
+      hipLaunchKernelGGL(msm_large_piece29_kernel<kSeg>, dim3(sparse ? kSparsePieceBlocks : kLargePieceBlocks),
+                         dim3(kSumThreads), 0, st, chunk, sc.offsets.p, p.nkeys, sc.large.p, sc.large_off.p,
+                         (const Xyzz29*)sc.carry_own29.p, (const Xyzz29*)sc.carry_cont29.p, sc.large_part.p, pl);
+      NZ_HIP(hipGetLastError());
+      lmark("mark: L piece");
+      if (sparse)
+        hipLaunchKernelGGL((msm_large_final29_kernel<kSumThreads, kSeg>), dim3(kSparseFinalBlocks), dim3(kSumThreads),
+                           0, st, sc.large.p, sc.large_off.p, sc.large_part.p, sc.buckets29.p,
+                           (const uint32_t*)pl.mk);
+      else
+        hipLaunchKernelGGL((msm_large_final29_kernel<64, kSeg>), dim3(kLargeFinalBlocks), dim3(64), 0, st, sc.large.p,
+                           sc.large_off.p, sc.large_part.p, sc.buckets29.p, (const uint32_t*)pl.mk);
+      NZ_HIP(hipGetLastError());
+      lmark("mark: L final");
+    };
+    if (seg) finalize(std::true_type()); else finalize(std::false_type());
     mark(5);
     int lparts = p.ltiles, hparts = p.htiles;
     if (p.c >= kStripMinC) {
@@ -1608,6 +1827,26 @@
   NZ_HIP(hipEventRecord(sc.done, st));
 }
 
+bool msm_debug_plan(MsmScratch& sc, hipStream_t st, std::vector<uint32_t>& offsets, std::vector<uint32_t>& start,
+                    std::vector<uint32_t>& len, std::vector<uint32_t>& bucket) {
+  if (!sc.cur_fixed || !sc.cur_seg || sc.cur_n == 0) return false;
+  NZ_HIP(hipStreamSynchronize(st));
+  uint32_t meta[2] = {0, 0};
+  NZ_HIP(hipMemcpy(meta, sc.seg_meta.p, sizeof(meta), hipMemcpyDeviceToHost));
+  if (meta[0] > sc.seg_start.n) throw Error(NZCB_ERR_INTERNAL, "segment plan larger than its bound");
+  offsets.resize((size_t)sc.cur_nkeys + 1);
+  start.resize(meta[0]);
+  len.resize(meta[0]);
+  bucket.resize(meta[0]);
+  NZ_HIP(hipMemcpy(offsets.data(), sc.offsets.p, offsets.size() * 4, hipMemcpyDeviceToHost));
+  if (meta[0]) {
+    NZ_HIP(hipMemcpy(start.data(), sc.seg_start.p, (size_t)meta[0] * 4, hipMemcpyDeviceToHost));
+    NZ_HIP(hipMemcpy(len.data(), sc.seg_len.p, (size_t)meta[0] * 4, hipMemcpyDeviceToHost));
+    NZ_HIP(hipMemcpy(bucket.data(), sc.seg_bucket.p, (size_t)meta[0] * 4, hipMemcpyDeviceToHost));
+  }
+  return true;
+}
+
 void msm_enqueue(MsmScratch& sc, const G1Affine* bases, const Fr* scalars, size_t n, bool mont, hipStream_t st,
                  const MsmBaseTable* table) {
   const Fr* one[1] = {scalars};
diff --git a/nzcb-circom_amd/csrc/msm_seg.h b/nzcb-circom_amd/csrc/msm_seg.h
--- /dev/null
+++ b/nzcb-circom_amd/csrc/msm_seg.h
@@ -0,0 +1,36 @@
+#pragma once
+#include <cstddef>
+#include <cstdint>
+
+namespace nzcb {
+
+#ifndef NZ_SEG_MAX
+#define NZ_SEG_MAX 256
+#endif
+constexpr uint32_t kSegMax = NZ_SEG_MAX;
+static_assert(kSegMax >= 4 && kSegMax <= 256, "segment cap: 4..256");
+
+#ifndef NZ_SEG_TILE
+#define NZ_SEG_TILE 512
+#endif
+constexpr uint32_t kSegTile = NZ_SEG_TILE;
+static_assert(kSegTile % 64 == 0, "whole waves of buckets");
+
+constexpr uint32_t seg_count(uint32_t len, uint32_t cap = kSegMax) { return (len + cap - 1) / cap; }
+
+constexpr size_t seg_bound(size_t entries, size_t nkeys, size_t cap = kSegMax) { return entries / cap + nkeys; }
+
+constexpr size_t seg_whole_bound(size_t entries, size_t cap = kSegMax) { return entries / cap; }
+
+constexpr size_t seg_multi_bound(size_t entries, size_t nkeys, size_t cap = kSegMax) {
+  return entries / (cap + 1) < nkeys ? entries / (cap + 1) : nkeys;
+}
+
+constexpr size_t seg_carry_bound(size_t entries, size_t nkeys, size_t cap = kSegMax) {
+  return seg_whole_bound(entries, cap) + seg_multi_bound(entries, nkeys, cap);
+}
+
+constexpr size_t seg_tiles(size_t nkeys) { return (nkeys + kSegTile - 1) / kSegTile; }
+constexpr size_t seg_counters(size_t nkeys, size_t cap = kSegMax) { return cap * seg_tiles(nkeys) + 256; }
+
+}
diff --git a/nzcb-circom_amd/nzcb/__init__.py b/nzcb-circom_amd/nzcb/__init__.py
--- a/nzcb-circom_amd/nzcb/__init__.py
+++ b/nzcb-circom_amd/nzcb/__init__.py
@@ -34,7 +34,7 @@
     "nzcb_nzcp_witness_dev", "nzcb_synth_setup_ex", "nzcb_memcpy_d2d",
     "nzcb_plonk_setup", "nzcb_prove_batch_status", "nzcb_wprog_remap", "nzcb_prove_logged", "nzcb_memcpy_d2d_async",
     "nzcb_debug_guard_check", "nzcb_debug_guard_selftest", "nzcb_debug_inject_fault", "nzcb_debug_f29",
-    "nzcb_debug_ntt_coset",
+    "nzcb_debug_ntt_coset", "nzcb_debug_msm_plan",
     "nzcb_msm_table_create_lagrange",
     "nzcb_verify_batch", "nzcb_engine_g1_lincomb", "nzcb_engine_verify_batch", "nzcb_debug_verify_batch_timings",
     "nzcb_r1cs_create", "nzcb_r1cs_create_file", "nzcb_r1cs_info", "nzcb_r1cs_check", "nzcb_r1cs_destroy",
@@ -213,6 +213,9 @@
                                               c_int, u8p, POINTER(_Err)]),
         "nzcb_engine_msm_sets_dev": (c_int, [c_void_p, c_void_p, c_size_t, POINTER(c_void_p), c_int, c_size_t, c_int,
                                              c_int, u8p, POINTER(_Err)]),
+        "nzcb_debug_msm_plan": (c_int, [c_void_p, c_void_p, c_size_t, c_void_p, c_size_t, c_int, c_int, c_int,
+                                        POINTER(c_uint32), POINTER(c_uint32), c_size_t, POINTER(c_uint32), c_size_t,
+                                        u8p, POINTER(_Err)]),
         "nzcb_plonk_setup": (c_int, [ctypes.c_char_p, c_size_t, ctypes.c_char_p, c_size_t, c_int, POINTER(POINTER(c_uint8)),
                                      POINTER(c_size_t), POINTER(_Err)]),
         "nzcb_nzcp_input_signals": (c_size_t, [POINTER(NzcpParams)]),
@@ -538,6 +541,22 @@
                                                       out, ctypes.byref(err)), err)
         return bytes(out)
 
+    def msm_plan(self, dev_bases: int, n_table: int, dev_scalars: int, n: int, scalars_mont: bool, window: int = 0,
+                 fold: bool = False):
+        c = window or 20
+        off_cap = (1 << (c - 1)) + 1
+        seg_cap = 3 * (n * ((255 + c - 1) // c) + 1)
+        info, off, seg = (c_uint32 * 4)(), (c_uint32 * off_cap)(), (c_uint32 * seg_cap)()
+        out = _out(64)
+        err = _Err()
+        _check(self.lib.nzcb_debug_msm_plan(self.h, dev_bases, n_table, dev_scalars, n, int(scalars_mont), int(window),
+                                            int(fold), info, off, off_cap, seg, seg_cap, out, ctypes.byref(err)), err)
+        if not info[0]:
+            return bytes(out), None
+        nk, ns = info[1], info[2]
+        return bytes(out), {"seg_max": info[3], "offsets": off[:nk + 1], "start": seg[:ns], "len": seg[ns:2 * ns],
+                            "bucket": seg[2 * ns:3 * ns]}
+
     def msm_sets_dev(self, dev_bases: int, n_table: int, dev_scalars: list, n: int, scalars_mont: bool, *,
                      sparse: bool) -> list:
         k = len(dev_scalars)
```

After: 49.82 proofs/s, median of 6. 2.9% higher.
